# tjhladish/PLS

Hardware: AMD Instinct MI355X
Metric: NIPALS components/sec (higher is better)
Workload: dtype f64; 1 GPU; C3: synthetic tall n=1048576 x p=512, m=1, A=20, f64, resident in HBM; algo=nipals, fuse=1, deflation_written_back_every=1, rows_per_gpu=1048576, parallelism=single GPU

## Files before the change

pls_amd/csrc/ctx.hpp:

```cpp
#pragma once

namespace {

struct DevBuf {
    void *p = nullptr;
    size_t bytes = 0;
};

struct Launch {
    int fam;
    i64 bytes;
    hipEvent_t e0, e1;
};

}

struct pls_hip_context {
    int device = 0;
    hipStream_t stream = nullptr;
    pls_hip_allreduce_fn reducer = nullptr;
    void *reducer_user = nullptr;
    int rank = 0, nranks = 1;
    double *user_red = nullptr;
    i64 user_red_count = 0;
    i64 opt_algo = PLS_HIP_ALGO_KERNEL, opt_fuse = 1, opt_profile = 0, opt_power_iters = 48;
    i64 opt_fused_grid = 0, opt_work_layout = 1, opt_defer = 1, opt_graph = 0;
    std::vector<uint64_t> graph_key, graph_seen;
    hipGraphExec_t graph_exec = nullptr;
    DevBuf zeros, part, sspart, xbpart, wide1, red, red2, xx, xyp, praw, xy, v, cs, coop, lm, gxx, gxy, tab, work, cvidx, cvx, cvy, cvws, cve, cvtx, cvty, cvtt, cvm, cvkeep, cvred, hX, hY, hT, hW, hP, hQ, hR, hB, hIn, hOut;
    DevBuf valout, valpart, vale, valacc, valkeys, valhist;
    DevBuf xdS, xdQ, xdPT, xdred, xdtv, xdoQ, xdoT, xdoS, xdsmall;
    DevBuf bws, bv, bred, bmsg, bssy, bY, boR, boQ, bott, boB, bossy;
    DevBuf dG, dpart, dV, dT, dY, dZ, dC, dscr;
    DevBuf dcv;
    DevBuf dbat;
    DevBuf dcvb, cvbpos, cvbidx, cvbo, cvboE;
    DevBuf rsw, rsB, rsacc, rsX, rsY, rsW, rsoS;
    DevBuf mX, mws, mit, mzo;
    i64 opt_missing_iters = 500;
    int *mconv_host = nullptr;
    i64 opt_val_lds_rows = -1;
    i64 val_lds_rows_dev = -1;
    std::string err;
    std::vector<hipEvent_t> ev_pool;
    size_t ev_used = 0;
    std::vector<Launch> launches;
    std::vector<Launch> fits;
    Launch cur_fit{};
    bool fit_timed = false;
    int num_cu = 256;
    plsh::Stager stager;
    int copy_threads = 0;
    hipStream_t copy_stream = nullptr;
    const double *pre_xx = nullptr, *pre_xy = nullptr;
    bool defer_free = false;
    std::vector<void *> graveyard;
    struct XchgIpc *xchg = nullptr;
    struct XchgEndpoint {
        bool on = false;
        int n = 0, rank = 0;
        double *const *inbox = nullptr;
        unsigned long long *const *flags = nullptr;
        unsigned long long *seq = nullptr;
        int *status = nullptr, *host_status = nullptr;
        const long long *limit = nullptr;
    } xep;
    DevBuf tailcnt;
    DevBuf resident;
    DevBuf rgflags;
    unsigned rg_epoch = 0;
    unsigned long long resident_launches = 0;
    struct Env {
        bool turnaround = true;
        i64 turn_edge_bytes = plsk::TURN_EDGE_BYTES;
        bool batch_refit = false;
        i64 batch_round = 0;
        i64 dualcv_round = 0;
        i64 dualbatch_round = 0;
        i64 resample_round = 0;
        bool resample_refit = false;
        bool dualbatch_sweeps = false;
        bool cvbatch_refit = false;
        i64 dualcvb_round = 0;
        bool tiny = true, cv_refit = false, tail = true, replica_guard = true, resident = true;
        int tail_update = 1;
        int xb4 = 1;
        int resident_gram = 1;
    } env;
    int *diverged = nullptr, *diverged_dev = nullptr;
    DevBuf guard;
#ifdef PLS_HIP_TESTING
    int poison_new = -1;
#endif
};

#define PLS_HIP_WORKSPACES(SCRATCH, STATEFUL)                                                                                        \
    STATEFUL(zeros, WS_ALL, "256 zero bytes, cleared once when first used and only read afterwards: the source of out-of-range rows of the LDS-DMA panels") \
    STATEFUL(resident, 256, "two arrival counters of the resident fits, used in alternating parity (resident_launches): each launch zeroes the counter of the next; the payload behind the 256 bytes is scratch") \
    STATEFUL(rgflags, WS_ALL, "one arrival word per workgroup of resident_gram_fit_kernel: values only grow, a launch waits for words beyond rg_epoch, which the host advances by 4 per launch") \
    STATEFUL(gxx, c->pre_xx ? WS_ALL : 0, "X^T X accumulated during an upload, only while pre_xx points into it: from upload_accumulate to the end of the same host-memory fit") \
    STATEFUL(gxy, c->pre_xy ? WS_ALL : 0, "X^T Y accumulated during an upload, only while pre_xy points into it: from upload_accumulate to the end of the same host-memory fit") \
    SCRATCH(tailcnt) SCRATCH(part) SCRATCH(sspart) SCRATCH(xbpart) SCRATCH(wide1) SCRATCH(red) SCRATCH(red2) SCRATCH(xx) SCRATCH(xyp)  \
    SCRATCH(praw) SCRATCH(xy) SCRATCH(v) SCRATCH(cs) SCRATCH(coop) SCRATCH(lm) SCRATCH(tab) SCRATCH(work)                              \
    SCRATCH(cvidx) SCRATCH(cvx) SCRATCH(cvy) SCRATCH(cvws) SCRATCH(cve) SCRATCH(cvtx) SCRATCH(cvty) SCRATCH(cvtt) SCRATCH(cvm)         \
    SCRATCH(cvkeep) SCRATCH(cvred)                                                                                                     \
    SCRATCH(hX) SCRATCH(hY) SCRATCH(hT) SCRATCH(hW) SCRATCH(hP) SCRATCH(hQ) SCRATCH(hR) SCRATCH(hB) SCRATCH(hIn) SCRATCH(hOut)         \
    SCRATCH(valout) SCRATCH(valpart) SCRATCH(vale) SCRATCH(valacc) SCRATCH(valkeys) SCRATCH(valhist)                                   \
    SCRATCH(xdS) SCRATCH(xdQ) SCRATCH(xdPT) SCRATCH(xdred) SCRATCH(xdtv) SCRATCH(xdoQ) SCRATCH(xdoT) SCRATCH(xdoS) SCRATCH(xdsmall)    \
    SCRATCH(bws) SCRATCH(bv) SCRATCH(bred) SCRATCH(bmsg) SCRATCH(bssy) SCRATCH(bY) SCRATCH(boR) SCRATCH(boQ) SCRATCH(bott)             \
    SCRATCH(boB) SCRATCH(bossy)                                                                                                        \
    SCRATCH(dG) SCRATCH(dpart) SCRATCH(dV) SCRATCH(dT) SCRATCH(dY) SCRATCH(dZ) SCRATCH(dC) SCRATCH(dscr) SCRATCH(dcv) SCRATCH(dbat)    \
    SCRATCH(dcvb) SCRATCH(cvbpos) SCRATCH(cvbidx) SCRATCH(cvbo) SCRATCH(cvboE)                                                         \
    SCRATCH(rsw) SCRATCH(rsB) SCRATCH(rsacc) SCRATCH(rsX) SCRATCH(rsY) SCRATCH(rsW) SCRATCH(rsoS)                                      \
    SCRATCH(mX) SCRATCH(mws) SCRATCH(mit) SCRATCH(mzo)                                                                                 \
    SCRATCH(guard)

namespace {

constexpr size_t WS_ALL = ~(size_t)0;

template <typename F>
void for_each_workspace(pls_hip_context *c, F &&f) {
#define PLS_HIP_WS_SCRATCH(name) f(c->name, (size_t)0);
#define PLS_HIP_WS_STATEFUL(name, keep, reason) f(c->name, (size_t)(keep));
    PLS_HIP_WORKSPACES(PLS_HIP_WS_SCRATCH, PLS_HIP_WS_STATEFUL)
#undef PLS_HIP_WS_SCRATCH
#undef PLS_HIP_WS_STATEFUL
}

#define HIPCHK(ctx, call)                                                                  \
    do {                                                                                   \
        hipError_t e__ = (call);                                                           \
        if (e__ != hipSuccess) {                                                           \
            (ctx)->err = std::string(#call) + ": " + hipGetErrorString(e__);               \
            return PLS_HIP_ERR_DEVICE;                                                     \
        }                                                                                  \
    } while (0)

#define CHK(expr)                      \
    do {                               \
        int rc__ = (expr);             \
        if (rc__ != PLS_HIP_OK) return rc__; \
    } while (0)

int fail(pls_hip_context *c, int code, const std::string &msg) {
    c->err = msg;
    return code;
}

int ensure(pls_hip_context *c, DevBuf &b, size_t bytes) {
    if (bytes <= b.bytes && b.p) return PLS_HIP_OK;
    if (b.p) {
        if (c->defer_free) {
            c->graveyard.push_back(b.p);
        } else {
            HIPCHK(c, hipStreamSynchronize(c->stream));
            HIPCHK(c, hipFree(b.p));
        }
        b.p = nullptr;
        b.bytes = 0;
    }
    bytes = std::max<size_t>(bytes, 256);
    if (hipMalloc(&b.p, bytes) != hipSuccess) {
        (void)hipGetLastError();
        b.p = nullptr;
        return fail(c, PLS_HIP_ERR_ALLOC, "hipMalloc of " + std::to_string(bytes) + " bytes failed");
    }
    b.bytes = bytes;
#ifdef PLS_HIP_TESTING
    if (c->poison_new >= 0) {
        HIPCHK(c, hipMemsetAsync(b.p, c->poison_new, bytes, c->stream));
        HIPCHK(c, hipStreamSynchronize(c->stream));
    }
#endif
    return PLS_HIP_OK;
}

size_t esize(int dtype) { return dtype == PLS_HIP_F64 ? 8 : 4; }

hipEvent_t take_event(pls_hip_context *c) {
    if (c->ev_used == c->ev_pool.size()) {
        hipEvent_t e = nullptr;
        if (hipEventCreate(&e) != hipSuccess) return nullptr;
        c->ev_pool.push_back(e);
    }
    return c->ev_pool[c->ev_used++];
}
struct Scope {
    pls_hip_context *c;
    Launch l{};
    bool on;
    Scope(pls_hip_context *ctx, int fam, i64 bytes)
        : c(ctx), on(ctx->opt_profile >= 2 || (ctx->opt_profile == 1 && fam != PLS_HIP_FAM_SMALL)) {
        if (!on) return;
        l.fam = fam;
        l.bytes = bytes;
        l.e0 = take_event(c);
        l.e1 = take_event(c);
        if (!l.e0 || !l.e1) { on = false; return; }
        (void)hipEventRecord(l.e0, c->stream);
    }
    ~Scope() {
        if (!on) return;
        (void)hipEventRecord(l.e1, c->stream);
        c->launches.push_back(l);
    }
};

struct Roctx {
    int (*push)(const char *) = nullptr;
    int (*pop)() = nullptr;
    Roctx() {
        const char *e = getenv("PLS_HIP_ROCTX");
        if (!e || atoi(e) == 0) return;
        void *lib = dlopen("librocprofiler-sdk-roctx.so", RTLD_NOW | RTLD_GLOBAL);
        if (!lib) lib = dlopen("libroctx64.so", RTLD_NOW | RTLD_GLOBAL);
        if (!lib) return;
        push = reinterpret_cast<int (*)(const char *)>(dlsym(lib, "roctxRangePushA"));
        pop = reinterpret_cast<int (*)()>(dlsym(lib, "roctxRangePop"));
        if (!push || !pop) push = nullptr;
    }
};
inline Roctx &roctx() {
    static Roctx r;
    return r;
}
struct Range {
    bool on;
    explicit Range(const char *text) : on(roctx().push != nullptr) {
        if (on) roctx().push(text);
    }
    Range(const char *prefix, int n) : on(roctx().push != nullptr) {
        if (on) {
            char buf[64];
            std::snprintf(buf, sizeof(buf), "%s %d", prefix, n);
            roctx().push(buf);
        }
    }
    ~Range() {
        if (on) roctx().pop();
    }
};

#define LAUNCH_CHECK(ctx)                                                           \
    do {                                                                            \
        hipError_t e__ = hipGetLastError();                                         \
        if (e__ != hipSuccess) {                                                    \
            (ctx)->err = std::string("kernel launch: ") + hipGetErrorString(e__);   \
            return PLS_HIP_ERR_DEVICE;                                              \
        }                                                                           \
    } while (0)

}
```

pls_amd/csrc/fused_kernels.hpp:

```cpp
#pragma once
#include <type_traits>

#include "common.hpp"
#include "exchange_kernels.hpp"
#include "update_m1.hpp"

namespace plsk {

#ifdef PLS_HIP_TESTING
__device__ unsigned long long *g_pass_stamps = nullptr;
#define PLS_STAMP(slot)                                                                                 \
    do {                                                                                                \
        if (g_pass_stamps && threadIdx.x == 0) {                                                        \
            g_pass_stamps[(size_t)blockIdx.x * 8 + (slot)] = wall_clock64();                            \
            if ((slot) == 0) {         \
                g_pass_stamps[(size_t)blockIdx.x * 8 + 4] = __builtin_amdgcn_s_getreg((31 << 11) | 20);  \
                g_pass_stamps[(size_t)blockIdx.x * 8 + 5] = __builtin_amdgcn_s_getreg((31 << 11) | 4);   \
            }                                                                                           \
        }                                                                                               \
    } while (0)
#else
#define PLS_STAMP(slot) do { } while (0)
#endif

typedef unsigned int u32x4 __attribute__((ext_vector_type(4)));

constexpr int BUF_WORD3 = 0x00020000;
constexpr int AUX_SC1 = 16;

template <typename T, int V, int AUX = 0>
__device__ __forceinline__ Pack<T, V> buf_ld(__amdgpu_buffer_rsrc_t r, uint32_t voff) {
    static_assert(sizeof(Pack<T, V>) == 16, "16-byte accesses");
    const u32x4 raw = __builtin_amdgcn_raw_buffer_load_b128(r, voff, 0, AUX);
    Pack<T, V> p;
    __builtin_memcpy(&p, &raw, 16);
    return p;
}
template <typename T, int V, int AUX = 0>
__device__ __forceinline__ void buf_st(__amdgpu_buffer_rsrc_t r, uint32_t voff, const Pack<T, V> &p) {
    u32x4 raw;
    __builtin_memcpy(&raw, &p, 16);
    __builtin_amdgcn_raw_buffer_store_b128(raw, r, voff, 0, AUX);
}
template <typename T, int V, int AUX = 0>
__device__ __forceinline__ Pack<T, V> buf_ld_so(__amdgpu_buffer_rsrc_t r, uint32_t voff, int soff) {
    static_assert(sizeof(Pack<T, V>) == 16, "16-byte accesses");
    const u32x4 raw = __builtin_amdgcn_raw_buffer_load_b128(r, voff, soff, AUX);
    Pack<T, V> p;
    __builtin_memcpy(&p, &raw, 16);
    return p;
}
template <typename T, int V, int AUX = 0>
__device__ __forceinline__ void buf_st_so(__amdgpu_buffer_rsrc_t r, uint32_t voff, int soff, const Pack<T, V> &p) {
    u32x4 raw;
    __builtin_memcpy(&raw, &p, 16);
    __builtin_amdgcn_raw_buffer_store_b128(raw, r, voff, soff, AUX);
}

template <typename T, int V>
__device__ __forceinline__ Pack<T, V> ld_pack_u(const T *p) {
    Pack<T, V> o;
    __builtin_memcpy(&o, p, sizeof(o));
    return o;
}
template <typename T, int V>
__device__ __forceinline__ void st_pack_u(T *p, const Pack<T, V> &x) {
    __builtin_memcpy(p, &x, sizeof(x));
}

template <typename T>
__device__ __forceinline__ __amdgpu_buffer_rsrc_t score_rsrc(const T *col, i64 nvalid) {
    return __builtin_amdgcn_make_buffer_rsrc(const_cast<T *>(col), (short)0, (int)(nvalid * (i64)sizeof(T)), BUF_WORD3);
}

struct TailUpdate {
    double *XY = nullptr;
    double *W = nullptr, *P = nullptr, *Q = nullptr, *R = nullptr, *vnext = nullptr;
    int A = 0, a = 0, nipals = 0;
};

struct WalkWeights {
    int nfull = -1;
    unsigned mask = 0;
    int rev = 0;
    int edge = 0;
};

struct Turn {
    bool on = false;
    bool rev = false;
    i64 edge_bytes = 0;
};

#ifdef PLS_HIP_TESTING
struct TurnRecord {
    int rev = 0, edge = 0, ntiles = 0, grid = 0;
};
inline TurnRecord g_test_turn;
#endif

struct SliceTail {
    unsigned *cnt = nullptr;
    double *red = nullptr;
    int nrows = 0;
    int npush = 0;
    unsigned long long seq = 0;
    XchgPeers peers;
    TailUpdate upd;
    XchgGather gx;
};

constexpr int TAIL_MIN_WG = 32;
constexpr int TAIL_AUX_SYS = 17;

__device__ __noinline__ void tail_update_m1(const double *src, i64 stride, int n, int sys, int ok, double *XY, double *W, double *P,
                                            double *Q, double *R, double *vnext, int K, int A, int a, int nipals, double *scratch,
                                            double *wl) {
    typedef unsigned int u32x2 __attribute__((ext_vector_type(2)));
    static_assert(XCHG_MAX == 2 * RED_SLICES, "two batches of RED_SLICES loads");
    const int L = K + 1;
    update_m1<512, 1>(
        [&](int j) -> double {
            double sum = 0.0;
#pragma unroll
            for (int h = 0; h < 2; ++h) {
                if (h * RED_SLICES >= n) break;
                double x[RED_SLICES];
#pragma unroll
                for (int m = 0; m < RED_SLICES; ++m) {
                    const int mm = h * RED_SLICES + m;
                    const __amdgpu_buffer_rsrc_t rs = __builtin_amdgcn_make_buffer_rsrc(
                        const_cast<double *>(src + (i64)(mm < n ? mm : 0) * stride), (short)0, L * 8, BUF_WORD3);
                    const u32x2 raw = sys ? __builtin_amdgcn_raw_buffer_load_b64(rs, (uint32_t)j * 8u, 0, TAIL_AUX_SYS)
                                          : __builtin_amdgcn_raw_buffer_load_b64(rs, (uint32_t)j * 8u, 0, AUX_SC1);
                    __builtin_memcpy(&x[m], &raw, 8);
                }
#pragma unroll
                for (int m = 0; m < RED_SLICES; ++m)
                    if (h * RED_SLICES + m < n) sum += x[m];
            }
            return ok ? sum : __builtin_nan("");
        },
        XY, W, P, Q, R, vnext, K, A, a, nipals, 0, scratch + UPD1_VWAVES, scratch, wl);
}

template <int NT>
__device__ __forceinline__ void slice_tail(const SliceTail &st, const double *part, const double *sspart, int K, int *role,
                                        double *sm, double *scratch, double *wl) {
    static_assert(NT >= WG, "the t^T t sum takes the first four waves");
    const int tid = threadIdx.x, nb = st.nrows, nwg = gridDim.x, b = blockIdx.x;
    constexpr int NSL = RED_SLICES;
    const int sl = (int)(((i64)(b + 1) * NSL + nb - 1) / nb) - 1;
    if (tid == 0) {
        const int lo_ = (int)((i64)nb * sl / NSL), hi_ = (int)((i64)nb * (sl + 1) / NSL);
        const unsigned mine = (unsigned)(min(hi_, nwg) - lo_);
        const unsigned ticket = __hip_atomic_fetch_add(st.cnt + sl, 1u, __ATOMIC_RELAXED, __HIP_MEMORY_SCOPE_AGENT);
        const int last = (ticket + 1u == mine);
        if (last) {
            __hip_atomic_store(st.cnt + sl, 0u, __ATOMIC_RELAXED, __HIP_MEMORY_SCOPE_AGENT);
        }
        *role = last;
    }
    __syncthreads();
    if (!*role) return;
    const i64 LP = K + 1;
    typedef unsigned int u32x2 __attribute__((ext_vector_type(2)));
    {
        const int s8 = sl;
        const int lo = (int)((i64)nb * s8 / RED_SLICES), hi = (int)((i64)nb * (s8 + 1) / RED_SLICES);
        double ssl = 0.0;
        {
            const __amdgpu_buffer_rsrc_t rq =
                __builtin_amdgcn_make_buffer_rsrc(const_cast<double *>(sspart), (short)0, nb * 8, BUF_WORD3);
            if (tid < WG)
                for (int r = lo + tid; r < hi; r += WG) {
                    const u32x2 raw = __builtin_amdgcn_raw_buffer_load_b64(rq, (uint32_t)r * 8u, 0, AUX_SC1);
                    double d;
                    __builtin_memcpy(&d, &raw, 8);
                    ssl += d;
                }
        }
        {
            const __amdgpu_buffer_rsrc_t rs = __builtin_amdgcn_make_buffer_rsrc(const_cast<double *>(part + (i64)lo * K), (short)0,
                                                                                (int)((i64)(hi - lo) * K * 8), BUF_WORD3);
            auto ld = [&](int row, int j) -> double {
                const u32x2 raw = __builtin_amdgcn_raw_buffer_load_b64(rs, (uint32_t)(((i64)row * K + j) * 8), 0, AUX_SC1);
                double d;
                __builtin_memcpy(&d, &raw, 8);
                return d;
            };
            const int nr = hi - lo;
            for (int j = tid; j < K; j += NT) {
                double c[4] = {0.0, 0.0, 0.0, 0.0};
                int r = 0;
                for (; r + 16 <= nr; r += 16) {
                    double x[16];
#pragma unroll
                    for (int u = 0; u < 16; ++u) x[u] = ld(r + u, j);
#pragma unroll
                    for (int u = 0; u < 16; ++u) c[u & 3] += x[u];
                }
                for (; r < nr; r += 4) {
                    double x[4];
#pragma unroll
                    for (int u = 0; u < 4; ++u) x[u] = (r + u < nr) ? ld(r + u, j) : 0.0;
#pragma unroll
                    for (int u = 0; u < 4; ++u)
                        if (r + u < nr) c[u] += x[u];
                }
                st_agent(st.red + (i64)s8 * LP + j, (c[0] + c[1]) + (c[2] + c[3]));
            }
        }
        {
            double sw = wave_sum(ssl);
            __syncthreads();
            if ((tid & 63) == 0 && tid < WG) sm[tid >> 6] = sw;
            __syncthreads();
            if (tid == 0) st_agent(st.red + (i64)s8 * LP + K, ((sm[0] + sm[1]) + sm[2]) + sm[3]);
        }
    }
    if (st.npush <= 0 && !st.upd.XY) return;
    asm volatile("s_waitcnt vmcnt(0)" ::: "memory");
    __syncthreads();
    {
        if (tid == 0) {
            const unsigned ticket = __hip_atomic_fetch_add(st.cnt + RED_SLICES, 1u, __ATOMIC_RELAXED, __HIP_MEMORY_SCOPE_AGENT);
            const int last = (ticket + 1u == (unsigned)NSL);
            if (last) {
                __hip_atomic_store(st.cnt + RED_SLICES, 0u, __ATOMIC_RELAXED, __HIP_MEMORY_SCOPE_AGENT);
            }
            *role = last;
        }
        __syncthreads();
        if (!*role) return;
    }
    const __amdgpu_buffer_rsrc_t rr =
        __builtin_amdgcn_make_buffer_rsrc(st.red, (short)0, (int)((i64)RED_SLICES * LP * 8), BUF_WORD3);
    if (st.npush > 0) {
        for (int j = tid; j <= K; j += NT) {
            double x[RED_SLICES];
#pragma unroll
            for (int i = 0; i < RED_SLICES; ++i) {
                const u32x2 raw = __builtin_amdgcn_raw_buffer_load_b64(rr, (uint32_t)(((i64)i * LP + j) * 8), 0, AUX_SC1);
                __builtin_memcpy(&x[i], &raw, 8);
            }
            double sum = x[0];
#pragma unroll
            for (int i = 1; i < RED_SLICES; ++i) sum += x[i];
            for (int d = 0; d < st.npush; ++d) __hip_atomic_store(st.peers.slot[d] + j, sum, __ATOMIC_RELAXED, __HIP_MEMORY_SCOPE_SYSTEM);
        }
        asm volatile("s_waitcnt vmcnt(0)" ::: "memory");
        __syncthreads();
        if (tid < st.npush) __hip_atomic_store(st.peers.flag[tid], st.seq, __ATOMIC_RELEASE, __HIP_MEMORY_SCOPE_SYSTEM);
    }
    if (!st.upd.XY) return;
    const TailUpdate &u = st.upd;
    if (st.gx.n > 0) {
        const XchgGather &gx = st.gx;
        if (tid == 0) *role = (*gx.status == 0);
        __syncthreads();
        if (tid < gx.n && *role) {
            const long long t0 = wall_clock64();
            while (__hip_atomic_load(gx.flags + tid, __ATOMIC_RELAXED, __HIP_MEMORY_SCOPE_SYSTEM) < gx.seq) {
                if (wall_clock64() - t0 > gx.limit) {
                    *role = 0;
                    break;
                }
                __builtin_amdgcn_s_sleep(4);
            }
            __builtin_amdgcn_fence(__ATOMIC_ACQUIRE, "");
            asm volatile("s_waitcnt vmcnt(0)" ::: "memory");
        }
        __syncthreads();
        const int ok = *role;
        if (!ok && tid == 0) {
            *gx.status = 1;
            __hip_atomic_store(gx.host_status, 1, __ATOMIC_RELAXED, __HIP_MEMORY_SCOPE_SYSTEM);
        }
        tail_update_m1(gx.inbox, gx.cap, gx.n, 1, ok, u.XY, u.W, u.P, u.Q, u.R, u.vnext, K, u.A, u.a, u.nipals, scratch, wl);
        return;
    }
    tail_update_m1(st.red, LP, RED_SLICES, 0, 1, u.XY, u.W, u.P, u.Q, u.R, u.vnext, K, u.A, u.a, u.nipals, scratch, wl);
}

constexpr int AUX_NT = 2;
constexpr i64 TURN_EDGE_BYTES = 192ll << 20;
constexpr bool TURN_LEAD_ST_DEFAULT = true;

template <bool XCD, int R>
struct TileWalk {
    __device__ __forceinline__ explicit TileWalk(i64) {}
    __device__ __forceinline__ unsigned first() const { return blockIdx.x; }
    __device__ __forceinline__ unsigned step() const { return gridDim.x; }
    __device__ __forceinline__ i64 nlim(i64 N) const { return N; }
};
template <int R>
struct TileWalk<true, R> {
    i64 first_, step_, nlim_;
    __device__ __forceinline__ explicit TileWalk(i64 N) : first_(blockIdx.x), step_(gridDim.x), nlim_(N) {
        if ((gridDim.x & 7) == 0) {
            const i64 per = ((N + R - 1) / R + 7) / 8;
            first_ = (i64)(blockIdx.x & 7) * per + (blockIdx.x >> 3);
            step_ = gridDim.x >> 3;
            nlim_ = min(N, (i64)((blockIdx.x & 7) + 1) * per * R);
        }
    }
    __device__ __forceinline__ i64 first() const { return first_; }
    __device__ __forceinline__ i64 step() const { return step_; }
    __device__ __forceinline__ i64 nlim(i64) const { return nlim_; }
};

template <typename T, int V, int R, int NT, int CPT, bool DEFL, int LDAUX_ = AUX_NT, int STAUX = AUX_NT, bool RDST = false,
          int EDGE = 0, bool TILED = false, bool ONEWG = false, bool STORE = true>
__global__ __launch_bounds__(NT, (NT / 256) * ((CPT <= 16 && !DEFL && !ONEWG) ? 2 : 1)) void fused_pass_kernel(
    const T *X, i64 ldx, i64 tsx, T *dst, i64 ldd, i64 tsd, i64 N, int K,
    const double *__restrict__ v, const T *__restrict__ tprev, const double *__restrict__ pprev,
    T *__restrict__ tout, double *__restrict__ part, double *__restrict__ sspart, int rdst, i64 NV, const SliceTail st,
    const WalkWeights wk) {
    constexpr int RP = R / V;
    constexpr int CG = NT / RP;
    constexpr int NW = NT / WAVE;
    constexpr int LDAUX = (EDGE == 2) ? 0 : LDAUX_;
    static_assert(RP <= WAVE && WAVE % RP == 0 && NT % RP == 0, "tile shape");
    static_assert(!TILED || (EDGE == 0 && !RDST), "the tiled copy is aligned and keeps one tile shape");
    static_assert(STORE || (DEFL && !RDST), "only a deflating pass has a store side to drop; without it there is no destination tile shape");
    constexpr bool DYN = (size_t)2 * CG * CPT * sizeof(double) > 48 * 1024;
    struct alignas(16) Lds {
        alignas(16) double ps[(DEFL && !DYN) ? CG * CPT : 2];
        alignas(16) double vs[DYN ? 2 : CG * CPT];
        alignas(16) double tred[2][NW][R];
        alignas(16) double sred[NW];
    };
    __shared__ Lds lds;
    extern __shared__ double fused_dyn[];
    double *vs = DYN ? fused_dyn : lds.vs, *ps = DYN ? fused_dyn + CG * CPT : lds.ps;
    auto &tred = lds.tred;
    double *sred = lds.sred;

    const int tid = threadIdx.x, lane = tid & 63, wv = tid >> 6;
    const int rp = tid % RP, cg = tid / RP;
    PLS_STAMP(0);
    constexpr bool LATE_OK = TILED && DEFL && CG * CPT <= NT;
    const bool LATE_FILL = LATE_OK && (rdst & 0x10000);
    double v_late = 0.0, p_late = 0.0;
    if (LATE_FILL) {
        if (tid < CG * CPT) {
            v_late = (tid < K) ? v[tid] : 0.0;
            p_late = (tid < K) ? pprev[tid] : 0.0;
        }
    } else {
        for (int k = tid; k < CG * CPT; k += NT) {
            vs[k] = (k < K) ? v[k] : 0.0;
            if (DEFL) ps[k] = (k < K) ? pprev[k] : 0.0;
        }
        __syncthreads();
    }
    bool first_tile = true;

    double pacc[CPT];
#pragma unroll
    for (int j = 0; j < CPT; ++j) pacc[j] = 0.0;
    double ss = 0.0;
    int buf = 0;
    constexpr int CGD = EDGE ? WAVE / RP : CG;
    const int cgw = EDGE ? __builtin_amdgcn_readfirstlane(cg) : 0;
    const uint32_t xoff = (uint32_t)(((i64)rp * V + (i64)(cg - cgw) * ldx) * (i64)sizeof(T));
    uint32_t doff = (DEFL && STORE) ? (uint32_t)(((i64)rp * V + (i64)cg * ldd) * (i64)sizeof(T)) : 0u;
    i64 dtile = tsd;
    if constexpr (RDST && DEFL) {
        doff = (uint32_t)(((i64)((rp * V) / rdst) * tsd + (rp * V) % rdst + (i64)cg * ldd) * (i64)sizeof(T));
        dtile = (R / rdst) * tsd;
    }
    constexpr uint32_t OOR = 0x80000000u;
    constexpr bool TBUF = DEFL && sizeof(T) == 8 && R == 32 && CPT == 16;
    const __amdgpu_buffer_rsrc_t rs_tin = score_rsrc<T>(DEFL ? tprev : tout, NV);

    TileWalk<EDGE == 2, R> walk(N);
    const int pace = rdst & 0xffff;
    constexpr bool WEIGHTED = DEFL && EDGE != 2;
    const int wfast = (WEIGHTED && wk.nfull >= 0) ? ((wk.mask >> (blockIdx.x & 7)) & 1) : 0;
    const i64 wswitch = (WEIGHTED && wk.nfull >= 0) ? (i64)wk.nfull * gridDim.x : (i64)1 << 62;
    i64 wstep = walk.step();
    bool wshared = true;
    constexpr bool TURNS = DEFL;
    constexpr bool EDGES = TILED && DEFL && STORE;
    const bool rev = TURNS && wk.rev;
    const i64 ntl = (N + R - 1) / R;
    const i64 etrail = ntl - wk.edge;
    for (i64 pos = walk.first(); pos * R < walk.nlim(N); buf ^= 1) {
        const i64 tile = rev ? ntl - 1 - pos : pos;
        if constexpr (EDGES) {
            if (pos < wk.edge) {
                constexpr int LA = 0, SA = TURN_LEAD_ST_DEFAULT ? 0 : STAUX;
#include "fused_pass_tile.inc"
            } else if (pos >= etrail) {
                constexpr int LA = 0, SA = 0;
#include "fused_pass_tile.inc"
            } else {
                constexpr int LA = LDAUX, SA = STAUX;
#include "fused_pass_tile.inc"
            }
        } else {
            constexpr int LA = LDAUX, SA = STAUX;
#include "fused_pass_tile.inc"
        }
        if constexpr (!WEIGHTED) {
            pos += walk.step();
            continue;
        }
        pos += wstep;
        if (wshared && pos >= wswitch) {
            if (!wfast) break;
            wshared = false;
            const int nfc = __builtin_popcount(wk.mask), below = __builtin_popcount(wk.mask & ((1u << (blockIdx.x & 7)) - 1u));
            pos = wswitch + (i64)(blockIdx.x >> 3) * nfc + below;
            wstep = (i64)(gridDim.x >> 3) * nfc;
        }
    }

    PLS_STAMP(1);
#pragma unroll
    for (int j = 0; j < CPT; ++j) {
        const double s = xor_range_sum<1, RP>(pacc[j]);
        const int k = cg + CG * j;
        if (rp == 0 && k < K) st_agent(part + (i64)blockIdx.x * K + k, s);
    }
    ss = block_sum<NW>(ss, sred);
    if (tid == 0) st_agent(sspart + blockIdx.x, ss);
    constexpr bool ONE_PER_CU = !(CPT <= 16 && !DEFL) || ONEWG;
    if (ONE_PER_CU && st.cnt) {
        asm volatile("s_waitcnt vmcnt(0)" ::: "memory");
        __syncthreads();
        static_assert(NT == 512, "tail_update_m1 plays the update's 1024 virtual threads with 512");
        PLS_STAMP(2);
        slice_tail<NT>(st, part, sspart, K, reinterpret_cast<int *>(sred + NW - 1), sred, &tred[0][0][0], vs);
    }
    PLS_STAMP(3);
}

template <typename T, int V, int R, int NT, int CPT, int EDGE = 0>
__global__ __launch_bounds__(NT, (NT / 256) * 2) void deflate_score_kernel(
    const T *src, i64 lds_, i64 tss, T *dst, i64 ldd, i64 tsd, int rdst, i64 N, int K, const T *__restrict__ tprev,
    const double *__restrict__ pprev, const double *__restrict__ w, T *__restrict__ tout,
    double *__restrict__ sspart, i64 NV) {
    constexpr int RP = R / V, CG = NT / RP, NW = NT / WAVE;
    extern __shared__ double dyn[];
    __shared__ double tred[2][NW][R];
    __shared__ double sred[NW];
    double *ws = dyn, *ps = dyn + K;
    const int tid = threadIdx.x, lane = tid & 63, wv = tid >> 6;
    const int rp = tid % RP, cg = tid / RP;
    for (int k = tid; k < K; k += NT) {
        ws[k] = w[k];
        ps[k] = pprev[k];
    }
    __syncthreads();
    constexpr int CGD = EDGE ? WAVE / RP : CG;
    constexpr int LDAUX = (EDGE == 2) ? 0 : AUX_NT;
    const int cgw = EDGE ? __builtin_amdgcn_readfirstlane(cg) : 0;
    const uint32_t soff = (uint32_t)(((i64)rp * V + (i64)(cg - cgw) * lds_) * (i64)sizeof(T));
    const int dsub = (rp * V) / rdst, dwithin = (rp * V) % rdst, dtiles = R / rdst;
    const uint32_t doff = (uint32_t)(((i64)dsub * tsd + dwithin + (i64)cg * ldd) * (i64)sizeof(T));
    constexpr uint32_t OOR = 0x80000000u;
    const int ngroups = (K + CG - 1) / CG;
    const __amdgpu_buffer_rsrc_t rs_tin = score_rsrc<T>(tprev, NV);
    double ss = 0.0;
    int buf = 0;
    TileWalk<EDGE == 2, R> walk(N);
    for (i64 tile = walk.first(); tile * R < walk.nlim(N); tile += walk.step(), buf ^= 1) {
        const i64 i0 = tile * R + (i64)rp * V;
        const bool rowok = (i0 < N);
        const uint32_t so = rowok ? soff : OOR, dof = rowok ? doff : OOR;
        double tp[V], tacc[V];
        {
            const Pack<T, V> tpk = buf_ld<T, V>(rs_tin, rowok ? (uint32_t)(i0 * (i64)sizeof(T)) : OOR);
#pragma unroll
            for (int e = 0; e < V; ++e) tp[e] = -(double)tpk.v[e];
        }
#pragma unroll
        for (int e = 0; e < V; ++e) tacc[e] = 0.0;
        for (int g0 = 0; g0 < ngroups; g0 += CPT) {
            Pack<T, V> x[CPT];
#pragma unroll
            for (int j = 0; j < CPT; ++j) {
                const int cols = min(CGD, K - CG * (g0 + j) - cgw);
                const uint32_t nrec = cols > 0 ? (uint32_t)((i64)cols * lds_ * (i64)sizeof(T)) : 0u;
                const __amdgpu_buffer_rsrc_t rs = __builtin_amdgcn_make_buffer_rsrc(
                    const_cast<T *>(src + tile * tss + (i64)((g0 + j) * CG + cgw) * lds_), (short)0, (int)nrec, BUF_WORD3);
                x[j] = buf_ld<T, V, LDAUX>(rs, so);
                __builtin_amdgcn_sched_barrier(0);
            }
#pragma unroll
            for (int j = 0; j < CPT; ++j) {
                const int k = cg + CG * (g0 + j);
                const double pk = (k < K) ? ps[k] : 0.0, wk = (k < K) ? ws[k] : 0.0;
#pragma unroll
                for (int e = 0; e < V; ++e) {
                    x[j].v[e] = (T)fma(tp[e], pk, (double)x[j].v[e]);
                    tacc[e] = fma((double)x[j].v[e], wk, tacc[e]);
                }
                const __amdgpu_buffer_rsrc_t rd = __builtin_amdgcn_make_buffer_rsrc(
                    dst + tile * dtiles * tsd + (i64)(g0 + j) * CG * ldd, (short)0, 0x7fffffff, BUF_WORD3);
                buf_st<T, V, AUX_NT>(rd, (k < K) ? dof : OOR, x[j]);
            }
        }
#pragma unroll
        for (int e = 0; e < V; ++e)
            tacc[e] = xor_range_sum<RP, WAVE>(tacc[e]);
        if (lane < RP)
#pragma unroll
            for (int e = 0; e < V; ++e) tred[buf][wv][rp * V + e] = tacc[e];
        __syncthreads();
        if (cg == 0 && rowok) {
            Pack<T, V> o;
#pragma unroll
            for (int e = 0; e < V; ++e) {
                double s = 0.0;
#pragma unroll
                for (int q = 0; q < NW; ++q) s += tred[buf][q][rp * V + e];
                o.v[e] = (T)s;
                const double ts = (double)o.v[e];
                ss = fma(ts, ts, ss);
            }
            if (i0 + V <= NV) {
                st_pack_u<T, V>(tout + i0, o);
            } else {
#pragma unroll
                for (int e = 0; e < V; ++e)
                    if (i0 + e < NV) tout[i0 + e] = o.v[e];
            }
        }
    }
    ss = block_sum<NW>(ss, sred);
    if (tid == 0) sspart[blockIdx.x] = ss;
}

template <typename T>
struct TailArgs {
    const T *src = nullptr; i64 lds = 0, tss = 0; int rs = 1;
    T *dst = nullptr; i64 ldd = 0, tsd = 0; int rd = 1;
    const T *tprev = nullptr; const double *pprev = nullptr;
    const double *v = nullptr; T *tout = nullptr; const T *tgiven = nullptr;
    double *part = nullptr, *sspart = nullptr;
    const T *Y = nullptr; i64 ldy = 0; int M = 0;
    i64 row0 = 0; int nrows = 0, K = 0;
    int zero_rows = 0;
};

template <typename T>
__global__ __launch_bounds__(WG) void tail_rows_kernel(TailArgs<T> a) {
    __shared__ double sm[WG / WAVE];
    constexpr int MAXR = 16 / sizeof(T) - 1;
    double t[MAXR];
    double ss = 0.0;
    for (int r = 0; r < MAXR; ++r) {
        t[r] = 0.0;
        if (r >= a.nrows) continue;
        const i64 i = a.row0 + r;
        const T *srow = a.src + (i / a.rs) * a.tss + i % a.rs;
        T *drow = a.dst ? a.dst + (i / a.rd) * a.tsd + i % a.rd : nullptr;
        const double tp = a.tprev ? -(double)a.tprev[i] : 0.0;
        double sum = 0.0;
        for (int k = threadIdx.x; k < a.K; k += WG) {
            T x = srow[(i64)k * a.lds];
            if (a.tprev) x = (T)fma(tp, a.pprev[k], (double)x);
            if (drow) drow[(i64)k * a.ldd] = x;
            if (a.v) sum = fma((double)x, a.v[k], sum);
        }
        if (a.v) {
            t[r] = (double)(T)block_sum<WG / WAVE>(sum, sm);
            if (threadIdx.x == 0 && a.tout) a.tout[i] = (T)t[r];
        } else if (a.tgiven) {
            t[r] = (double)a.tgiven[i];
        }
        ss = fma(t[r], t[r], ss);
    }
    if (a.dst)
        for (int r = 0; r < a.zero_rows; ++r) {
            const i64 i = a.row0 + a.nrows + r;
            T *drow = a.dst + (i / a.rd) * a.tsd + i % a.rd;
            for (int k = threadIdx.x; k < a.K; k += WG) drow[(i64)k * a.ldd] = (T)0;
        }
    if (a.part) {
        const int nm = a.Y ? a.M : 1;
        for (int k = threadIdx.x; k < a.K; k += WG)
            for (int m = 0; m < nm; ++m) {
                double p = 0.0;
                for (int r = 0; r < MAXR; ++r)
                    if (r < a.nrows) {
                        const i64 i = a.row0 + r;
                        double x;
                        if (a.dst) {
                            x = (double)a.dst[(i / a.rd) * a.tsd + i % a.rd + (i64)k * a.ldd];
                        } else {
                            const T xs = a.src[(i / a.rs) * a.tss + i % a.rs + (i64)k * a.lds];
                            x = a.tprev ? (double)(T)fma(-(double)a.tprev[i], a.pprev[k], (double)xs) : (double)xs;
                        }
                        p = fma(x, a.Y ? (double)a.Y[i + (i64)m * a.ldy] : t[r], p);
                    }
                a.part[k + (i64)m * a.K] = p;
            }
    }
    if (a.sspart && threadIdx.x == 0) *a.sspart = ss;
}

template <typename T>
void launch_tail_rows(hipStream_t stream, const TailArgs<T> &a) {
    hipLaunchKernelGGL((tail_rows_kernel<T>), dim3(1), dim3(WG), 0, stream, a);
}

template <typename T, int V, int R, int NT, int CPTB, int MT, int EDGE = 0, bool LT = false>
__global__ __launch_bounds__(NT, NT / 256) void retile_xty_kernel(const T *src, i64 lds_, const T *__restrict__ Y,
                                                                        i64 ldy, T *dst, i64 ldd, i64 tsd, int rdst, i64 N,
                                                                        int K, int M, double *__restrict__ part, int tpw) {
    constexpr int RP = R / V, CG = NT / RP;
    constexpr int LDAUX = (EDGE == 2) ? 0 : AUX_NT;
    constexpr bool YLDS = MT >= 4;
    constexpr int TU = (CPTB < 8) ? 2 : 1;
    constexpr int YE = (TU * R * MT + NT - 1) / NT;
    __shared__ alignas(16) T ys[2][YLDS ? TU * MT : 1][YLDS ? R : V];
    extern __shared__ __attribute__((aligned(16))) unsigned char retile_dyn[];
    Pack<T, V> *trans = reinterpret_cast<Pack<T, V> *>(retile_dyn);
    constexpr int W = CG * CPTB;
    static_assert(!LT || (W % 16 == 0 && (RP * W) % NT == 0 && RP <= 16), "transposed store shape");
    const int rp = threadIdx.x % RP, cg = threadIdx.x / RP;
    const int g0 = blockIdx.y * CPTB;
    constexpr int CGD = EDGE ? WAVE / RP : CG;
    const int cgw = EDGE ? __builtin_amdgcn_readfirstlane(cg) : 0;
    const uint32_t soff = (uint32_t)(((i64)rp * V + (i64)(cg - cgw) * lds_) * (i64)sizeof(T));
    const int dsub = (rp * V) / rdst, dwithin = (rp * V) % rdst, dtiles = R / rdst;
    const uint32_t doff = (uint32_t)(((i64)dsub * tsd + dwithin + (i64)cg * ldd) * (i64)sizeof(T));
    constexpr uint32_t OOR = 0x80000000u;
    const i64 ntiles = (N + R - 1) / R;
    const i64 tile0 = (i64)blockIdx.x * tpw, tile1 = min(ntiles, tile0 + (i64)tpw);
    double acc[CPTB][MT];
#pragma unroll
    for (int j = 0; j < CPTB; ++j)
#pragma unroll
        for (int m = 0; m < MT; ++m) acc[j][m] = 0.0;
    int buf = 0;
    for (i64 tile = tile0; tile < tile1; tile += TU, buf ^= 1) {
        Pack<T, V> x[TU][CPTB];
#pragma unroll
        for (int u = 0; u < TU; ++u) {
            const bool rowok = (tile + u < tile1) && ((tile + u) * R + (i64)rp * V < N);
#pragma unroll
            for (int j = 0; j < CPTB; ++j) {
                const int cols = min(CGD, K - CG * (g0 + j) - cgw);
                const uint32_t nrec = cols > 0 ? (uint32_t)((i64)cols * lds_ * (i64)sizeof(T)) : 0u;
// ... 32 lines not shown
                __syncthreads();
#pragma unroll
                for (int j = 0; j < CPTB; ++j) trans[rp * W + ((cg + CG * j) ^ rp)] = x[u][j];
                __syncthreads();
                const __amdgpu_buffer_rsrc_t rd =
                    __builtin_amdgcn_make_buffer_rsrc(dst + (tile + u) * dtiles * tsd, (short)0, 0x7fffffff, BUF_WORD3);
                const int Q = rdst / V;
#pragma unroll
                for (int jj = 0; jj < RP * W / NT; ++jj) {
                    const int L = jj * NT + (int)threadIdx.x;
                    const int d = L / (W * Q), rem = L - d * (W * Q);
                    const int c = (Q == 1) ? rem : (rem >> 1), q = (Q == 1) ? 0 : (rem & 1);
                    const int rp2 = d * Q + q;
                    const Pack<T, V> pk = trans[rp2 * W + (c ^ rp2)];
                    const int k = g0 * CG + c;
                    const bool ok = (tile + u < tile1) && ((tile + u) * R + (i64)rp2 * V < N) && (k < K);
                    const uint32_t off = (uint32_t)(((i64)d * tsd + (i64)q * V + (i64)k * ldd) * (i64)sizeof(T));
                    buf_st<T, V, AUX_NT>(rd, ok ? off : OOR, pk);
                }
            }
#pragma unroll
            for (int m = 0; m < MT; ++m) {
                Pack<T, V> yp;
                if constexpr (YLDS) {
                    yp = *reinterpret_cast<const Pack<T, V> *>(&ys[buf][u * MT + m][rp * V]);
                } else {
                    if (m < M && rowok) {
                        yp = ld_pack_u<T, V>(Y + i0 + (i64)m * ldy);
                    } else {
#pragma unroll
                        for (int e = 0; e < V; ++e) yp.v[e] = (T)0;
                    }
                }
#pragma unroll
                for (int e = 0; e < V; ++e) {
                    const double ye = (double)yp.v[e];
#pragma unroll
                    for (int j = 0; j < CPTB; ++j) acc[j][m] = fma((double)x[u][j].v[e], ye, acc[j][m]);
                }
            }
        }
    }
#pragma unroll
    for (int j = 0; j < CPTB; ++j) {
        const int k = cg + CG * (g0 + j);
#pragma unroll
        for (int m = 0; m < MT; ++m) {
            const double s = xor_range_sum<1, RP>(acc[j][m]);
            if (rp == 0 && k < K && m < M) part[(i64)blockIdx.x * ((i64)K * M) + k + (i64)m * K] = s;
        }
    }
}

template <typename T, int CGX = 32>
int launch_retile_xty(hipStream_t stream, int num_cu, const T *src, i64 lds_, const T *Y, i64 ldy, T *dst, i64 ldd, i64 tsd,
                      int rdst, i64 N, int K, int M, double *part, int max_rows, int *nb) {
    constexpr int V = 16 / sizeof(T);
    constexpr int R = (512 / CGX) * V, NT = 512;
    constexpr int CG = NT / (R / V);
    const bool nostore = dst == nullptr;
    if (nostore) { ldd = R; tsd = (i64)R * K; rdst = R; }
    if ((!nostore && !cols_aligned((uintptr_t)dst, ldd, sizeof(T))) || tsd % V != 0 || rdst < V || R % rdst != 0 || N < 1 || M < 1 || M > 8 || max_rows < 2 ||
        !elem_aligned((uintptr_t)Y, sizeof(T)))
        return 1;
    const int edge = edge_level((uintptr_t)src, lds_, sizeof(T), CG, WAVE / (R / V));
    if (edge < 0) return 1;
    if (!nostore && ((i64)(R / rdst) * tsd + (i64)CG * ldd) * (i64)sizeof(T) >= (1ll << 31)) return 1;
    const i64 Nf = N - N % V;
    int gx = 0;
    if (Nf > 0) {
        const i64 ntiles = (Nf + R - 1) / R;
        const int cptb = (M > 4 || (M > 2 && sizeof(T) == 4)) ? 4 : 8;
        const int nkb = (K + CG * cptb - 1) / (CG * cptb);
        const i64 want = std::max<i64>(1, std::min<i64>(((i64)(nostore ? 4 : 1) * num_cu + nkb - 1) / nkb, max_rows - 1));
        const i64 tpw = (ntiles + want - 1) / want;
        gx = (int)((ntiles + tpw - 1) / tpw);
        const dim3 g((unsigned)gx, (unsigned)nkb), b(NT);
        const bool lt = CGX == 32 && rdst == V && M <= 2 && !nostore;
#define RX_LAUNCH(CPTB_, MT_, E_) \
    hipLaunchKernelGGL((retile_xty_kernel<T, V, R, NT, CPTB_, MT_, E_>), g, b, 0, stream, src, lds_, Y, ldy, dst, ldd, tsd, rdst, Nf, K, M, part, (int)tpw)
#define RX_LAUNCH_LT(CPTB_, MT_, E_)                                                                                      \
    do {                                                                                                                  \
        if constexpr (CGX == 32) {                                                                                        \
            auto kfn = &retile_xty_kernel<T, V, R, NT, CPTB_, MT_, E_, true>;                                             \
            const int dynb = (R / V) * CG * CPTB_ * 16;                                                                   \
            if (dynb > 48 * 1024 && !raise_dynamic_lds(reinterpret_cast<const void *>(kfn), dynb)) return 1;              \
            hipLaunchKernelGGL(kfn, g, b, dynb, stream, src, lds_, Y, ldy, dst, ldd, tsd, rdst, Nf, K, M, part, (int)tpw); \
        }                                                                                                                 \
    } while (0)
#define RX_CASE(CPTB_, MT_)                                                                                               \
    do {                                                                                                                  \
        if (lt) { if (edge == 2) RX_LAUNCH_LT(CPTB_, MT_, 2); else if (edge) RX_LAUNCH_LT(CPTB_, MT_, 1); else RX_LAUNCH_LT(CPTB_, MT_, 0); } \
        else if (edge == 2) RX_LAUNCH(CPTB_, MT_, 2); else if (edge) RX_LAUNCH(CPTB_, MT_, 1); else RX_LAUNCH(CPTB_, MT_, 0); \
    } while (0)
#define RX_CASE_D(CPTB_, MT_) \
    do { if (edge == 2) RX_LAUNCH(CPTB_, MT_, 2); else if (edge) RX_LAUNCH(CPTB_, MT_, 1); else RX_LAUNCH(CPTB_, MT_, 0); } while (0)
        if (M > 4) RX_CASE_D(4, 8);
        else if (M > 2 && cptb == 4) RX_CASE_D(4, 4);
        else if (M > 2) RX_CASE_D(8, 4);
        else if (M > 1) RX_CASE(8, 2);
        else RX_CASE(8, 1);
#undef RX_CASE_D
#undef RX_CASE
#undef RX_LAUNCH_LT
#undef RX_LAUNCH
    }
    if (Nf < N) {
        TailArgs<T> a;
        a.src = src; a.lds = lds_; a.tss = R; a.rs = R;
        a.dst = dst; a.ldd = ldd; a.tsd = tsd; a.rd = rdst;
        a.part = part + (i64)gx * K * M; a.Y = Y; a.ldy = ldy; a.M = M;
        a.row0 = Nf; a.nrows = (int)(N - Nf); a.K = K; a.zero_rows = V - a.nrows;
        launch_tail_rows(stream, a);
        ++gx;
    }
    *nb = gx;
    return 0;
}

template <typename T>
int launch_deflate_score(hipStream_t stream, int num_cu, const T *src, i64 lds_, i64 tss, T *dst, i64 ldd, i64 tsd,
                         int rdst, i64 N, int K, const T *tprev, const double *pprev, const double *w, T *tout,
                         double *sspart, int max_rows, int *nss, bool src_padded = false) {
    constexpr int V = 16 / sizeof(T);
    constexpr int R = 256 / sizeof(T), NT = 512, CPT = 8;
    constexpr int CG = NT / (R / V);
    if (N < 1 || max_rows < 2 || !cols_aligned((uintptr_t)dst, ldd, sizeof(T)) || !elem_aligned((uintptr_t)tprev, sizeof(T)) || !elem_aligned((uintptr_t)tout, sizeof(T))) return 1;
    if ((N + V) * (i64)sizeof(T) >= (1ll << 31)) return 1;
    const int edge = edge_level((uintptr_t)src, lds_, sizeof(T), CG, WAVE / (R / V));
    if (edge < 0 || (edge == 0 && tss % V != 0)) return 1;
    if (tsd % V != 0 || rdst < V || R % rdst != 0) return 1;
    if (((i64)(R / rdst) * tsd + (i64)CG * ldd) * (i64)sizeof(T) >= (1ll << 31)) return 1;
    if ((i64)CG * ldd * (i64)sizeof(T) >= (1ll << 31)) return 1;
    const size_t dyn = (size_t)K * 16;
    if (dyn > 72 * 1024) return 1;
    auto kfn = edge == 2 ? &deflate_score_kernel<T, V, R, NT, CPT, 2>
                         : (edge == 1 ? &deflate_score_kernel<T, V, R, NT, CPT, 1> : &deflate_score_kernel<T, V, R, NT, CPT, 0>);
    if (dyn > 48 * 1024 && !raise_dynamic_lds(reinterpret_cast<const void *>(kfn), 72 * 1024)) return 1;
    const i64 Nf = src_padded ? (N + V - 1) / V * V : N - N % V;
    i64 grid = 0;
    if (Nf > 0) {
        const i64 ntiles = (Nf + R - 1) / R;
        grid = std::min<i64>(std::min<i64>(ntiles, 2 * (i64)num_cu), max_rows - 1);
        hipLaunchKernelGGL(kfn, dim3((unsigned)grid), dim3(NT), (size_t)K * 16, stream, src, lds_, tss, dst, ldd, tsd, rdst, Nf,
                           K, tprev, pprev, w, tout, sspart, N);
    }
    if (Nf < N) {
        TailArgs<T> a;
        a.src = src; a.lds = lds_; a.tss = tss; a.rs = R;
        a.dst = dst; a.ldd = ldd; a.tsd = tsd; a.rd = rdst;
        a.tprev = tprev; a.pprev = pprev; a.v = w; a.tout = tout; a.sspart = sspart + grid;
        a.row0 = Nf; a.nrows = (int)(N - Nf); a.K = K; a.zero_rows = V - a.nrows;
        launch_tail_rows(stream, a);
        ++grid;
    }
    *nss = (int)grid;
    return 0;
}

template <typename T, int V, int R, int NT, int CPT, int EDGE = 0>
__global__ __launch_bounds__(NT, (NT / 256) * 2) void retile_kernel(const T *src, i64 lds_, T *dst, i64 ldd, i64 tsd,
                                                                    int rdst, i64 N, int K) {
    constexpr int RP = R / V, CG = NT / RP;
    constexpr int CGD = EDGE ? WAVE / RP : CG;
    constexpr int LDAUX = (EDGE == 2) ? 0 : AUX_NT;
    const int rp = threadIdx.x % RP, cg = threadIdx.x / RP;
    const int cgw = EDGE ? __builtin_amdgcn_readfirstlane(cg) : 0;
    const uint32_t soff = (uint32_t)(((i64)rp * V + (i64)(cg - cgw) * lds_) * (i64)sizeof(T));
    const int dsub = (rp * V) / rdst, dwithin = (rp * V) % rdst, dtiles = R / rdst;
    const uint32_t doff = (uint32_t)(((i64)dsub * tsd + dwithin + (i64)cg * ldd) * (i64)sizeof(T));
    constexpr uint32_t OOR = 0x80000000u;
    const int ngroups = (K + CG - 1) / CG;
    TileWalk<EDGE == 2, R> walk(N);
    for (i64 tile = walk.first(); tile * R < walk.nlim(N); tile += walk.step()) {
        const bool rowok = (tile * R + (i64)rp * V < N);
        const uint32_t so = rowok ? soff : OOR, dof = rowok ? doff : OOR;
        for (int g0 = 0; g0 < ngroups; g0 += CPT) {
            Pack<T, V> x[CPT];
#pragma unroll
            for (int j = 0; j < CPT; ++j) {
                const int cols = min(CGD, K - CG * (g0 + j) - cgw);
                const uint32_t nrec = cols > 0 ? (uint32_t)((i64)cols * lds_ * (i64)sizeof(T)) : 0u;
                const __amdgpu_buffer_rsrc_t rs = __builtin_amdgcn_make_buffer_rsrc(
                    const_cast<T *>(src + tile * R + (i64)((g0 + j) * CG + cgw) * lds_), (short)0, (int)nrec, BUF_WORD3);
                x[j] = buf_ld<T, V, LDAUX>(rs, so);
                __builtin_amdgcn_sched_barrier(0);
            }
#pragma unroll
            for (int j = 0; j < CPT; ++j) {
                const int k = cg + CG * (g0 + j);
                const __amdgpu_buffer_rsrc_t rd = __builtin_amdgcn_make_buffer_rsrc(
                    dst + tile * dtiles * tsd + (i64)(g0 + j) * CG * ldd, (short)0, 0x7fffffff, BUF_WORD3);
                buf_st<T, V, AUX_NT>(rd, (k < K) ? dof : OOR, x[j]);
            }
        }
    }
}

template <typename T>
int launch_retile(hipStream_t stream, int num_cu, const T *src, i64 lds_, T *dst, i64 ldd, i64 tsd, int rdst, i64 N,
                  int K) {
    constexpr int V = 16 / sizeof(T);
    constexpr int R = 256 / sizeof(T), NT = 512, CPT = 8;
    constexpr int CG = NT / (R / V);
    if (!cols_aligned((uintptr_t)dst, ldd, sizeof(T)) || tsd % V != 0 || rdst < V || R % rdst != 0 || N < 1) return 1;
    const int edge = edge_level((uintptr_t)src, lds_, sizeof(T), CG, WAVE / (R / V));
    if (edge < 0) return 1;
    if (((i64)(R / rdst) * tsd + (i64)CG * ldd) * (i64)sizeof(T) >= (1ll << 31)) return 1;
    const i64 Nf = N - N % V;
    if (Nf > 0) {
        const i64 ntiles = (Nf + R - 1) / R;
        const i64 grid = std::min<i64>(ntiles, 2 * (i64)num_cu);
        auto kfn = edge == 2 ? &retile_kernel<T, V, R, NT, CPT, 2>
                             : (edge == 1 ? &retile_kernel<T, V, R, NT, CPT, 1> : &retile_kernel<T, V, R, NT, CPT, 0>);
        hipLaunchKernelGGL(kfn, dim3((unsigned)grid), dim3(NT), 0, stream, src, lds_, dst, ldd, tsd, rdst, Nf, K);
    }
    if (Nf < N) {
        TailArgs<T> a;
        a.src = src; a.lds = lds_; a.tss = R; a.rs = R;
        a.dst = dst; a.ldd = ldd; a.tsd = tsd; a.rd = rdst;
        a.row0 = Nf; a.nrows = (int)(N - Nf); a.K = K; a.zero_rows = V - a.nrows;
        launch_tail_rows(stream, a);
    }
    return 0;
}

template <typename T, int V, int R, int NT, int CPT>
__global__ __launch_bounds__(NT, (NT / 256) * 2) void xty_tiled_kernel(const T *X, i64 ldx, i64 tsx, i64 N, int K,
                                                                       const T *__restrict__ t,
                                                                       double *__restrict__ part, int tpw, i64 NV) {
    constexpr int RP = R / V, CG = NT / RP;
    const int rp = threadIdx.x % RP, cg = threadIdx.x / RP;
    const int g0 = blockIdx.y * CPT;
    const i64 ntiles = (N + R - 1) / R;
    const i64 tile0 = (i64)blockIdx.x * tpw, tile1 = min(ntiles, tile0 + (i64)tpw);
    const uint32_t xoff = (uint32_t)(((i64)rp * V + (i64)cg * ldx) * (i64)sizeof(T));
    constexpr uint32_t OOR = 0x80000000u;
    const __amdgpu_buffer_rsrc_t rs_t = score_rsrc<T>(t, NV);
    double pacc[CPT];
#pragma unroll
    for (int j = 0; j < CPT; ++j) pacc[j] = 0.0;
    for (i64 tile = tile0; tile < tile1; ++tile) {
        const i64 i0 = tile * R + (i64)rp * V;
        const bool rowok = (i0 < N);
        const uint32_t xo = rowok ? xoff : OOR;
        Pack<T, V> x[CPT];
#pragma unroll
        for (int j = 0; j < CPT; ++j) {
            const int cols = min(CG, K - CG * (g0 + j));
            const uint32_t nrec = cols > 0 ? (uint32_t)((i64)cols * ldx * (i64)sizeof(T)) : 0u;
            const __amdgpu_buffer_rsrc_t rs = __builtin_amdgcn_make_buffer_rsrc(
                const_cast<T *>(X + tile * tsx + (i64)(g0 + j) * CG * ldx), (short)0, (int)nrec, BUF_WORD3);
            x[j] = buf_ld<T, V, AUX_NT>(rs, xo);
            __builtin_amdgcn_sched_barrier(0);
        }
        double tv[V];
        {
            const Pack<T, V> tpk = buf_ld<T, V>(rs_t, rowok ? (uint32_t)(i0 * (i64)sizeof(T)) : OOR);
#pragma unroll
            for (int e = 0; e < V; ++e) tv[e] = (double)tpk.v[e];
        }
#pragma unroll
        for (int j = 0; j < CPT; ++j)
#pragma unroll
            for (int e = 0; e < V; ++e) pacc[j] = fma((double)x[j].v[e], tv[e], pacc[j]);
    }
#pragma unroll
    for (int j = 0; j < CPT; ++j) {
        const double s = xor_range_sum<1, RP>(pacc[j]);
        const int k = cg + CG * (g0 + j);
        if (rp == 0 && k < K) part[(i64)blockIdx.x * K + k] = s;
    }
}

template <typename T, int CGX = 32>
int launch_xty_tiled(hipStream_t stream, int num_cu, const T *X, i64 ldx, i64 tsx, i64 N, int K, const T *t,
                     double *part, int max_rows, int *nb) {
    constexpr int V = 16 / sizeof(T);
    constexpr int R = (512 / CGX) * V, NT = 512, CPT = 16;
    constexpr int CG = NT / (R / V);
    if (!cols_aligned((uintptr_t)X, ldx, sizeof(T)) || !elem_aligned((uintptr_t)t, sizeof(T)) || tsx % V != 0 || N < 1 || max_rows < 2) return 1;
    if ((N + V) * (i64)sizeof(T) >= (1ll << 31)) return 1;
    if ((i64)CG * ldx * (i64)sizeof(T) >= (1ll << 31)) return 1;
    const i64 Nf = (N + V - 1) / V * V;
    const i64 ntiles = (Nf + R - 1) / R;
    const int nkb = (K + CG * CPT - 1) / (CG * CPT);
    const i64 want = std::max<i64>(1, std::min<i64>((8 * (i64)num_cu + nkb - 1) / nkb, max_rows));
    const i64 tpw = (ntiles + want - 1) / want;
    const i64 gx = (ntiles + tpw - 1) / tpw;
    hipLaunchKernelGGL((xty_tiled_kernel<T, V, R, NT, CPT>), dim3((unsigned)gx, (unsigned)nkb), dim3(NT), 0, stream, X,
                       ldx, tsx, Nf, K, t, part, (int)tpw, N);
    *nb = (int)gx;
    return 0;
}

template <typename T, int CGX = 32>
constexpr int tile_rows() { return (512 / CGX) * (16 / (int)sizeof(T)); }

template <typename T, int CGX = 32>
int launch_fused_pass(hipStream_t stream, int num_cu, const T *X, i64 ldx, i64 tsx, T *dst, i64 ldd, i64 tsd,
                      i64 N, int K, const double *v, const T *tprev, const double *pprev, T *tout,
                      double *part, int max_rows, double *sspart, int *nb, int *nss, int grid_hint, int rdst = 0,
                      bool src_padded = false, const SliceTail *tail = nullptr, bool *tail_used = nullptr,
                      bool *upd_done = nullptr, bool store = true, const Turn &turn = Turn()) {
    constexpr int V = 16 / sizeof(T);
    constexpr int R = tile_rows<T, CGX>(), NT = 512;
    constexpr int CG = NT / (R / V);
    static_assert(CG == CGX, "tile shape");
    const bool defl = (tprev != nullptr);
    const bool stores = defl && store;
    if (!stores) dst = nullptr;
    if (!elem_aligned((uintptr_t)tout, sizeof(T)) || (defl && !elem_aligned((uintptr_t)tprev, sizeof(T))) || (stores && !cols_aligned((uintptr_t)dst, ldd, sizeof(T)))) return 1;
    int edge = edge_level((uintptr_t)X, ldx, sizeof(T), CG, WAVE / (R / V));
    if (edge < 0 || (edge == 0 && tsx % V != 0) || (stores && tsd % V != 0)) return 1;
    if (K > CG * ((CGX == 64 || CGX == 128 || CGX == 256 || CGX < 32 || (CGX == 512 && defl)) ? 16 : 32) || N < 1 || max_rows < 2) return 1;
    if ((N + V) * (i64)sizeof(T) >= (1ll << 31)) return 1;
    if (stores && (i64)CG * ldd * (i64)sizeof(T) >= (1ll << 31)) return 1;
    if (rdst > 0 && (CGX != 32 || !stores || rdst < V || R % rdst != 0 ||
                     ((i64)(R / rdst) * tsd + (i64)CG * ldd) * (i64)sizeof(T) >= (1ll << 31)))
        return 1;
    if (CGX > 32 && edge != 0) return 1;
    if constexpr (CGX == 32) {
        if (rdst > 0 && K <= CG * 16) return 1;
    }
    const i64 Nf = src_padded ? (N + V - 1) / V * V : N - N % V;
    i64 grid = 0;
    if (tail_used) *tail_used = false;
    if (upd_done) *upd_done = false;
    if (Nf > 0) {
        const i64 ntiles = (Nf + R - 1) / R;
        const bool onewg = !defl && K <= CG * 16 && CGX <= 64 && edge == 0 && tail && tail->cnt && rdst == 0 &&
                           ntiles >= (i64)num_cu && (double)ntiles * R * K * sizeof(T) <= 1.5e9;
        const int per_cu = (K <= CG * 16 && !defl && !onewg) ? 2 : 1;
        grid = grid_hint > 0 ? grid_hint : per_cu * (i64)num_cu;
        grid = std::min<i64>(std::min<i64>(grid, ntiles), max_rows - 1);
        if (grid < 1) return 1;
        const dim3 g((unsigned)grid), b(NT);
        SliceTail st;
        if (tail && tail->cnt && grid >= TAIL_MIN_WG && per_cu == 1 && grid <= (i64)num_cu) {
            st = *tail;
            st.nrows = (int)grid + (Nf < N ? 1 : 0);
            if (tail_used) *tail_used = true;
            if (st.upd.XY && upd_done && K <= UPD1_VTHREADS && 2 * (NT / WAVE) * R >= UPD1_VWAVES + st.upd.A) {
                *upd_done = true;
            } else {
                st.upd.XY = nullptr;
                st.gx.n = 0;
            }
        }
        if (Nf < N) {
            TailArgs<T> a;
            a.src = X; a.lds = ldx; a.tss = tsx; a.rs = R;
            if (defl) {
                if (stores) { a.dst = dst; a.ldd = ldd; a.tsd = tsd; a.rd = rdst > 0 ? rdst : R; }
                a.tprev = tprev; a.pprev = pprev;
            }
            a.v = v; a.tout = tout; a.part = part + grid * K; a.sspart = sspart + grid;
            a.row0 = Nf; a.nrows = (int)(N - Nf); a.K = K; a.zero_rows = V - a.nrows;
            launch_tail_rows(stream, a);
        }
        const bool tiled = defl && edge == 0 && rdst == 0 && ldx == R && tsx == (i64)R * K && (!stores || (ldd == R && tsd == (i64)R * K));
        WalkWeights wk;
        {
            constexpr double rho = 1.08;
            constexpr unsigned fast_mask = 0x55u;
            const int nfc = __builtin_popcount(fast_mask);
            if (defl && per_cu == 1 && grid == (i64)num_cu && grid % 8 == 0 && edge != 2 && ntiles >= 2 * grid) {
                const double share = (double)ntiles / ((double)grid * (1.0 + (rho - 1.0) * nfc / 8.0));
                wk.nfull = (int)std::max<i64>(1, std::min<i64>((i64)(share + 0.5), ntiles / grid));
                wk.mask = fast_mask;
            }
        }
        if (turn.on && defl) {
            wk.rev = turn.rev ? 1 : 0;
            if (tiled) {
                const i64 round_bytes = grid * (i64)R * K * (i64)sizeof(T);
                const i64 epos = turn.edge_bytes / round_bytes * grid;
                wk.edge = (int)(2 * epos >= ntiles ? ntiles : epos);
            }
        }
#ifdef PLS_HIP_TESTING
        if (stores) g_test_turn = TurnRecord{wk.rev, wk.edge, (int)ntiles, (int)grid};
#endif
        if (CGX > 32 && defl && !tiled) return 1;
#define FUSED_LAUNCH(CPT_, DEFL_, EDGE_, TILED_, STORE_, dyn_)                                                            \
    do {                                                                                                                  \
        if constexpr (!(DEFL_) && (CPT_) <= 16 && CGX <= 64 && (EDGE_) == 0) {                                            \
            if (onewg) {                                                                                                  \
                auto kfn1 = &fused_pass_kernel<T, V, R, NT, CPT_, DEFL_, AUX_NT, AUX_NT, false, EDGE_, TILED_, true>;     \
                hipLaunchKernelGGL(kfn1, g, b, dyn_, stream, X, ldx, tsx, dst, ldd, tsd, Nf, K, v, tprev, pprev, tout, part, sspart, 0, N, st, wk); \
                break;                                                                                                    \
            }                                                                                                             \
        }                                                                                                                 \
        auto kfn = &fused_pass_kernel<T, V, R, NT, CPT_, DEFL_, AUX_NT, AUX_NT, false, EDGE_, TILED_, false, STORE_>;    \
        if ((dyn_) > 48 * 1024 && !raise_dynamic_lds(reinterpret_cast<const void *>(kfn), (int)(dyn_))) return 1;         \
        hipLaunchKernelGGL(kfn, g, b, dyn_, stream, X, ldx, tsx, dst, ldd, tsd, Nf, K, v, tprev, pprev, tout, part, sspart, (TILED_) ? ((STORE_) ? 2 * (CPT_) : 0) | 0x10000 : 0, N, st, wk); \
    } while (0)
#define FUSED_EDGE(CPT_, DEFL_, STORE_, dyn_)                                                                             \
    do {                                                                                                                  \
        if constexpr (DEFL_) {                                                                                            \
            if (tiled) { FUSED_LAUNCH(CPT_, DEFL_, 0, true, STORE_, dyn_); break; }                                       \
        }                                                                                                                 \
        if constexpr (CGX <= 32) {                                                                                        \
            if (edge == 2) { FUSED_LAUNCH(CPT_, DEFL_, 2, false, STORE_, dyn_); break; }                                  \
            if (edge == 1) { FUSED_LAUNCH(CPT_, DEFL_, 1, false, STORE_, dyn_); break; }                                  \
        }                                                                                                                 \
        if constexpr (CGX <= 32 || !DEFL_) FUSED_LAUNCH(CPT_, DEFL_, 0, false, STORE_, dyn_);                             \
    } while (0)
#define FUSED_CASE(CPT_)                                                                                                  \
    do {                                                                                                                  \
        const size_t dyn = ((size_t)2 * CG * CPT_ * sizeof(double) > 48 * 1024) ? (size_t)2 * CG * CPT_ * sizeof(double) : 0; \
        if (stores) FUSED_EDGE(CPT_, true, true, dyn);                                                                    \
        else if (defl) FUSED_EDGE(CPT_, true, false, dyn);                        \
        else FUSED_EDGE(CPT_, false, true, (CGX >= 512 ? dyn / 2 : dyn));    \
    } while (0)
        if constexpr (CGX == 32) {
            if (rdst > 0) {
                auto kfn = edge == 2 ? &fused_pass_kernel<T, V, R, NT, 32, true, AUX_NT, AUX_NT, true, 2>
                                     : (edge == 1 ? &fused_pass_kernel<T, V, R, NT, 32, true, AUX_NT, AUX_NT, true, 1>
                                                  : &fused_pass_kernel<T, V, R, NT, 32, true, AUX_NT, AUX_NT, true, 0>);
                hipLaunchKernelGGL(kfn, g, b, 0, stream, X, ldx, tsx, dst, ldd, tsd, Nf, K, v, tprev, pprev, tout, part, sspart, rdst, N, st, wk);
            } else if (K <= CG * 4) FUSED_CASE(4);
            else if (K <= CG * 8) FUSED_CASE(8);
            else if (K <= CG * 12) FUSED_CASE(12);
            else if (K <= CG * 16) FUSED_CASE(16);
            else if (K <= CG * 24) FUSED_CASE(24);
            else FUSED_CASE(32);
        } else if constexpr (CGX == 64 || CGX == 128) {
            if (K <= CG * 12) FUSED_CASE(12);
            else FUSED_CASE(16);
        } else if constexpr (CGX == 8) {
            if (K <= CG * 4) FUSED_CASE(4);
            else if (K <= CG * 8) FUSED_CASE(8);
            else if (K <= CG * 12) FUSED_CASE(12);
            else FUSED_CASE(16);
        } else if constexpr (CGX == 16) {
            if (K <= CG * 12) FUSED_CASE(12);
            else FUSED_CASE(16);
        } else if constexpr (CGX == 512) {
            if (K <= CG * 12) FUSED_CASE(12);
            else if (K <= CG * 16) FUSED_CASE(16);
            else FUSED_EDGE(32, false, true, (size_t)CG * 32 * sizeof(double));
        } else {
            if (K <= CG * 12) FUSED_CASE(12);
            else FUSED_CASE(16);
        }
#undef FUSED_CASE
#undef FUSED_EDGE
#undef FUSED_LAUNCH
    }
    if (Nf < N) {
        if (Nf <= 0) {
            TailArgs<T> a;
            a.src = X; a.lds = ldx; a.tss = tsx; a.rs = R;
            if (defl) {
                if (stores) { a.dst = dst; a.ldd = ldd; a.tsd = tsd; a.rd = rdst > 0 ? rdst : R; }
                a.tprev = tprev; a.pprev = pprev;
            }
            a.v = v; a.tout = tout; a.part = part + grid * K; a.sspart = sspart + grid;
            a.row0 = Nf; a.nrows = (int)(N - Nf); a.K = K; a.zero_rows = V - a.nrows;
            launch_tail_rows(stream, a);
        }
        ++grid;
    }
    *nb = (int)grid;
    *nss = (int)grid;
    return 0;
}

}
```

pls_amd/csrc/fused_pass_tile.inc:

```
        const i64 i0 = tile * R + (i64)rp * V;
        const bool rowok = (i0 < N);
        const uint32_t xo = rowok ? xoff : OOR, dof = rowok ? doff : OOR;
        int cgz = cg;
        asm volatile("" : "+v"(cgz));
        if constexpr (TILED && DEFL && STORE) {
            if (!LATE_FILL || !first_tile)
                for (int q = 0; q < pace; ++q) __builtin_amdgcn_s_sleep(1);
        }
        Pack<T, V> x[CPT];
        constexpr int GSTEP = CG * R * (int)sizeof(T);
        const int trec = K * R * (int)sizeof(T);
        if constexpr (TILED) {
            const __amdgpu_buffer_rsrc_t rs =
                __builtin_amdgcn_make_buffer_rsrc(const_cast<T *>(X + tile * tsx), (short)0, trec, BUF_WORD3);
#pragma unroll
            for (int j = 0; j < CPT; ++j) x[j] = buf_ld_so<T, V, LA>(rs, xo, j * GSTEP);
            __builtin_amdgcn_sched_barrier(0);
            if constexpr (LATE_OK) {
                if (LATE_FILL && first_tile) {
                    first_tile = false;
                    if (tid < CG * CPT) {
                        vs[tid] = v_late;
                        ps[tid] = p_late;
                    }
                    __syncthreads();
                }
            }
        } else {
#pragma unroll
            for (int j = 0; j < CPT; ++j) {
                const int cols = min(CGD, K - CG * j - cgw);
                const uint32_t nrec = cols > 0 ? (uint32_t)((i64)cols * ldx * (i64)sizeof(T)) : 0u;
                const __amdgpu_buffer_rsrc_t rs = __builtin_amdgcn_make_buffer_rsrc(
                    const_cast<T *>(X + tile * tsx + (i64)(j * CG + cgw) * ldx), (short)0, (int)nrec, BUF_WORD3);
                x[j] = buf_ld<T, V, LA>(rs, xo);
                __builtin_amdgcn_sched_barrier(0);
            }
        }
        if (DEFL) {
            double tp[V];
            {
                Pack<T, V> tpk;
                if constexpr (TBUF) {
                    tpk = buf_ld<T, V>(rs_tin, rowok ? (uint32_t)(i0 * (i64)sizeof(T)) : OOR);
                } else if (rowok && i0 + V <= NV) {
                    tpk = ld_pack_u<T, V>(tprev + i0);
                } else {
#pragma unroll
                    for (int e = 0; e < V; ++e) tpk.v[e] = (rowok && i0 + e < NV) ? tprev[i0 + e] : (T)0;
                }
#pragma unroll
                for (int e = 0; e < V; ++e) tp[e] = -(double)tpk.v[e];
            }
#pragma unroll
            for (int j = 0; j < CPT; ++j) {
                const double pk = ps[cgz + CG * j];
#pragma unroll
                for (int e = 0; e < V; ++e) x[j].v[e] = (T)fma(tp[e], pk, (double)x[j].v[e]);
                if constexpr (!STORE) {
                    continue;
                } else if constexpr (TILED) {
                    const __amdgpu_buffer_rsrc_t rd =
                        __builtin_amdgcn_make_buffer_rsrc(dst + tile * tsd, (short)0, trec, BUF_WORD3);
                    buf_st_so<T, V, SA>(rd, dof, j * GSTEP, x[j]);
                } else if constexpr (RDST) {
                    const __amdgpu_buffer_rsrc_t rd = __builtin_amdgcn_make_buffer_rsrc(
                        dst + tile * dtile + (i64)j * CG * ldd, (short)0, 0x7fffffff, BUF_WORD3);
                    buf_st<T, V, SA>(rd, (cg + CG * j < K) ? dof : OOR, x[j]);
                } else {
                    const int cols = min(CG, K - CG * j);
                    const uint32_t nrec = cols > 0 ? (uint32_t)((i64)cols * ldd * (i64)sizeof(T)) : 0u;
                    const __amdgpu_buffer_rsrc_t rd = __builtin_amdgcn_make_buffer_rsrc(
                        dst + tile * tsd + (i64)j * CG * ldd, (short)0, (int)nrec, BUF_WORD3);
                    buf_st<T, V, SA>(rd, dof, x[j]);
                }
            }
        }
        if constexpr (DEFL && STORE) __builtin_amdgcn_sched_barrier(0);
        double tp2[V];
#pragma unroll
        for (int e = 0; e < V; ++e) tp2[e] = 0.0;
#pragma unroll
        for (int j = 0; j < CPT; ++j) {
            const double vk = vs[cgz + CG * j];
#pragma unroll
            for (int e = 0; e < V; ++e) tp2[e] = fma((double)x[j].v[e], vk, tp2[e]);
        }
#pragma unroll
        for (int e = 0; e < V; ++e)
            tp2[e] = xor_range_sum<RP, WAVE>(tp2[e]);
        if (lane < RP)
#pragma unroll
            for (int e = 0; e < V; ++e) tred[buf][wv][rp * V + e] = tp2[e];
        __syncthreads();
        double t[V];
#pragma unroll
        for (int e = 0; e < V; ++e) {
            double s = 0.0;
#pragma unroll
            for (int w = 0; w < NW; ++w) s += tred[buf][w][rp * V + e];
            t[e] = (double)(T)s;
        }
        if (cg == 0 && rowok) {
            Pack<T, V> o;
#pragma unroll
            for (int e = 0; e < V; ++e) o.v[e] = (T)t[e];
            if (i0 + V <= NV) {
                st_pack_u<T, V>(tout + i0, o);
            } else {
#pragma unroll
                for (int e = 0; e < V; ++e)
                    if (i0 + e < NV) tout[i0 + e] = o.v[e];
            }
#pragma unroll
            for (int e = 0; e < V; ++e) ss = fma(t[e], t[e], ss);
        }
        if (sizeof(T) < sizeof(double)) {
#pragma unroll
            for (int j = 0; j < CPT; ++j)
#pragma unroll
                for (int e = 0; e < V; ++e) asm volatile("" : "+v"(x[j].v[e]));
        }
#pragma unroll
        for (int j = 0; j < CPT; ++j)
#pragma unroll
            for (int e = 0; e < V; ++e) pacc[j] = fma((double)x[j].v[e], t[e], pacc[j]);
```

pls_amd/csrc/launch_update.hpp:

```cpp
#pragma once

namespace {

constexpr i64 ROTATE_SPLIT_MIN = 16384;

int launch_update_large(pls_hip_context *c, const double *red, double *XY, double *W, double *P, double *Q, double *R,
                        double *v, int K, int M, int A, int a, int nip) {
    const i64 MM = (i64)M * M;
    const int nparts = (K + plsk::WG - 1) / plsk::WG;
    const i64 prows = max_partial_rows(c, K, M);
    const size_t need = (size_t)(3 * MM + 2 * M + nparts + 8 + K + prows * MM + (i64)plsk::RED_SLICES * MM) * 8;
    CHK(ensure(c, c->lm, need));
    double *G = (double *)c->lm.p, *Bm = G + MM, *Cm = Bm + MM, *qe = Cm + MM, *qv = qe + M, *ssp = qv + M;
    double *tr = ssp + nparts, *wraw = tr + 8, *xpart = wraw + K, *xred = xpart + prows * MM;
    const dim3 blk(plsk::WG);
    Scope s(c, PLS_HIP_FAM_SMALL, ((i64)K * M * 4 + MM * 3 * c->opt_power_iters) * 8);
    if (a >= 0) {
        hipLaunchKernelGGL(plsk::lm_pq_kernel, dim3(M + nparts), blk, 0, c->stream, red, (const double *)XY, (const double *)R, P,
                           Q, qv, K, M, a);
        LAUNCH_CHECK(c);
        hipLaunchKernelGGL(plsk::lm_deflate_kernel, dim3((unsigned)(((i64)K * M + plsk::WG - 1) / plsk::WG)), blk, 0, c->stream,
                           red, XY, (const double *)P, (const double *)qv, K, M, a);
        LAUNCH_CHECK(c);
    } else {
        hipLaunchKernelGGL(plsk::sum_slices_kernel, dim3((unsigned)(((i64)K * M + plsk::WG - 1) / plsk::WG)), blk, 0, c->stream,
                           red, K * M, XY);
        LAUNCH_CHECK(c);
    }
    const int n = a + 1;
    if (n >= A) return PLS_HIP_OK;
    {
        int nb = 0;
        CHK(launch_xty<double>(c, XY, K, XY, K, K, M, M, xpart, &nb));
        CHK(launch_reduce(c, xpart, nb, (int)MM, nullptr, 0, xred));
        hipLaunchKernelGGL(plsk::sum_slices_kernel, dim3((unsigned)((MM + plsk::WG - 1) / plsk::WG)), blk, 0, c->stream,
                           (const double *)xred, (int)MM, G);
        LAUNCH_CHECK(c);
    }
    if (M <= plsk::MMAX) {
        hipLaunchKernelGGL(plsk::lm_eig_lds_kernel, dim3(1), dim3(plsk::UPD_THREADS), 0, c->stream, (const double *)G, M,
                           (int)c->opt_power_iters, qe);
        LAUNCH_CHECK(c);
    } else if (M <= plsk::LM_LDS_MAX &&
               plsk::raise_dynamic_lds(reinterpret_cast<const void *>(&plsk::lm_eig_lds_big_kernel), (2 * M * M + M) * 8)) {
        hipLaunchKernelGGL(plsk::lm_eig_lds_big_kernel, dim3(1), dim3(plsk::UPD_THREADS), (size_t)(2 * M * M + M) * 8, c->stream,
                           (const double *)G, M, (int)c->opt_power_iters, qe);
        LAUNCH_CHECK(c);
    } else {
        const dim3 sq((M + 15) / 16, (M + 15) / 16), sqb(16, 16);
        const double *src = G;
        double *dst = Bm;
        for (int it = 0; it < std::max(1, (int)c->opt_power_iters); ++it) {
            hipLaunchKernelGGL(plsk::lm_square_normalised_kernel, sq, sqb, 0, c->stream, src, M, dst);
            src = dst;
            dst = (dst == Bm) ? Cm : Bm;
        }
        LAUNCH_CHECK(c);
        const double *Bfin = src;
        hipLaunchKernelGGL(plsk::lm_eig_finish_kernel, dim3(1), dim3(plsk::UPD_THREADS), 0, c->stream, (const double *)G,
                           Bfin, M, qe);
        LAUNCH_CHECK(c);
    }
    hipLaunchKernelGGL(plsk::lm_w_kernel, dim3(nparts), blk, 0, c->stream, (const double *)XY, (const double *)qe, K, M, wraw, ssp);
    LAUNCH_CHECK(c);
    double *wn = W + (i64)n * K;
    hipLaunchKernelGGL(plsk::lm_normalize_kernel, dim3(nparts), blk, 0, c->stream, (const double *)wraw, (const double *)ssp,
                       nparts, K, wn, n == 0 ? R : (double *)nullptr, n == 0 ? v : (double *)nullptr);
    LAUNCH_CHECK(c);
    if (n > 0) {
        double *cs = (double *)c->cs.p;
        hipLaunchKernelGGL(plsk::rotate_dots_kernel, dim3(n), blk, 0, c->stream, P, W, K, n, cs);
        LAUNCH_CHECK(c);
        hipLaunchKernelGGL(plsk::rotate_apply_kernel, dim3(nparts), blk, 0, c->stream, W, R, cs, v, K, n, nip);
        LAUNCH_CHECK(c);
    }
    return PLS_HIP_OK;
}

constexpr int WIDE1_MIN = 4097;
constexpr int WIDEM_MIN = plsk::COOP_MAXG * plsk::COOP_WG + 1;

bool update_is_single(int K, int M, int A, int a) {
    int g = 0, e = 0;
    if (M > plsk::MMAX || (M > 8 && (i64)K * M >= 16384)) return false;
    if (M == 1 && K >= WIDE1_MIN && plsk::wide1_geometry(K, &g, &e)) return false;
    if (M >= 2 && M <= 8 && K >= WIDEM_MIN && (i64)K * M >= 16384 && A <= 4096 && plsk::wide1_geometry(K, &g, &e)) return false;
    if (plsk::coop_update_covers(K, M) && A <= 4096) return false;
    const int n = a + 1;
    return !(n < A && n > 0 && (i64)n * K >= ROTATE_SPLIT_MIN);
}

int launch_update(pls_hip_context *c, double *red, double *XY, double *W, double *P,
                  double *Q, double *R, double *v, int K, int M, int A, int a, int nip, const plsk::XchgGather *gx = nullptr) {
    const int n = a + 1;
    if (M > plsk::MMAX || (M > 8 && (i64)K * M >= 16384))
        return launch_update_large(c, (const double *)red, XY, W, P, Q, R, v, K, M, A, a, nip);
    int w1g = 0, w1e = 0;
    if (M == 1 && K >= WIDE1_MIN && plsk::wide1_geometry(K, &w1g, &w1e)) {
        CHK(ensure(c, c->wide1, (size_t)((i64)(A + 2) * w1g + A + 1) * 8));
        double *w1part = (double *)c->wide1.p, *w1q = w1part + (i64)(A + 1) * w1g, *w1tot = w1q + w1g;
        Scope s(c, PLS_HIP_FAM_SMALL, ((i64)K * 3 + (i64)K * (2 * (a + 2)) + K) * 8);
        hipLaunchKernelGGL(plsk::wide1_a_kernel, dim3(w1g), dim3(plsk::W1_WG), (size_t)plsk::W1_WG * w1e * 8, c->stream, red, XY, P, Q,
                           K, A, a, w1e, (const double *)w1q, w1part);
        LAUNCH_CHECK(c);
        if (n < A && n + 1 <= 4096) {
            hipLaunchKernelGGL(plsk::wide1_b_kernel<false>, dim3(w1g), dim3(plsk::W1_WG), (size_t)(n + 1) * 8, c->stream,
                               (const double *)XY, W, R, v, K, n, w1e, nip, (const double *)w1part, w1q, (const double *)nullptr);
            LAUNCH_CHECK(c);
        } else if (n < A) {
            hipLaunchKernelGGL(plsk::wide1_totals_kernel, dim3((n + 4) / 4), dim3(plsk::W1_WG), 0, c->stream, (const double *)w1part, n,
                               w1g, w1tot);
            hipLaunchKernelGGL(plsk::wide1_b_kernel<true>, dim3(w1g), dim3(plsk::W1_WG), 0, c->stream, (const double *)XY, W, R, v, K,
                               n, w1e, nip, (const double *)w1part, w1q, (const double *)w1tot);
            LAUNCH_CHECK(c);
        }
        return PLS_HIP_OK;
    }
    if (M >= 2 && M <= 8 && K >= WIDEM_MIN && (i64)K * M >= 16384 && A <= 4096 && plsk::wide1_geometry(K, &w1g, &w1e)) {
        CHK(ensure(c, c->wide1, (size_t)((i64)(A + plsk::WM_GSTRIDE + plsk::WM_QSTRIDE) * w1g) * 8));
        double *gp = (double *)c->wide1.p, *cp = gp + (i64)plsk::WM_GSTRIDE * w1g, *qp = cp + (i64)A * w1g;
        const dim3 g(w1g), b(plsk::W1_WG);
        Scope s(c, PLS_HIP_FAM_SMALL, ((i64)K * M * 3 + (i64)K * (2 * (a + 2)) + K) * 8);
        with_mm(M, [&](auto mm) {
            constexpr int MM = decltype(mm)::value;
            hipLaunchKernelGGL((plsk::widem_a_kernel<MM>), g, b, 0, c->stream, red, XY, P, Q, K, M, A, a, w1e, (const double *)qp, gp);
            if (n < A) {
                hipLaunchKernelGGL((plsk::widem_b_kernel<MM>), g, b, (size_t)plsk::W1_WG * w1e * 8, c->stream, (const double *)XY, W,
                                   (const double *)P, K, M, n, w1e, (int)c->opt_power_iters, (const double *)gp, cp);
                hipLaunchKernelGGL((plsk::widem_c_kernel<MM>), g, b, (size_t)(n + 1) * 8, c->stream, (const double *)XY,
                                   (const double *)W, R, v, K, M, n, w1e, nip, (const double *)cp, qp);
            }
        });
        LAUNCH_CHECK(c);
        return PLS_HIP_OK;
    }
    if (plsk::coop_update_covers(K, M) && A <= 4096) {
        const size_t need = plsk::coop_scratch_bytes(A);
        if (c->coop.bytes < need) {
            CHK(ensure(c, c->coop, need));
            HIPCHK(c, hipMemsetAsync(c->coop.p, 0, c->coop.bytes, c->stream));
        }
        unsigned *cnt = (unsigned *)c->coop.p;
        if (a < 0) HIPCHK(c, hipMemsetAsync(cnt, 0, 256, c->stream));
        double *qraw = (double *)((char *)c->coop.p + 256), *gpart = qraw + plsk::COOP_MAXG * plsk::COOP_QSTRIDE;
        double *cpart = gpart + plsk::COOP_MAXG * plsk::COOP_GSTRIDE;
        const dim3 grid((K + plsk::COOP_WG - 1) / plsk::COOP_WG), blk(plsk::COOP_WG);
        Scope s(c, PLS_HIP_FAM_SMALL, ((i64)K * M * 3 + (i64)K * (2 * (a + 2)) + K) * 8);
        with_mm(M, [&](auto mm) {
            hipLaunchKernelGGL((plsk::coop_update_kernel<decltype(mm)::value>), grid, blk, (size_t)A * sizeof(double), c->stream, red, XY, W, P,
                               Q, R, v, K, M, A, a, nip, (int)c->opt_power_iters, cnt, qraw, gpart, cpart);
        });
        LAUNCH_CHECK(c);
        return PLS_HIP_OK;
    }
    const bool split = n < A && n > 0 && (i64)n * K >= ROTATE_SPLIT_MIN;
    Scope s(c, PLS_HIP_FAM_SMALL, ((i64)K * M * 3 + (i64)K * (2 * (a + 2)) + K) * 8);
    if (gx) {
        if (split) return fail(c, PLS_HIP_ERR_DEVICE, "internal: gather prologue on a split update");
        hipLaunchKernelGGL(plsk::component_update_gather_kernel, dim3(1), dim3(plsk::UPD_THREADS),
                           (size_t)std::min(A, 4096) * sizeof(double), c->stream, *gx, red, XY, W, P, Q, R, v, K, M, A, a, nip,
                           (int)c->opt_power_iters, 0);
    } else {
        hipLaunchKernelGGL(plsk::component_update_kernel, dim3(1), dim3(plsk::UPD_THREADS),
                           (size_t)std::min(A, 4096) * sizeof(double), c->stream, (const double *)red, XY, W, P, Q, R, v, K, M, A, a, nip,
                           (int)c->opt_power_iters, (int)split);
    }
    LAUNCH_CHECK(c);
    if (split) {
        double *cs = (double *)c->cs.p;
        hipLaunchKernelGGL(plsk::rotate_dots_kernel, dim3(n), dim3(plsk::WG), 0, c->stream, P, W, K, n, cs);
        LAUNCH_CHECK(c);
        hipLaunchKernelGGL(plsk::rotate_apply_kernel, dim3((K + plsk::WG - 1) / plsk::WG), dim3(plsk::WG), 0,
                           c->stream, W, R, cs, v, K, n, nip);
        LAUNCH_CHECK(c);
    }
    return PLS_HIP_OK;
}

}
```

pls_amd/csrc/plan_fit.hpp:

```cpp
#pragma once

namespace {

template <typename T>
struct FitWork {
    double *red, *part, *sspart, *XY, *v;
    T *work;
    plsk::SliceTail tail;
    bool retiled = false;
    bool xx_local_done = false;
    int nip;
};

template <typename T>
int fit_workspace(pls_hip_context *c, const plsk::FitShape &shape, plsk::FitPlan &plan, FitWork<T> &w) {
    CHK(ensure(c, c->part, plan.part_bytes));
    CHK(ensure(c, c->sspart, plan.sspart_bytes));
    CHK(ensure(c, c->xy, (size_t)shape.K * shape.M * 8));
    CHK(ensure(c, c->v, (size_t)shape.K * 8));
    CHK(ensure(c, c->cs, (size_t)shape.A * 8));
    if (c->user_red) {
        if (c->user_red_count < (i64)(plan.red_bytes / 8)) return fail(c, PLS_HIP_ERR_INVALID, "reduce buffer too small");
        w.red = c->user_red;
    } else {
        CHK(ensure(c, c->red, plan.red_bytes));
        w.red = (double *)c->red.p;
    }
    if (plan.retile_fit && ensure(c, c->work, plan.work_bytes) != PLS_HIP_OK) {
        c->err.clear();
        plan = plsk::fit_plan(shape, plsk::FIT_NO_COPY);
    }
    if (plan.work_bytes) CHK(ensure(c, c->work, plan.work_bytes));
    w.part = (double *)c->part.p;
    w.sspart = (double *)c->sspart.p;
    w.XY = (double *)c->xy.p;
    w.v = (double *)c->v.p;
    w.work = (T *)c->work.p;
    if (c->env.tail && c->opt_fuse && shape.N > 0) {
        if (!c->tailcnt.p) CHK(ensure(c, c->tailcnt, 256));
        HIPCHK(c, hipMemsetAsync(c->tailcnt.p, 0, 256, c->stream));
        w.tail.cnt = (unsigned *)c->tailcnt.p;
        w.tail.red = w.red;
    }
    w.nip = plan.algo == plsk::FIT_NIPALS ? 1 : 0;
    return PLS_HIP_OK;
}

template <typename T>
int fit_xty(pls_hip_context *c, const FitArgs<T> &f, const plsk::FitPlan &p, FitWork<T> &w) {
    const T *X = f.X;
    const i64 N = f.N, ldx = f.ldx;
    const int K = f.K, M = f.M;
    const i64 L0 = (i64)K * M;
    const bool type2 = p.algo == plsk::FIT_GRAM || p.algo == plsk::FIT_TYPE2;
    Range r_phase("X^T Y");
    if (!p.use_pre && N > 0 && (p.retile_fit || p.nip_copy) && M <= 8) {
        int nb = 0, rc = 1;
        {
            Scope s(c, PLS_HIP_FAM_DEFLATE, 2 * (i64)N * K * sizeof(T) + (i64)N * M * sizeof(T) + L0 * 8);
            rc = pick_int<8, 16, 32>(p.fused_mode ? p.tall_cg : 32, [&](auto cg) {
                return plsk::launch_retile_xty<T, decltype(cg)::value>(c->stream, c->num_cu, X, ldx, f.Y, f.ldy, w.work, p.WR, p.WR * (i64)K, (int)p.WR, N, K,
                                                                       M, w.part, (int)p.prow, &nb);
            });
            if (rc != 0) s.on = false;
        }
        if (rc == 0) {
            LAUNCH_CHECK(c);
            CHK(launch_reduce(c, w.part, nb, (int)L0, nullptr, 0, w.red));
            w.retiled = true;
        }
    }
    if (p.wide_only && !w.retiled && N > 0 && M <= 8) return fail(c, PLS_HIP_ERR_DEVICE, "copy into row-pack tiles failed");
    if (w.retiled) {
    } else if (p.use_pre) {
        hipLaunchKernelGGL(plsk::fill_slices_kernel, dim3((unsigned)((L0 + plsk::WG - 1) / plsk::WG)), dim3(plsk::WG), 0,
                           c->stream, c->pre_xy, (int)L0, w.red);
        LAUNCH_CHECK(c);
    } else if (N > 0) {
        bool xy_from_syrk = false;
        if (type2) {
            CHK(compute_xx_local<T>(c, X, ldx, N, K, f.Y, f.ldy, M, w.red, &xy_from_syrk));
            w.xx_local_done = true;
            w.part = (double *)c->part.p;
        }
        if (!xy_from_syrk) {
            int nb = 0;
            CHK(launch_xty<T>(c, X, ldx, f.Y, f.ldy, N, K, M, w.part, &nb));
            CHK(launch_reduce(c, w.part, nb, (int)L0, nullptr, 0, w.red));
        }
    } else {
        HIPCHK(c, hipMemsetAsync(w.red, 0, (size_t)plsk::RED_SLICES * L0 * 8, c->stream));
    }
    CHK(do_allreduce(c, w.red, (i64)plsk::RED_SLICES * L0));
    CHK(launch_update(c, w.red, w.XY, f.W, f.P, f.Q, f.R, w.v, K, M, f.A, -1, w.nip));
    return PLS_HIP_OK;
}

template <typename T>
int fit_type2(pls_hip_context *c, const FitArgs<T> &f, const plsk::FitPlan &p, FitWork<T> &w) {
    const i64 N = f.N;
    const int K = f.K, M = f.M, A = f.A;
    double *red = w.red, *XY = w.XY, *v = w.v, *W = f.W, *P = f.P, *Q = f.Q, *R = f.R;
    CHK(ensure(c, c->xx, (size_t)K * K * 8));
    CHK(ensure(c, c->praw, (size_t)K * 8));
    double *XX = (double *)c->xx.p, *praw = (double *)c->praw.p;
    {
        Range r_phase("X^T X (SYRK)");
        if (p.use_pre) {
            const i64 KK = (i64)K * K;
            CHK(ensure(c, c->red2, (size_t)plsk::RED_SLICES * KK * 8));
            hipLaunchKernelGGL(plsk::fill_slices_kernel, dim3((unsigned)((KK + plsk::WG - 1) / plsk::WG)), dim3(plsk::WG), 0,
                               c->stream, c->pre_xx, (int)KK, (double *)c->red2.p);
            LAUNCH_CHECK(c);
            CHK(do_allreduce(c, (double *)c->red2.p, (i64)plsk::RED_SLICES * KK));
            hipLaunchKernelGGL(plsk::sum_slices_kernel, dim3((unsigned)((KK + plsk::WG - 1) / plsk::WG)), dim3(plsk::WG), 0,
                               c->stream, (const double *)c->red2.p, (int)KK, XX);
            LAUNCH_CHECK(c);
        } else {
            if (!w.xx_local_done) CHK(compute_xx_local<T>(c, f.X, f.ldx, N, K));
            CHK(compute_xx_finish(c, K, XX));
        }
    }
    for (int a = 0; a < A; ++a) {
        Range r_comp("component", a);
        {
            Scope s(c, PLS_HIP_FAM_SMALL, ((i64)K * K + 2 * K) * 8);
            hipLaunchKernelGGL(plsk::symv_kernel, dim3((K + 3) / 4), dim3(plsk::WG), 0, c->stream,
                               (const double *)XX, (const double *)v, K, praw);
            LAUNCH_CHECK(c);
        }
        if (update_is_single(K, M, A, a)) {
            Scope s(c, PLS_HIP_FAM_SMALL, ((i64)K * M * 3 + (i64)K * (2 * (a + 2)) + 2 * K) * 8);
            hipLaunchKernelGGL(plsk::component_update_type2_kernel, dim3(1), dim3(plsk::UPD_THREADS),
                               (size_t)std::min(A, 4096) * sizeof(double), c->stream, (const double *)praw, (const double *)v, red,
                               XY, W, P, Q, R, v, K, M, A, a, (int)c->opt_power_iters, 0);
            LAUNCH_CHECK(c);
            continue;
        }
        hipLaunchKernelGGL(plsk::type2_pack_kernel, dim3(1), dim3(plsk::UPD_THREADS), 0, c->stream,
                           (const double *)praw, (const double *)v, K, red);
        LAUNCH_CHECK(c);
        CHK(launch_update(c, red, XY, W, P, Q, R, v, K, M, A, a, 0));
    }
    if (f.B) {
        const int nblk = (int)(((i64)K * M + plsk::WG - 1) / plsk::WG);
        hipLaunchKernelGGL(plsk::coefficients_kernel, dim3(nblk), dim3(plsk::WG), 0, c->stream, R, Q, K, M, A, f.B);
        LAUNCH_CHECK(c);
    }
    if (p.algo == plsk::FIT_GRAM && N > 0) {
        Range r_t("T = X R");
        int nss = 0;
        CHK(launch_xb<T>(c, f.X, f.ldx, N, K, R, K, A, f.Tm, f.ldt, nullptr, &nss));
    }
    return replica_guard(c, W, P, Q, R, f.B, K, M, A);
}

template <typename T>
struct PassState {
    const T *Xc;
    i64 ldc, tsc;
    bool cur_tiled = false;
    int defer_b = 0;
    bool tail_used, upd_done;
    bool store_x;
    plsk::Turn turn;
};
constexpr int PASS_NOT_COVERED = -1;

template <typename T>
int pass_deferred(pls_hip_context *c, const FitArgs<T> &f, const plsk::FitPlan &p, FitWork<T> &w, PassState<T> &st, int a) {
    if (!(p.fused_mode && p.defer > 1 && a > 0)) return PASS_NOT_COVERED;
    const i64 N = f.N;
    const int K = f.K;
    int nb = 0, nss = 0, rc;
    const int np = a - st.defer_b;
    const bool store = (np == p.defer) && (a + 1 < f.A);
    plsk::PendingUpdates<T> pend{};
    for (int n = 0; n < np; ++n) {
        pend.t[n] = f.Tm + (i64)(st.defer_b + n) * f.ldt;
        pend.p[n] = f.P + (i64)(st.defer_b + n) * K;
    }
    {
        const i64 bytes = (store ? 2 : 1) * (i64)N * K * sizeof(T) + (np + 1) * (i64)N * sizeof(T) +
                          (np + 2) * (i64)K * 8;
        Scope s(c, PLS_HIP_FAM_FUSED, bytes);
        rc = plsk::launch_fused_defer<T>(c->stream, c->num_cu, st.Xc, st.ldc, st.tsc, w.work, p.ldw, p.tsw, N, K, w.v, np, pend,
                                         store, f.Tm + (i64)a * f.ldt, w.part, (int)p.prow, w.sspart, &nb, &nss);
        if (rc != 0) s.on = false;
    }
    if (rc != 0) return fail(c, PLS_HIP_ERR_DEVICE, "deferred fused pass launch failed");
    LAUNCH_CHECK(c);
    if (store) { st.Xc = w.work; st.ldc = p.ldw; st.tsc = p.tsw; st.cur_tiled = true; st.defer_b = a; }
    CHK(launch_reduce(c, w.part, nb, K, w.sspart, nss, w.red));
    return PLS_HIP_OK;
}

template <typename T>
int pass_tall(pls_hip_context *c, const FitArgs<T> &f, const plsk::FitPlan &p, FitWork<T> &w, PassState<T> &st, int a) {
    if (!(p.fused_mode && !p.retile_fit)) return PASS_NOT_COVERED;
    const i64 N = f.N;
    const int K = f.K;
    const bool nipals = p.algo == plsk::FIT_NIPALS;
    T *work = w.work;
    int nb = 0, nss = 0;
    const T *tprev = (nipals && a > 0) ? f.Tm + (i64)(a - 1) * f.ldt : nullptr;
    const double *pprev = (nipals && a > 0) ? f.P + (i64)(a - 1) * K : nullptr;
    int rc;
    {
        const i64 bytes = ((tprev && st.store_x) ? 2 : 1) * (i64)N * K * sizeof(T) +
                          (tprev ? 2 : 1) * (i64)N * sizeof(T) + (tprev ? 3 : 2) * (i64)K * 8;
        Scope s(c, PLS_HIP_FAM_FUSED, bytes);
        if (p.mid_cg && a >= 2)
            rc = plsk::launch_fused_pass<T, 64>(c->stream, c->num_cu, work, p.ldw, p.tsw, work, p.ldw, p.tsw, N, K, w.v,
                                                tprev, pprev, f.Tm + (i64)a * f.ldt, w.part, (int)p.prow, w.sspart,
                                                &nb, &nss, (int)c->opt_fused_grid, 0, true, &w.tail, &st.tail_used, &st.upd_done, st.store_x, st.turn);
        else
            rc = pick_int<8, 16, 32>(p.tall_cg, [&](auto cg) {
                return plsk::launch_fused_pass<T, decltype(cg)::value>(
                    c->stream, c->num_cu, st.Xc, st.ldc, st.tsc, (tprev && st.store_x) ? work : nullptr, p.ldw, p.tsw, N, K, w.v, tprev, pprev,
                    f.Tm + (i64)a * f.ldt, w.part, (int)p.prow, w.sspart, &nb, &nss, (int)c->opt_fused_grid,
                    (p.mid_cg && tprev && st.store_x) ? (int)p.WR : 0, st.Xc == work, &w.tail, &st.tail_used, &st.upd_done, st.store_x, st.turn);
            });
        if (rc != 0) s.on = false;
    }
    if (rc != 0) return fail(c, PLS_HIP_ERR_DEVICE, "fused pass launch failed");
    LAUNCH_CHECK(c);
    if (tprev && st.store_x) { st.Xc = work; st.ldc = p.ldw; st.tsc = p.tsw; st.cur_tiled = p.tiled_work; }
    if (!st.tail_used) CHK(launch_reduce(c, w.part, nb, K, w.sspart, nss, w.red));
    return PLS_HIP_OK;
}

template <typename T>
int pass_short_tile(pls_hip_context *c, const FitArgs<T> &f, const plsk::FitPlan &p, FitWork<T> &w, PassState<T> &st, int a) {
    const bool nipals = p.algo == plsk::FIT_NIPALS;
    if (!(p.wide_cg && (nipals ? (a >= 2 || w.retiled || p.wide_only) : true))) return PASS_NOT_COVERED;
    const i64 N = f.N;
    const int K = f.K;
    T *work = w.work;
    int nb = 0, nss = 0, rc;
    const T *tprev = (nipals && a > 0) ? f.Tm + (i64)(a - 1) * f.ldt : nullptr;
    const double *pprev = (nipals && a > 0) ? f.P + (i64)(a - 1) * K : nullptr;
    if ((!nipals || p.wide_only) && a == 0 && !w.retiled) {
        Scope s(c, PLS_HIP_FAM_DEFLATE, 2 * (i64)N * K * sizeof(T));
        if (plsk::launch_retile<T>(c->stream, c->num_cu, f.X, f.ldx, work, p.ldw, p.tsw, (int)p.WR, N, K) != 0) {
            s.on = false;
            return fail(c, PLS_HIP_ERR_DEVICE, "retile launch failed");
        }
        LAUNCH_CHECK(c);
    }
    {
        const i64 bytes = ((tprev && st.store_x) ? 2 : 1) * (i64)N * K * sizeof(T) + (tprev ? 2 : 1) * (i64)N * sizeof(T) + 3 * (i64)K * 8;
        Scope s(c, PLS_HIP_FAM_FUSED, bytes);
        rc = pick_int<8, 16, 32, 64, 128, 256, 512>(p.wide_cg, [&](auto cg) {
            return plsk::launch_fused_pass<T, decltype(cg)::value>(c->stream, c->num_cu, work, p.ldw, p.tsw, work, p.ldw, p.tsw, N, K, w.v, tprev, pprev,
                                                                   f.Tm + (i64)a * f.ldt, w.part, (int)p.prow, w.sspart, &nb, &nss, (int)c->opt_fused_grid, 0,
                                                                   true, &w.tail, &st.tail_used, &st.upd_done, st.store_x, st.turn);
        });
        if (rc != 0) s.on = false;
    }
    if (rc != 0) return fail(c, PLS_HIP_ERR_DEVICE, "short-tile fused pass launch failed");
    LAUNCH_CHECK(c);
    if (!st.tail_used) CHK(launch_reduce(c, w.part, nb, K, w.sspart, nss, w.red));
    return PLS_HIP_OK;
}

template <typename T>
int pass_unfused(pls_hip_context *c, const FitArgs<T> &f, const plsk::FitPlan &p, FitWork<T> &w, PassState<T> &st, int a) {
    const i64 N = f.N;
    const int K = f.K;
    T *work = w.work;
    int nss = 0, nb = 0;
    bool have_t = false;
    if (p.algo == plsk::FIT_NIPALS && a > 0) {
        const T *tprev = f.Tm + (i64)(a - 1) * f.ldt;
        const double *pprev = f.P + (i64)(a - 1) * K;
        if (p.semi_fit) {
            const i64 bytes = 2 * (i64)N * K * sizeof(T) + 2 * (i64)N * sizeof(T) + 2 * (i64)K * 8;
            Scope s(c, PLS_HIP_FAM_DEFLATE, bytes);
            const int rc = plsk::launch_deflate_score<T>(c->stream, c->num_cu, st.Xc, st.ldc, st.tsc, work, p.ldw, p.tsw,
                                                         (int)(p.tiled_work ? p.WR : p.TR), N, K, tprev, pprev, w.v,
                                                         f.Tm + (i64)a * f.ldt, w.sspart, (int)p.ssmax, &nss, st.Xc == work);
            if (rc != 0) {
                s.on = false;
                return fail(c, PLS_HIP_ERR_DEVICE, "deflate+score launch failed");
            }
            LAUNCH_CHECK(c);
            have_t = true;
        }
        if (!have_t) CHK(launch_deflate<T>(c, st.Xc, st.ldc, work, p.ldw, N, K, tprev, pprev));
        st.Xc = work;
        st.ldc = p.ldw;
        st.tsc = p.tsw;
        st.cur_tiled = p.tiled_work;
    }
    if (!have_t)
        CHK(launch_xb<T>(c, st.Xc, st.ldc, N, K, w.v, K, 1, f.Tm + (i64)a * f.ldt, f.ldt, w.sspart, &nss));
    if (st.cur_tiled) {
        Scope s(c, PLS_HIP_FAM_XTY, (i64)N * K * sizeof(T) + (i64)N * sizeof(T) + (i64)K * 8);
        const T *ta = f.Tm + (i64)a * f.ldt;
        const int cg = (p.wide_cg == 64 || p.wide_cg == 128 || p.wide_cg == 256) ? p.wide_cg : 32;
        const int xrc = pick_int<32, 64, 128, 256>(cg, [&](auto g) {
            return plsk::launch_xty_tiled<T, decltype(g)::value>(c->stream, c->num_cu, st.Xc, st.ldc, st.tsc, N, K, ta, w.part, (int)p.prow, &nb);
        });
        if (xrc != 0) {
            s.on = false;
            return fail(c, PLS_HIP_ERR_DEVICE, "tiled loading launch failed");
        }
        LAUNCH_CHECK(c);
    } else {
        CHK(launch_xty<T>(c, st.Xc, st.ldc, f.Tm + (i64)a * f.ldt, f.ldt, N, K, 1, w.part, &nb));
    }
    CHK(launch_reduce(c, w.part, nb, K, w.sspart, nss, w.red));
    return PLS_HIP_OK;
}

inline plsk::XchgGather exchange_gather(const pls_hip_context *c, unsigned long long seq) {
    const int par = (int)(seq & 1);
    plsk::XchgGather gx;
    gx.inbox = c->xep.inbox[c->xep.rank] + (i64)par * c->xep.n * plsk::XCHG_CAP;
    gx.flags = c->xep.flags[c->xep.rank] + par * c->xep.n;
    gx.n = c->xep.n; gx.cap = plsk::XCHG_CAP; gx.seq = seq;
    gx.status = c->xep.status; gx.host_status = c->xep.host_status; gx.limit = *c->xep.limit;
    return gx;
}

template <typename T>
int fit_passes(pls_hip_context *c, const FitArgs<T> &f, const plsk::FitPlan &p, FitWork<T> &w) {
    const i64 N = f.N;
    const int K = f.K, M = f.M, A = f.A;
    plsk::SliceTail &tail = w.tail;
    PassState<T> st;
    st.Xc = f.X;
    st.ldc = f.ldx;
    st.tsc = p.TR;
    using Route = int (*)(pls_hip_context *, const FitArgs<T> &, const plsk::FitPlan &, FitWork<T> &, PassState<T> &, int);
    const Route routes[] = {pass_deferred<T>, pass_tall<T>, pass_short_tile<T>, pass_unfused<T>};
    for (int a = 0; a < A; ++a) {
        Range r_comp("component", a);
        st.tail_used = st.upd_done = false;
        const bool want_push = tail.cnt && p.xep_ok && update_is_single(K, M, A, a);
        const bool defl_pass = w.nip && a > 0;
        st.store_x = (a + 1 < A);
        st.turn = plsk::Turn{c->env.turnaround, c->env.turnaround && a % 2 == 0, c->env.turn_edge_bytes};
        const bool want_upd = tail.cnt && (c->env.tail_update == 2 || (c->env.tail_update == 1 && !defl_pass)) && M == 1 &&
                              K <= plsk::UPD1_KMAX && update_is_single(K, M, A, a) && (!c->reducer || want_push);
        tail.npush = 0;
        tail.upd = plsk::TailUpdate();
        tail.gx = plsk::XchgGather();
        if (want_push) {
            const unsigned long long seq = *c->xep.seq + 1;
            const int par = (int)(seq & 1);
            tail.npush = c->xep.n;
            tail.seq = seq;
            for (int j = 0; j < c->xep.n; ++j) {
                tail.peers.slot[j] = c->xep.inbox[j] + ((i64)par * c->xep.n + c->xep.rank) * plsk::XCHG_CAP;
                tail.peers.flag[j] = c->xep.flags[j] + par * c->xep.n + c->xep.rank;
            }
            if (want_upd) tail.gx = exchange_gather(c, seq);
        }
        if (want_upd) {
            tail.upd.XY = w.XY; tail.upd.W = f.W; tail.upd.P = f.P; tail.upd.Q = f.Q; tail.upd.R = f.R; tail.upd.vnext = w.v;
            tail.upd.A = A; tail.upd.a = a; tail.upd.nipals = w.nip;
        }
        if (N > 0) {
            int rc = PASS_NOT_COVERED;
            for (Route route : routes)
                if ((rc = route(c, f, p, w, st, a)) != PASS_NOT_COVERED) break;
            CHK(rc);
        } else {
            HIPCHK(c, hipMemsetAsync(w.red, 0, (size_t)plsk::RED_SLICES * (K + 1) * 8, c->stream));
        }
        if (st.upd_done) {
            if (want_push) ++*c->xep.seq;
        } else if (st.tail_used && want_push) {
            const plsk::XchgGather gx = exchange_gather(c, ++*c->xep.seq);
            CHK(launch_update(c, w.red, w.XY, f.W, f.P, f.Q, f.R, w.v, K, M, A, a, w.nip, &gx));
        } else {
            CHK(do_allreduce(c, w.red, (i64)plsk::RED_SLICES * (K + 1)));
            CHK(launch_update(c, w.red, w.XY, f.W, f.P, f.Q, f.R, w.v, K, M, A, a, w.nip));
        }
    }
    if (f.B) {
        Scope s(c, PLS_HIP_FAM_SMALL, ((i64)K * A + (i64)M * A + (i64)K * M) * 8);
        const int nblk = (int)(((i64)K * M + plsk::WG - 1) / plsk::WG);
        hipLaunchKernelGGL(plsk::coefficients_kernel, dim3(nblk), dim3(plsk::WG), 0, c->stream, f.R, f.Q,
                           K, M, A, f.B);
        LAUNCH_CHECK(c);
    }
    return replica_guard(c, f.W, f.P, f.Q, f.R, f.B, K, M, A);
}

template <typename T>
int fit_device(pls_hip_context *c, const T *X, i64 ldx, const T *Y, i64 ldy, i64 N, int K, int M,
               int A, int method, double *W, double *P, double *Q, double *R, T *Tm, i64 ldt, double *B) {
    if (method == PLS_HIP_KERNEL_TYPE1 && c->opt_algo == PLS_HIP_ALGO_DUAL)
        return fit_dual<T>(c, X, ldx, Y, ldy, N, K, M, A, W, P, Q, R, Tm, ldt, B);
    const FitArgs<T> f{X, ldx, Y, ldy, N, K, M, A, method, W, P, Q, R, Tm, ldt, B};
    bool taken = false;
    CHK(fit_single_launch<T>(c, f, &taken));
    if (taken) return PLS_HIP_OK;
    const plsk::FitShape shape{N, K, M, A, (int)sizeof(T), ldx, ldy, ldt, (uintptr_t)X, (uintptr_t)Y, (uintptr_t)Tm, c->num_cu, method,
                               c->opt_algo, c->opt_fuse, c->opt_work_layout, c->opt_defer, c->opt_fused_grid,
                               c->reducer != nullptr, c->pre_xx && c->pre_xy, c->xep.on};
    plsk::FitPlan plan = plsk::fit_plan(shape, 0);
    FitWork<T> w;
    CHK(fit_workspace<T>(c, shape, plan, w));
    Range r_fit("pls_hip_fit");
    CHK(fit_xty<T>(c, f, plan, w));
    if (plan.algo == plsk::FIT_GRAM || plan.algo == plsk::FIT_TYPE2) return fit_type2<T>(c, f, plan, w);
    return fit_passes<T>(c, f, plan, w);
}

}
```

pls_amd/csrc/pls_hip.hip:

```cpp
#include <dlfcn.h>
#include <unistd.h>
#include <hip/hip_runtime.h>

#include <algorithm>
#include <atomic>
#include <cstdio>
#include <cstring>
#include <memory>
#include <new>
#include <string>
#include <type_traits>
#include <vector>

#include "../../include/pls_hip.h"
#include "fused_kernels.hpp"
#include "defer_kernels.hpp"
#include "small_kernels.hpp"
#include "coop_update.hpp"
#include "wide1_update.hpp"
#include "largem_kernels.hpp"
#include "tiny_kernels.hpp"
#include "resident_kernels.hpp"
#include "resident_gram.hpp"
#include "stream_kernels.hpp"
#include "xb_mfma4.hpp"
#include "xb_mfma4w.hpp"
#include "syrk_kernels.hpp"
#include "cv_kernels.hpp"
#include "validation_kernels.hpp"
#include "xdiag_kernels.hpp"
#include "batch_kernels.hpp"
#include "dual_kernels.hpp"
#include "dual_cv_kernels.hpp"
#include "dual_batch_kernels.hpp"
#include "dual_cvbatch_kernels.hpp"
#include "resample_kernels.hpp"
#include "synth_kernels.hpp"
#include "missing_kernels.hpp"
#include "host_pipeline.hpp"
#include "exchange_kernels.hpp"

using plsk::i64;

#include "ctx.hpp"
#include "xb_route.hpp"
#include "launch_products.hpp"
#include "plan_common.hpp"
#include "launch_update.hpp"
#include "plan_dual.hpp"
#include "plan_fit_single.hpp"
#include "plan_fit.hpp"
#include "host_entry.hpp"
#include "plan_validation.hpp"
#include "plan_xdiag.hpp"

extern "C" {

int pls_hip_abi_version(void) { return PLS_HIP_ABI_VERSION; }

#ifdef PLS_HIP_TESTING
__attribute__((visibility("default"))) int pls_hip_test_set_pass_stamps(void *buf) {
    unsigned long long *p = (unsigned long long *)buf;
    return hipMemcpyToSymbol(HIP_SYMBOL(plsk::g_pass_stamps), &p, sizeof(p)) == hipSuccess ? 0 : 1;
}
__attribute__((visibility("default"))) int pls_hip_test_last_turn(int *out) {
    if (!out) return 1;
    out[0] = plsk::g_test_turn.rev; out[1] = plsk::g_test_turn.edge; out[2] = plsk::g_test_turn.ntiles; out[3] = plsk::g_test_turn.grid;
    return 0;
}
__attribute__((visibility("default"))) long long pls_hip_test_poison_workspace(pls_hip_handle h, int byte, int also_new) {
    if (!h || hipSetDevice(h->device) != hipSuccess || hipStreamSynchronize(h->stream) != hipSuccess) return -1;
    long long filled = 0;
    bool ok = true;
    for_each_workspace(h, [&](DevBuf &b, size_t keep) {
        if (!b.p || keep >= b.bytes) return;
        ok = ok && hipMemsetAsync((char *)b.p + keep, byte & 0xFF, b.bytes - keep, h->stream) == hipSuccess;
        filled += (long long)(b.bytes - keep);
    });
    h->poison_new = also_new ? (byte & 0xFF) : -1;
    return ok && hipStreamSynchronize(h->stream) == hipSuccess ? filled : -1;
}
#endif

int pls_hip_create(pls_hip_handle *out, int device, void *stream) {
    if (!out) return PLS_HIP_ERR_INVALID;
    *out = nullptr;
    int ndev = 0;
    if (hipGetDeviceCount(&ndev) != hipSuccess || ndev <= 0 || device < 0 || device >= ndev) {
        (void)hipGetLastError();
        return PLS_HIP_ERR_DEVICE;
    }
    hipDeviceProp_t prop;
    if (hipGetDeviceProperties(&prop, device) != hipSuccess) return PLS_HIP_ERR_DEVICE;
    if (std::strncmp(prop.gcnArchName, "gfx950", 6) != 0) return PLS_HIP_ERR_DEVICE;
    pls_hip_context *c = new (std::nothrow) pls_hip_context();
    if (!c) return PLS_HIP_ERR_ALLOC;
    {
        auto off = [](const char *name) { const char *e = getenv(name); return e && atoi(e) == 0; };
        auto on = [](const char *name) { const char *e = getenv(name); return e && atoi(e) != 0; };
        c->env.tiny = !off("PLS_HIP_TINY");
        c->env.cv_refit = on("PLS_HIP_CV_REFIT");
        c->env.batch_refit = on("PLS_HIP_BATCH_REFIT");
        if (const char *e = getenv("PLS_HIP_BATCH_ROUND")) c->env.batch_round = atoll(e);
        if (const char *e = getenv("PLS_HIP_DUALCV_ROUND")) c->env.dualcv_round = atoll(e);
        if (const char *e = getenv("PLS_HIP_DUALBATCH_ROUND")) c->env.dualbatch_round = atoll(e);
        if (const char *e = getenv("PLS_HIP_RESAMPLE_ROUND")) c->env.resample_round = atoll(e);
        c->env.resample_refit = on("PLS_HIP_RESAMPLE_REFIT");
        c->env.dualbatch_sweeps = on("PLS_HIP_DUALBATCH_SWEEPS");
        c->env.cvbatch_refit = on("PLS_HIP_CVBATCH_REFIT");
        if (const char *e = getenv("PLS_HIP_DUALCVB_ROUND")) c->env.dualcvb_round = atoll(e);
        c->env.tail = !off("PLS_HIP_TAIL");
        {
            const char *e = getenv("PLS_HIP_TAIL");
            c->env.tail_update = e ? (atoi(e) >= 2 ? 2 : 0) : 1;
        }
        c->env.replica_guard = !off("PLS_HIP_REPLICA_GUARD");
        c->env.resident = !off("PLS_HIP_RESIDENT");
        c->env.turnaround = !off("PLS_HIP_TURNAROUND");
#ifdef PLS_HIP_TESTING
        if (const char *e = getenv("PLS_HIP_TEST_TURN_EDGE_BYTES")) c->env.turn_edge_bytes = atoll(e);
#endif
        if (const char *e = getenv("PLS_HIP_XB4")) c->env.xb4 = atoi(e);
        if (const char *e = getenv("PLS_HIP_RESIDENT_GRAM")) c->env.resident_gram = atoi(e);
    }
    c->device = device;
    c->num_cu = prop.multiProcessorCount > 0 ? prop.multiProcessorCount : 256;
    if (hipSetDevice(device) != hipSuccess) { delete c; return PLS_HIP_ERR_DEVICE; }
    c->stream = (hipStream_t)stream;
    *out = c;
    return PLS_HIP_OK;
}

int pls_hip_destroy(pls_hip_handle h) {
    if (!h) return PLS_HIP_OK;
    (void)hipSetDevice(h->device);
    (void)hipStreamSynchronize(h->stream);
    for_each_workspace(h, [](DevBuf &b, size_t) {
        if (b.p) (void)hipFree(b.p);
    });
    for (void *q : h->graveyard) (void)hipFree(q);
    if (h->xchg) xchg_release(h);
    if (h->diverged) (void)hipHostFree(h->diverged);
    if (h->mconv_host) (void)hipHostFree(h->mconv_host);
    for (hipEvent_t e : h->ev_pool) (void)hipEventDestroy(e);
    if (h->graph_exec) (void)hipGraphExecDestroy(h->graph_exec);
    h->stager.release();
    if (h->copy_stream) (void)hipStreamDestroy(h->copy_stream);
    delete h;
    return PLS_HIP_OK;
}

int pls_hip_set_stream(pls_hip_handle h, void *stream) {
    CHK(check_handle(h));
    CHK(set_device(h));
    HIPCHK(h, hipStreamSynchronize(h->stream));
    h->stream = (hipStream_t)stream;
    return PLS_HIP_OK;
}

int pls_hip_set_option(pls_hip_handle h, int option, int64_t value) {
    CHK(check_handle(h));
    switch (option) {
        case PLS_HIP_OPT_ALGO:
            if (value != PLS_HIP_ALGO_KERNEL && value != PLS_HIP_ALGO_NIPALS && value != PLS_HIP_ALGO_GRAM &&
                value != PLS_HIP_ALGO_AUTO && value != PLS_HIP_ALGO_DUAL)
                return fail(h, PLS_HIP_ERR_INVALID, "unknown algo");
            h->opt_algo = value;
            return PLS_HIP_OK;
        case PLS_HIP_OPT_FUSE: h->opt_fuse = value ? 1 : 0; return PLS_HIP_OK;
        case PLS_HIP_OPT_PROFILE: h->opt_profile = value < 0 ? 0 : (value > 2 ? 2 : value); return PLS_HIP_OK;
        case PLS_HIP_OPT_POWER_ITERS:
            if (value < 1 || value > 4096) return fail(h, PLS_HIP_ERR_INVALID, "power iters out of range");
            h->opt_power_iters = value;
            return PLS_HIP_OK;
        case PLS_HIP_OPT_FUSED_GRID:
            if (value < 0 || value > (1 << 20)) return fail(h, PLS_HIP_ERR_INVALID, "fused grid out of range");
            h->opt_fused_grid = value;
            return PLS_HIP_OK;
        case PLS_HIP_OPT_WORK_LAYOUT: h->opt_work_layout = value ? 1 : 0; return PLS_HIP_OK;
        case PLS_HIP_OPT_DEFER:
            if (value < 1 || value > plsk::DEFER_MAX) return fail(h, PLS_HIP_ERR_INVALID, "defer out of range");
            h->opt_defer = value;
            return PLS_HIP_OK;
        case PLS_HIP_OPT_GRAPH: h->opt_graph = value ? 1 : 0; return PLS_HIP_OK;
        case PLS_HIP_OPT_VALIDATION_LDS_ROWS:
            if (value < 0 || value > val_lds_rows_device(h)) return fail(h, PLS_HIP_ERR_INVALID, "validation LDS rows out of range");
            h->opt_val_lds_rows = value;
            return PLS_HIP_OK;
        case PLS_HIP_OPT_MISSING_ITERS:
            if (value < 1 || value > (1 << 20)) return fail(h, PLS_HIP_ERR_INVALID, "missing iters out of range");
            h->opt_missing_iters = value;
            return PLS_HIP_OK;
        default: return fail(h, PLS_HIP_ERR_INVALID, "unknown option");
    }
}

int pls_hip_get_option(pls_hip_handle h, int option, int64_t *value) {
    CHK(check_handle(h));
    if (!value) return PLS_HIP_ERR_INVALID;
    switch (option) {
        case PLS_HIP_OPT_ALGO: *value = h->opt_algo; return PLS_HIP_OK;
        case PLS_HIP_OPT_FUSE: *value = h->opt_fuse; return PLS_HIP_OK;
        case PLS_HIP_OPT_PROFILE: *value = h->opt_profile; return PLS_HIP_OK;
        case PLS_HIP_OPT_POWER_ITERS: *value = h->opt_power_iters; return PLS_HIP_OK;
        case PLS_HIP_OPT_FUSED_GRID: *value = h->opt_fused_grid; return PLS_HIP_OK;
        case PLS_HIP_OPT_GRAPH: *value = h->opt_graph; return PLS_HIP_OK;
        case PLS_HIP_OPT_WORK_LAYOUT: *value = h->opt_work_layout; return PLS_HIP_OK;
        case PLS_HIP_OPT_DEFER: *value = h->opt_defer; return PLS_HIP_OK;
        case PLS_HIP_OPT_VALIDATION_LDS_ROWS: *value = h->opt_val_lds_rows >= 0 ? h->opt_val_lds_rows : val_lds_rows_device(h); return PLS_HIP_OK;
        case PLS_HIP_OPT_MISSING_ITERS: *value = h->opt_missing_iters; return PLS_HIP_OK;
        default: return fail(h, PLS_HIP_ERR_INVALID, "unknown option");
    }
}

int pls_hip_set_reducer(pls_hip_handle h, pls_hip_allreduce_fn fn, void *user, int rank, int nranks) {
    CHK(check_handle(h));
    if (nranks < 1 || rank < 0 || rank >= nranks || (nranks > 1 && !fn))
        return fail(h, PLS_HIP_ERR_INVALID, "bad reducer arguments");
    h->reducer = fn;
    h->reducer_user = user;
    h->rank = rank;
    h->nranks = nranks;
    return PLS_HIP_OK;
}

int pls_hip_get_reducer(pls_hip_handle h, int *installed, int *rank, int *nranks) {
    CHK(check_handle(h));
    if (installed) *installed = h->reducer ? 1 : 0;
    if (rank) *rank = h->rank;
    if (nranks) *nranks = h->nranks;
    return PLS_HIP_OK;
}

int pls_hip_set_reduce_buffer(pls_hip_handle h, void *buf, int64_t count) {
    CHK(check_handle(h));
    if ((buf && count <= 0) || (!buf && count != 0)) return fail(h, PLS_HIP_ERR_INVALID, "bad reduce buffer");
    h->user_red = (double *)buf;
    h->user_red_count = count;
    return PLS_HIP_OK;
}

int pls_hip_synchronize(pls_hip_handle h) {
    CHK(check_handle(h));
    CHK(set_device(h));
    HIPCHK(h, hipStreamSynchronize(h->stream));
    return check_diverged(h);
}

const char *pls_hip_last_error(pls_hip_handle h) { return h ? h->err.c_str() : "null handle"; }

int pls_hip_get_timing(pls_hip_handle h, pls_hip_timing *out) {
    CHK(check_handle(h));
    if (!out) return PLS_HIP_ERR_INVALID;
    std::memset(out, 0, sizeof(*out));
    CHK(set_device(h));
    HIPCHK(h, hipStreamSynchronize(h->stream));
    for (const Launch &l : h->fits) {
        float ms = 0.f;
        HIPCHK(h, hipEventElapsedTime(&ms, l.e0, l.e1));
        out->fit_ms += ms;
        out->fits += 1;
    }
    for (const Launch &l : h->launches) {
        float ms = 0.f;
        HIPCHK(h, hipEventElapsedTime(&ms, l.e0, l.e1));
        out->fam_ms[l.fam] += ms;
        out->fam_launches[l.fam] += 1;
        out->fam_bytes[l.fam] += l.bytes;
    }
    h->launches.clear();
    h->fits.clear();
    h->ev_used = 0;
    return PLS_HIP_OK;
}

int pls_hip_fit(pls_hip_handle h, const void *X, int64_t ldx, const void *Y, int64_t ldy, int64_t N,
                int64_t K, int64_t M, int64_t A, int method, int dtype, int mem, double *W, double *P,
                double *Q, double *R, void *T, int64_t ldt, double *B) {
    CHK(check_handle(h));
    if (dtype != PLS_HIP_F64 && dtype != PLS_HIP_F32) return fail(h, PLS_HIP_ERR_INVALID, "bad dtype");
    if (mem != PLS_HIP_MEM_HOST && mem != PLS_HIP_MEM_DEVICE) return fail(h, PLS_HIP_ERR_INVALID, "bad mem kind");
    if (method != PLS_HIP_KERNEL_TYPE1 && method != PLS_HIP_KERNEL_TYPE2)
        return fail(h, PLS_HIP_ERR_INVALID, "bad method");
    const bool sharded = h->nranks > 1;
    if (N < 0 || (N == 0 && !sharded) || K < 1 || M < 1 || A < 1 || A > K)
        return fail(h, PLS_HIP_ERR_INVALID, "bad shape: need N>=1, K>=1, M>=1, 1<=A<=K");
    if (K > (1 << 30) || M > plsk::LM_MAX)
        return fail(h, PLS_HIP_ERR_UNSUPPORTED, "more than 1024 responses (or K > 2^30) not supported on the device");
    if (N > 0 && (!X || !Y || (!T && method == PLS_HIP_KERNEL_TYPE1))) return fail(h, PLS_HIP_ERR_INVALID, "null X/Y/T");
    if ((method == PLS_HIP_KERNEL_TYPE2 || h->opt_algo == PLS_HIP_ALGO_GRAM) && K > 32768)
        return fail(h, PLS_HIP_ERR_UNSUPPORTED, "KERNEL_TYPE2 keeps a K x K matrix and 8 reduction slices of it (77 GB at K = 32768): K <= 32768");
    if (!W || !P || !Q || !R) return fail(h, PLS_HIP_ERR_INVALID, "null W/P/Q/R");
    if (ldx < std::max<i64>(N, 1) || ldy < std::max<i64>(N, 1) || (T && ldt < std::max<i64>(N, 1)))
        return fail(h, PLS_HIP_ERR_INVALID, "leading dimension smaller than N");
    const bool dual = method == PLS_HIP_KERNEL_TYPE1 && h->opt_algo == PLS_HIP_ALGO_DUAL;
    if (dual)
        if (const char *why = dual_refusal(h, N, M)) return fail(h, PLS_HIP_ERR_UNSUPPORTED, why);
    CHK(set_device(h));
    const size_t es = esize(dtype);
    const int Ki = (int)K, Mi = (int)M, Ai = (int)A;

    const void *dX = X, *dY = Y;
    void *dT = T;
    double *dW = W, *dP = P, *dQ = Q, *dR = R, *dB = B;
    i64 dldx = ldx, dldy = ldy, dldt = ldt;
    if (mem == PLS_HIP_MEM_HOST) {
        const i64 ldn = std::max<i64>(N, 1) + (std::max<i64>(N, 1) & 1);
        CHK(ensure(h, h->hX, (size_t)ldn * K * es));
        CHK(ensure(h, h->hY, (size_t)ldn * M * es));
        CHK(ensure(h, h->hT, (size_t)ldn * A * es));
        CHK(ensure(h, h->hW, (size_t)K * A * 8));
        CHK(ensure(h, h->hP, (size_t)K * A * 8));
        CHK(ensure(h, h->hR, (size_t)K * A * 8));
        CHK(ensure(h, h->hQ, (size_t)M * A * 8));
        CHK(ensure(h, h->hB, (size_t)K * M * 8));
        CHK(h2d(h, h->hY.p, ldn, Y, ldy, N, M, es));
        bool pre = false;
        const bool wants_gram = h->opt_algo == PLS_HIP_ALGO_AUTO || h->opt_algo == PLS_HIP_ALGO_GRAM || method == PLS_HIP_KERNEL_TYPE2;
        const bool single_launch = method == PLS_HIP_KERNEL_TYPE1 && h->opt_algo == PLS_HIP_ALGO_AUTO && h->opt_fuse &&
                                   (plsk::tiny_fit_covers(N, Ki, Mi, Ai, ldn, es) || plsk::tiny_fit_m_covers(N, Ki, Mi, Ai, ldn, es) ||
                                    plsk::micro_fit_covers(N, Ki, Mi, Ai, ldn, es));
        if (wants_gram && !single_launch && !h->reducer && N > 0 && K <= 4096 && ensure(h, h->gxx, (size_t)K * K * 8) == PLS_HIP_OK &&
            ensure(h, h->gxy, (size_t)K * M * 8) == PLS_HIP_OK) {
            CHK(by_dtype(dtype, [&](auto t) {
                using Tx = decltype(t);
                return upload_accumulate<Tx>(h, (Tx *)h->hX.p, ldn, (const Tx *)X, ldx, N, Ki, (const Tx *)h->hY.p, ldn, Mi, (double *)h->gxx.p,
                                            (double *)h->gxy.p, &pre);
            }));
        } else {
            h->err.clear();
            CHK(h2d(h, h->hX.p, ldn, X, ldx, N, K, es));
        }
        if (pre) {
            h->pre_xx = (const double *)h->gxx.p;
            h->pre_xy = (const double *)h->gxy.p;
        }
        dX = h->hX.p; dY = h->hY.p; dT = h->hT.p;
        dW = (double *)h->hW.p; dP = (double *)h->hP.p; dQ = (double *)h->hQ.p; dR = (double *)h->hR.p;
        dB = B ? (double *)h->hB.p : nullptr;
        dldx = dldy = dldt = ldn;
    }
    const bool graphable = h->opt_graph && mem == PLS_HIP_MEM_DEVICE && !h->reducer && h->opt_profile == 0 && !h->user_red &&
                           h->stream != nullptr && !dual;
    std::vector<uint64_t> key;
    if (graphable) {
        key = {(uint64_t)(uintptr_t)X, (uint64_t)ldx, (uint64_t)(uintptr_t)Y, (uint64_t)ldy, (uint64_t)N, (uint64_t)K, (uint64_t)M,
               (uint64_t)A, (uint64_t)method, (uint64_t)dtype, (uint64_t)(uintptr_t)W, (uint64_t)(uintptr_t)P, (uint64_t)(uintptr_t)Q,
               (uint64_t)(uintptr_t)R, (uint64_t)(uintptr_t)T, (uint64_t)ldt, (uint64_t)(uintptr_t)B, (uint64_t)h->opt_algo,
               (uint64_t)h->opt_fuse, (uint64_t)h->opt_power_iters, (uint64_t)h->opt_fused_grid, (uint64_t)h->opt_work_layout,
               (uint64_t)h->opt_defer, (uint64_t)(uintptr_t)h->stream, (uint64_t)(uintptr_t)h->pre_xx, (uint64_t)(uintptr_t)h->pre_xy};
        if (h->graph_exec && key == h->graph_key) {
            HIPCHK(h, hipGraphLaunch(h->graph_exec, h->stream));
            return PLS_HIP_OK;
        }
    }
    const bool capture = graphable && key == h->graph_seen;
    if (capture) {
        if (h->graph_exec) { (void)hipGraphExecDestroy(h->graph_exec); h->graph_exec = nullptr; h->graph_key.clear(); }
        HIPCHK(h, hipStreamBeginCapture(h->stream, hipStreamCaptureModeThreadLocal));
    }
    begin_fit_timing(h);
    const int rc = by_dtype(dtype, [&](auto t) {
        using Tx = decltype(t);
        return fit_device<Tx>(h, (const Tx *)dX, dldx, (const Tx *)dY, dldy, N, Ki, Mi, Ai, method, dW, dP, dQ, dR, (Tx *)dT, dldt, dB);
    });
    end_fit_timing(h);
    if (capture) {
        hipGraph_t graph = nullptr;
        const hipError_t ce = hipStreamEndCapture(h->stream, &graph);
        if (rc == PLS_HIP_OK && ce == hipSuccess && graph && hipGraphInstantiate(&h->graph_exec, graph, nullptr, nullptr, 0) == hipSuccess) {
            h->graph_key = key;
            (void)hipGraphDestroy(graph);
            HIPCHK(h, hipGraphLaunch(h->graph_exec, h->stream));
        } else {
            if (graph) (void)hipGraphDestroy(graph);
            h->graph_exec = nullptr;
            h->graph_seen.clear();
            (void)hipGetLastError();
            if (rc != PLS_HIP_OK) return rc;
            return fail(h, PLS_HIP_ERR_DEVICE, "stream capture of the fit failed");
        }
    } else if (graphable) {
        h->graph_seen = key;
    }
    if (mem == PLS_HIP_MEM_HOST) h->pre_xx = h->pre_xy = nullptr;
    if (rc != PLS_HIP_OK) return rc;
    if (mem == PLS_HIP_MEM_HOST) {
        CHK(d2h(h, W, K, dW, K, K, A, 8));
        CHK(d2h(h, P, K, dP, K, K, A, 8));
        CHK(d2h(h, R, K, dR, K, K, A, 8));
        CHK(d2h(h, Q, M, dQ, M, M, A, 8));
        if (B) CHK(d2h(h, B, K, dB, K, K, M, 8));
        if (method == PLS_HIP_KERNEL_TYPE1) CHK(d2h(h, T, ldt, dT, dldt, N, A, es));
        HIPCHK(h, hipStreamSynchronize(h->stream));
        CHK(check_diverged(h));
    }
    return PLS_HIP_OK;
}

int pls_hip_coefficients(pls_hip_handle h, const double *R, const double *Q, int64_t K, int64_t M,
                         int64_t A, int64_t cc, int mem, double *B) {
    CHK(check_handle(h));
    if (!R || !Q || !B || K < 1 || M < 1 || A < 1 || cc < 0 || cc > A || K > (1 << 30))
        return fail(h, PLS_HIP_ERR_INVALID, "bad coefficients arguments");
    CHK(set_device(h));
    const double *dR = R, *dQ = Q;
    double *dB = B;
    if (mem == PLS_HIP_MEM_HOST) {
        CHK(ensure(h, h->hR, (size_t)K * A * 8));
        CHK(ensure(h, h->hQ, (size_t)M * A * 8));
        CHK(ensure(h, h->hB, (size_t)K * M * 8));
        CHK(h2d(h, h->hR.p, K, R, K, K, A, 8));
        CHK(h2d(h, h->hQ.p, M, Q, M, M, A, 8));
        dR = (double *)h->hR.p; dQ = (double *)h->hQ.p; dB = (double *)h->hB.p;
    } else if (mem != PLS_HIP_MEM_DEVICE) {
        return fail(h, PLS_HIP_ERR_INVALID, "bad mem kind");
    }
    const int nblk = (int)((K * M + plsk::WG - 1) / plsk::WG);
    hipLaunchKernelGGL(plsk::coefficients_kernel, dim3(nblk), dim3(plsk::WG), 0, h->stream, dR, dQ,
                       (int)K, (int)M, (int)cc, dB);
    LAUNCH_CHECK(h);
// ... 569 lines not shown
```

pls_amd/csrc/small_kernels.hpp:

```cpp
#pragma once
#include "common.hpp"
#include "exchange_kernels.hpp"
#include "fused_kernels.hpp"
#include "update_m1.hpp"
#include "stream_kernels.hpp"

namespace plsk {

__device__ __forceinline__ double red_sum(const double *red, int LP, int j) {
    double s = 0.0;
#pragma unroll
    for (int i = 0; i < RED_SLICES; ++i) s += red[(i64)i * LP + j];
    return s;
}
__device__ __forceinline__ double red_sum_n(const double *red, int nsl, int LP, int j) {
    if (nsl == RED_SLICES) return red_sum(red, LP, j);
    double s = 0.0;
    for (int i = 0; i < nsl; ++i) s += red[(i64)i * LP + j];
    return s;
}

struct UpdShared {
    double sred[1024 / 64];
    double qs[32];
// ... 18 lines not shown
            double s = 0.0;
            for (int c = 0; c < M; ++c) s = fma(Bm[a + c * M], Bm[c + b * M], s);
            Cm[a + b * M] = s;
        }
        __syncthreads();
        double t2 = 0.0;
        for (int c = 0; c < M; ++c) t2 += Cm[c + c * M];
        int same = 1;
        if (act) {
            const double nb = Cm[a + b * M] / t2, ob = Bm[a + b * M];
            same = fabs(nb - ob) <= 4.0e-16 * fabs(nb) + 1.0e-18;
            Bm[a + b * M] = nb;
        }
        if (__syncthreads_and(same)) break;
    }
    int best = 0;
    double bd = Bm[0];
    for (int c = 1; c < M; ++c)
        if (Bm[c + c * M] > bd) { bd = Bm[c + c * M]; best = c; }
    if (tid < M) qv[tid] = Bm[tid + best * M];
    __syncthreads();
    for (int pol = 0; pol < 2; ++pol) {
        double s = 0.0;
        if (tid < M)
            for (int c = 0; c < M; ++c) s = fma(G[tid + c * M], qv[c], s);
        __syncthreads();
        if (tid < M) qv[tid] = s;
        __syncthreads();
        double n2 = 0.0;
        for (int c = 0; c < M; ++c) n2 = fma(qv[c], qv[c], n2);
        const double inv = 1.0 / sqrt(n2);
        __syncthreads();
        if (tid < M) qv[tid] = s * inv;
        __syncthreads();
    }
    int big = 0;
    for (int c = 1; c < M; ++c)
        if (fabs(qv[c]) > fabs(qv[big])) big = c;
    const double sgn = (qv[big] < 0.0) ? -1.0 : 1.0;
    __syncthreads();
    if (tid < M) qv[tid] *= sgn;
    __syncthreads();
}


__device__ __forceinline__ void wave_lds_sync() {
    __builtin_amdgcn_fence(__ATOMIC_SEQ_CST, "wavefront");
    __builtin_amdgcn_wave_barrier();
}

template <int MM>
__device__ __forceinline__ void dominant_eigvec_wave(const double *G, double *Bm, double *Cm, double *qv, int iters) {
    static_assert(MM * MM <= WAVE, "one matrix entry per lane");
    const int lane = threadIdx.x & 63;
    const int a = lane % MM, b = lane / MM;
    const bool act = lane < MM * MM;
    double tr = 0.0;
#pragma unroll
    for (int c = 0; c < MM; ++c) tr += G[c + c * MM];
    double cur = act ? G[a + b * MM] / tr : 0.0;
    if (act) Bm[a + b * MM] = cur;
    wave_lds_sync();
    for (int it = 0; it < iters; ++it) {
        double s = 0.0;
        if (act) {
#pragma unroll
            for (int c = 0; c < MM; ++c) s = fma(Bm[a + c * MM], Bm[c + b * MM], s);
            Cm[a + b * MM] = s;
        }
        wave_lds_sync();
        double t2 = 0.0;
#pragma unroll
        for (int c = 0; c < MM; ++c) t2 += Cm[c + c * MM];
        const double nb = s / t2;
        const bool moved = act && !(fabs(nb - cur) <= 4.0e-16 * fabs(nb) + 1.0e-18);
        cur = nb;
        if (act) Bm[a + b * MM] = nb;
        wave_lds_sync();
        if (__builtin_amdgcn_ballot_w64(moved) == 0) break;
    }
    int best = 0;
    double bd = Bm[0];
#pragma unroll
    for (int c = 1; c < MM; ++c)
        if (Bm[c + c * MM] > bd) { bd = Bm[c + c * MM]; best = c; }
    if (lane < MM) qv[lane] = Bm[lane + best * MM];
    wave_lds_sync();
    for (int pol = 0; pol < 2; ++pol) {
        double s = 0.0;
        if (lane < MM) {
#pragma unroll
            for (int c = 0; c < MM; ++c) s = fma(G[lane + c * MM], qv[c], s);
        }
        wave_lds_sync();
        if (lane < MM) qv[lane] = s;
        wave_lds_sync();
        double n2 = 0.0;
#pragma unroll
        for (int c = 0; c < MM; ++c) n2 = fma(qv[c], qv[c], n2);
        const double inv = 1.0 / sqrt(n2);
        wave_lds_sync();
        if (lane < MM) qv[lane] = s * inv;
        wave_lds_sync();
    }
    int big = 0;
#pragma unroll
    for (int c = 1; c < MM; ++c)
        if (fabs(qv[c]) > fabs(qv[big])) big = c;
    const double sgn = (qv[big] < 0.0) ? -1.0 : 1.0;
    wave_lds_sync();
    if (lane < MM) qv[lane] *= sgn;
    wave_lds_sync();
}

template <int N, int LEVEL>
__device__ __forceinline__ int wave_multi_sum_levels(double *g, int lane, bool &valid) {
    if constexpr (LEVEL == 6) {
        return 0;
    } else {
        constexpr int H = (N + 1) / 2;
        constexpr int BIT = LEVEL == 0 ? 32 : LEVEL == 1 ? 16 : LEVEL == 2 ? 8 : LEVEL == 3 ? 4 : LEVEL == 4 ? 2 : 1;
        const bool up = (lane & BIT) != 0;
#pragma unroll
        for (int i = 0; i < H; ++i) {
            double lo = g[i], hi = (N > 1) ? ((i + H < N) ? g[i + H] : 0.0) : g[i];
            if constexpr (LEVEL <= 1) {
                permlane_swap_f64<LEVEL == 1>(lo, hi);
                g[i] = lo + hi;
            } else {
                const double keep = (N > 1 && up) ? hi : lo, send = (N > 1 && up) ? lo : hi;
                constexpr int CTRL = LEVEL == 2 ? 0x140 : LEVEL == 3 ? 0x141 : LEVEL == 4 ? 0x4E : 0xB1;
                g[i] = keep + dpp_mov_f64<CTRL>(send);
            }
        }
        const int idx = wave_multi_sum_levels<H, LEVEL + 1>(g, lane, valid) + ((N > 1 && up) ? H : 0);
        valid = valid && (idx < N);
        return idx;
    }
}

template <int N, int MASK>
__device__ __forceinline__ int wave_multi_sum(double *g, int lane, bool &valid) {
    static_assert(MASK == 32, "whole-wave sums");
    return wave_multi_sum_levels<N, 0>(g, lane, valid);
}

template <int MM>
__device__ __forceinline__ void gram_add(const double (&x)[MM], double (&g)[MM * (MM + 1) / 2]) {
#pragma unroll
    for (int i = 0; i < MM; ++i)
#pragma unroll
        for (int j = i; j < MM; ++j) {
            const int idx = i * MM - (i * (i - 1)) / 2 + (j - i);
            g[idx] = fma(x[i], x[j], g[idx]);
        }
}

template <int MM>
__device__ __forceinline__ void narrow_update(const double *__restrict__ red, int nsl, double *__restrict__ XY,
                                     double *__restrict__ P, double *__restrict__ Q,
                                     const double *__restrict__ R, double *__restrict__ W, int K, int M, int A,
                                     int a, int power_iters, UpdShared &sh) {
    constexpr int NP = MM * (MM + 1) / 2;
    static_assert(UPD_WAVES * NP <= 32 * 32, "wave partials live in UpdShared::Bs");
    const int tid = threadIdx.x, lane = tid & 63, wv = tid >> 6;
    const bool last = (a + 1 >= A);
    i64 co[MM];
#pragma unroll
    for (int m = 0; m < MM; ++m) co[m] = (i64)(m < M ? m : M - 1) * K;
    double g[NP];
#pragma unroll
    for (int i = 0; i < NP; ++i) g[i] = 0.0;

    if (a >= 0) {
        const double tt = red_sum_n(red, nsl, K + 1, K);
        const double *ra = R + (i64)a * K;
        double qa[MM];
#pragma unroll
        for (int m = 0; m < MM; ++m) qa[m] = 0.0;
        double *pa = P + (i64)a * K;
#pragma unroll 2
        for (int k = tid; k < K; k += UPD_THREADS) {
            pa[k] = red_sum_n(red, nsl, K + 1, k) / tt;
            const double rk = ra[k];
            double x[MM];
#pragma unroll
            for (int m = 0; m < MM; ++m) x[m] = XY[k + co[m]];
#pragma unroll
            for (int m = 0; m < MM; ++m) qa[m] = fma(rk, (m < M) ? x[m] : 0.0, qa[m]);
        }
        {
            bool valid = true;
            const int idx = wave_multi_sum<MM, 32>(qa, lane, valid);
            if (valid) sh.Cs[wv * MM + idx] = qa[0];
        }
        __syncthreads();
        if (tid < MM) {
            double s = 0.0;
#pragma unroll
            for (int w = 0; w < UPD_WAVES; ++w) s += sh.Cs[w * MM + tid];
            s /= tt;
            sh.qs[tid] = s;
            if (tid < M) Q[tid + (i64)a * M] = s;
        }
        __syncthreads();
        double qv[MM];
#pragma unroll
        for (int m = 0; m < MM; ++m) qv[m] = sh.qs[m];
        for (int k = tid; k < K; k += UPD_THREADS) {
            const double p = pa[k];
            double x[MM];
#pragma unroll
            for (int m = 0; m < MM; ++m) x[m] = XY[k + co[m]];
#pragma unroll
            for (int m = 0; m < MM; ++m) x[m] = (m < M) ? x[m] - (p * qv[m]) * tt : 0.0;
#pragma unroll
            for (int m = 0; m < MM; ++m)
                if (m < M) XY[k + (i64)m * K] = x[m];
            if (!last) gram_add<MM>(x, g);
        }
    } else {
        for (int k = tid; k < K; k += UPD_THREADS) {
            double x[MM];
#pragma unroll
            for (int m = 0; m < MM; ++m) {
                x[m] = 0.0;
                if (m < M) {
                    if (red) {
                        x[m] = red_sum_n(red, nsl, K * M, k + m * K);
                        XY[k + (i64)m * K] = x[m];
                    } else {
                        x[m] = XY[k + (i64)m * K];
                    }
                }
            }
            gram_add<MM>(x, g);
        }
    }
    if (last) return;

    double *part = sh.Bs;
    {
        bool valid = true;
        const int idx = wave_multi_sum<NP, 32>(g, lane, valid);
        if (valid) part[wv * NP + idx] = g[0];
    }
    __syncthreads();
    if (tid < NP) {
        int i = 0, rem = tid;
        while (rem >= MM - i) { rem -= MM - i; ++i; }
        const int j = i + rem;
        double s = 0.0;
#pragma unroll
        for (int w = 0; w < UPD_WAVES; ++w) s += part[w * NP + tid];
        sh.Gs[i + j * MM] = s;
        sh.Gs[j + i * MM] = s;
    }
    __syncthreads();
    if (wv == 0) dominant_eigvec_wave<MM>(sh.Gs, sh.Bs, sh.Cs, sh.qs, power_iters);
    __syncthreads();
    double qv[MM];
#pragma unroll
    for (int m = 0; m < MM; ++m) qv[m] = sh.qs[m];
    double *wn = W + (i64)(a + 1) * K;
    double ss = 0.0;
    double wl[4];
#pragma unroll
    for (int i = 0; i < 4; ++i) {
        const int k = tid + i * UPD_THREADS, kc = k < K ? k : K - 1;
        double x[MM];
#pragma unroll
        for (int m = 0; m < MM; ++m) x[m] = XY[kc + co[m]];
        double s = 0.0;
#pragma unroll
        for (int m = 0; m < MM; ++m) s = fma((m < M) ? x[m] : 0.0, qv[m], s);
        wl[i] = (k < K) ? s : 0.0;
        ss = fma(wl[i], wl[i], ss);
    }
    for (int k = tid + 4 * UPD_THREADS; k < K; k += UPD_THREADS) {
        double x[MM];
#pragma unroll
        for (int m = 0; m < MM; ++m) x[m] = XY[k + co[m]];
        double s = 0.0;
#pragma unroll
        for (int m = 0; m < MM; ++m) s = fma((m < M) ? x[m] : 0.0, qv[m], s);
        wn[k] = s;
        ss = fma(s, s, ss);
    }
    ss = block_sum<UPD_WAVES>(ss, sh.sred);
    const double nrm = sqrt(ss);
#pragma unroll
    for (int i = 0; i < 4; ++i) {
        const int k = tid + i * UPD_THREADS;
        if (k < K) wn[k] = wl[i] / nrm;
    }
    for (int k = tid + 4 * UPD_THREADS; k < K; k += UPD_THREADS) wn[k] = wn[k] / nrm;
}

__device__ __forceinline__ void component_update_body(const double *__restrict__ red, int nsl,
                                             double *__restrict__ XY, double *__restrict__ W,
                                             double *__restrict__ P, double *__restrict__ Q,
                                             double *__restrict__ R, double *__restrict__ vnext, int K,
                                             int M, int A, int a, int nipals, int power_iters,
                                             int split_rotate, double *cs, UpdShared &sh) {
    double *sred = sh.sred, *qs = sh.qs, *Gs = sh.Gs, *Bs = sh.Bs, *Cs = sh.Cs;
    const int tid = threadIdx.x, lane = tid & 63, wv = tid >> 6;

    const bool fast = (M == 1 && K <= 4 * UPD_THREADS && a >= 0);
    const bool narrow = (M >= 2 && M <= 8);
    const double *Rq = R;
    if (narrow) {
        if (M <= 2)
            narrow_update<2>(red, nsl, XY, P, Q, Rq, W, K, M, A, a, power_iters, sh);
        else if (M <= 4)
            narrow_update<4>(red, nsl, XY, P, Q, Rq, W, K, M, A, a, power_iters, sh);
        else
            narrow_update<8>(red, nsl, XY, P, Q, Rq, W, K, M, A, a, power_iters, sh);
    } else if (fast) {
        if (K <= UPD1_VTHREADS)
            update_m1<UPD_THREADS, 1>([&](int j) { return red_sum_n(red, nsl, K + 1, j); }, XY, W, P, Q, R, vnext, K, A, a, nipals,
                                      split_rotate, cs, sred, (double *)nullptr);
        else
            update_m1<UPD_THREADS, 4>([&](int j) { return red_sum_n(red, nsl, K + 1, j); }, XY, W, P, Q, R, vnext, K, A, a, nipals,
                                      split_rotate, cs, sred, (double *)nullptr);
        return;
    } else if (a < 0) {
        if (red)
            for (int j = tid; j < K * M; j += UPD_THREADS) XY[j] = red_sum_n(red, nsl, K * M, j);
    } else {
        const double tt = red_sum_n(red, nsl, K + 1, K);
        const double *ra = Rq + (i64)a * K;
        for (int m = wv; m < M; m += UPD_WAVES) {
            const double *xm = XY + (i64)m * K;
            double s0 = 0.0, s1 = 0.0, s2 = 0.0, s3 = 0.0;
            int k = lane;
            for (; k + 3 * WAVE < K; k += 4 * WAVE) {
                s0 = fma(ra[k], xm[k], s0);
                s1 = fma(ra[k + WAVE], xm[k + WAVE], s1);
                s2 = fma(ra[k + 2 * WAVE], xm[k + 2 * WAVE], s2);
                s3 = fma(ra[k + 3 * WAVE], xm[k + 3 * WAVE], s3);
            }
            for (; k < K; k += WAVE) s0 = fma(ra[k], xm[k], s0);
            double s = wave_sum((s0 + s1) + (s2 + s3));
            if (lane == 0) {
                qs[m] = s / tt;
                Q[m + (i64)a * M] = s / tt;
            }
        }
        __syncthreads();
        for (int k = tid; k < K; k += UPD_THREADS) {
            const double p = red_sum_n(red, nsl, K + 1, k) / tt;
            P[k + (i64)a * K] = p;
            for (int m = 0; m < M; ++m) XY[k + (i64)m * K] -= (p * qs[m]) * tt;
        }
    }
    const int n = a + 1;
    if (n >= A) return;
    __syncthreads();

    double *wn = W + (i64)n * K;
    if (narrow) {
    } else if (M == 1) {
        double ss = 0.0;
        for (int k = tid; k < K; k += UPD_THREADS) ss = fma(XY[k], XY[k], ss);
        ss = block_sum<UPD_WAVES>(ss, sred);
        const double nrm = sqrt(ss);
        for (int k = tid; k < K; k += UPD_THREADS) wn[k] = XY[k] / nrm;
    } else {
        const int npairs = M * (M + 1) / 2;
        for (int pr = wv; pr < npairs; pr += UPD_WAVES) {
            int i = 0, rem = pr;
            while (rem >= M - i) { rem -= M - i; ++i; }
            const int j = i + rem;
            const double *xi = XY + (i64)i * K, *xj = XY + (i64)j * K;
            double s0 = 0.0, s1 = 0.0, s2 = 0.0, s3 = 0.0;
            int k = lane;
            for (; k + 3 * WAVE < K; k += 4 * WAVE) {
                s0 = fma(xi[k], xj[k], s0);
                s1 = fma(xi[k + WAVE], xj[k + WAVE], s1);
                s2 = fma(xi[k + 2 * WAVE], xj[k + 2 * WAVE], s2);
                s3 = fma(xi[k + 3 * WAVE], xj[k + 3 * WAVE], s3);
            }
            for (; k < K; k += WAVE) s0 = fma(xi[k], xj[k], s0);
            const double s = wave_sum((s0 + s1) + (s2 + s3));
            if (lane == 0) { Gs[i + j * M] = s; Gs[j + i * M] = s; }
        }
        __syncthreads();
        dominant_eigvec_lds(Gs, Bs, Cs, qs, M, power_iters);
        double ss = 0.0;
        for (int k = tid; k < K; k += UPD_THREADS) {
            double s = 0.0;
            for (int m = 0; m < M; ++m) s = fma(XY[k + (i64)m * K], qs[m], s);
            wn[k] = s;
            ss = fma(s, s, ss);
        }
        ss = block_sum<UPD_WAVES>(ss, sred);
        const double nrm = sqrt(ss);
        for (int k = tid; k < K; k += UPD_THREADS) wn[k] = wn[k] / nrm;
    }
    if (split_rotate) return;
    __syncthreads();
    for (int j = wv; j < n; j += UPD_WAVES) {
        const double *pj = P + (i64)j * K;
        double s0 = 0.0, s1 = 0.0, s2 = 0.0, s3 = 0.0;
        int k = lane;
        for (; k + 3 * WAVE < K; k += 4 * WAVE) {
            const double a0 = pj[k], a1 = pj[k + WAVE], a2 = pj[k + 2 * WAVE], a3 = pj[k + 3 * WAVE];
            s0 = fma(a0, wn[k], s0);
            s1 = fma(a1, wn[k + WAVE], s1);
            s2 = fma(a2, wn[k + 2 * WAVE], s2);
            s3 = fma(a3, wn[k + 3 * WAVE], s3);
        }
        for (; k < K; k += WAVE) s0 = fma(pj[k], wn[k], s0);
        const double s = wave_sum((s0 + s1) + (s2 + s3));
        if (lane == 0) cs[j] = s;
    }
    __syncthreads();
    double *rn = R + (i64)n * K;
    for (int k = tid; k < K; k += UPD_THREADS) {
        const double w = wn[k];
        double r = w;
        int j = 0;
        for (; j + 4 <= n; j += 4) {
            const double r0 = R[k + (i64)j * K], r1 = R[k + (i64)(j + 1) * K];
            const double r2 = R[k + (i64)(j + 2) * K], r3 = R[k + (i64)(j + 3) * K];
            r -= cs[j] * r0;
            r -= cs[j + 1] * r1;
            r -= cs[j + 2] * r2;
            r -= cs[j + 3] * r3;
        }
        for (; j < n; ++j) r -= cs[j] * R[k + (i64)j * K];
        rn[k] = r;
        vnext[k] = nipals ? w : r;
    }
}

__device__ __noinline__ void component_update_call(const double *red, int nsl, double *XY, double *W, double *P,
                                                   double *Q, double *R, double *vnext, int K, int M, int A,
                                                   int a, int nipals, int power_iters, int split_rotate,
                                                   double *cs, UpdShared &sh) {
    component_update_body(red, nsl, XY, W, P, Q, R, vnext, K, M, A, a, nipals, power_iters, split_rotate, cs, sh);
}

__global__ __launch_bounds__(UPD_THREADS) void component_update_kernel(
    const double *__restrict__ red, double *__restrict__ XY, double *__restrict__ W,
    double *__restrict__ P, double *__restrict__ Q, double *__restrict__ R,
    double *__restrict__ vnext, int K, int M, int A, int a, int nipals, int power_iters,
    int split_rotate) {
    extern __shared__ double cs[];
    __shared__ UpdShared sh;
    component_update_body(red, RED_SLICES, XY, W, P, Q, R, vnext, K, M, A, a, nipals, power_iters, split_rotate,
                          cs, sh);
}

constexpr int AUX_SYS = 17;
__global__ __launch_bounds__(UPD_THREADS) void component_update_gather_kernel(
    const XchgGather gx, double *red, double *__restrict__ XY, double *__restrict__ W, double *__restrict__ P,
    double *__restrict__ Q, double *__restrict__ R, double *__restrict__ vnext, int K, int M, int A, int a, int nipals,
    int power_iters, int split_rotate) {
    extern __shared__ double cs[];
    __shared__ UpdShared sh;
    __shared__ int ok;
    const int tid = threadIdx.x;
    if (tid == 0) ok = (*gx.status == 0);
    __syncthreads();
    if (tid < gx.n && ok) {
        const long long t0 = wall_clock64();
        while (__hip_atomic_load(gx.flags + tid, __ATOMIC_RELAXED, __HIP_MEMORY_SCOPE_SYSTEM) < gx.seq) {
            if (wall_clock64() - t0 > gx.limit) {
                ok = 0;
                break;
            }
            __builtin_amdgcn_s_sleep(4);
        }
        __builtin_amdgcn_fence(__ATOMIC_ACQUIRE, "");
        asm volatile("s_waitcnt vmcnt(0)" ::: "memory");
    }
    __syncthreads();
    if (!ok && tid == 0) {
        *gx.status = 1;
        __hip_atomic_store(gx.host_status, 1, __ATOMIC_RELAXED, __HIP_MEMORY_SCOPE_SYSTEM);
    }
    {
        const int L = K + 1;
        typedef unsigned int u32x2 __attribute__((ext_vector_type(2)));
        for (int j = tid; j < L; j += UPD_THREADS) {
            double x[XCHG_MAX];
#pragma unroll
            for (int m = 0; m < XCHG_MAX; ++m) {
                const __amdgpu_buffer_rsrc_t rs = __builtin_amdgcn_make_buffer_rsrc(
                    const_cast<double *>(gx.inbox + (i64)(m < gx.n ? m : 0) * gx.cap), (short)0, L * 8, BUF_WORD3);
                const u32x2 raw = __builtin_amdgcn_raw_buffer_load_b64(rs, (uint32_t)j * 8u, 0, AUX_SYS);
                __builtin_memcpy(&x[m], &raw, 8);
            }
            double sum = x[0];
#pragma unroll
            for (int m = 1; m < XCHG_MAX; ++m)
                if (m < gx.n) sum += x[m];
            red[j] = ok ? sum : __builtin_nan("");
        }
    }
    __syncthreads();
    component_update_body(red, 1, XY, W, P, Q, R, vnext, K, M, A, a, nipals, power_iters, split_rotate, cs, sh);
}

__global__ __launch_bounds__(UPD_THREADS) void component_update_type2_kernel(
    const double *__restrict__ praw, const double *r, double *red, double *__restrict__ XY, double *__restrict__ W,
    double *__restrict__ P, double *__restrict__ Q, double *__restrict__ R, double *vnext, int K, int M, int A, int a,
    int power_iters, int split_rotate) {
    extern __shared__ double cs[];
    __shared__ UpdShared sh;
    double s = 0.0;
    for (int k = threadIdx.x; k < K; k += UPD_THREADS) {
        const double p = praw[k];
        s = fma(r[k], p, s);
        red[k] = p;
    }
    s = block_sum<UPD_WAVES>(s, sh.sred);
    if (threadIdx.x == 0) red[K] = s;
    __syncthreads();
    component_update_body(red, 1, XY, W, P, Q, R, vnext, K, M, A, a, 0, power_iters, split_rotate, cs, sh);
}

__global__ __launch_bounds__(WG) void rotate_dots_kernel(const double *__restrict__ P,
                                                         const double *__restrict__ W, int K, int n,
                                                         double *__restrict__ cs) {
    __shared__ double sm[WG / WAVE];
    const int j = blockIdx.x;
    const double *pj = P + (i64)j * K, *wn = W + (i64)n * K;
    double s = 0.0;
    for (int k = threadIdx.x; k < K; k += WG) s = fma(pj[k], wn[k], s);
    s = block_sum<WG / WAVE>(s, sm);
    if (threadIdx.x == 0) cs[j] = s;
}

__global__ __launch_bounds__(WG) void rotate_apply_kernel(const double *__restrict__ W,
                                                          double *__restrict__ R,
                                                          const double *__restrict__ cs,
                                                          double *__restrict__ vnext, int K, int n,
                                                          int nipals) {
    const int k = blockIdx.x * WG + threadIdx.x;
    if (k >= K) return;
    const double w = W[k + (i64)n * K];
    double r = w;
    int j = 0;
    for (; j + 4 <= n; j += 4) {
        const double r0 = R[k + (i64)j * K], r1 = R[k + (i64)(j + 1) * K];
        const double r2 = R[k + (i64)(j + 2) * K], r3 = R[k + (i64)(j + 3) * K];
        r -= cs[j] * r0;
        r -= cs[j + 1] * r1;
        r -= cs[j + 2] * r2;
        r -= cs[j + 3] * r3;
    }
    for (; j < n; ++j) r -= cs[j] * R[k + (i64)j * K];
    R[k + (i64)n * K] = r;
    vnext[k] = nipals ? w : r;
}

__global__ __launch_bounds__(WG) void symv_kernel(const double *__restrict__ XX, const double *__restrict__ r,
                                                  int K, double *__restrict__ praw) {
    const int k = blockIdx.x * (WG / WAVE) + (threadIdx.x >> 6), lane = threadIdx.x & 63;
    if (k >= K) return;
    const double *col = XX + (i64)k * K;
    double s0 = 0.0, s1 = 0.0;
    int j = lane;
    for (; j + WAVE < K; j += 2 * WAVE) {
        s0 = fma(col[j], r[j], s0);
        s1 = fma(col[j + WAVE], r[j + WAVE], s1);
    }
    if (j < K) s0 = fma(col[j], r[j], s0);
    const double s = wave_sum(s0 + s1);
    if (lane == 0) praw[k] = s;
}

__global__ __launch_bounds__(UPD_THREADS) void type2_pack_kernel(const double *__restrict__ praw,
                                                                const double *__restrict__ r, int K,
                                                                double *__restrict__ red) {
    __shared__ double sm[UPD_WAVES];
    double s = 0.0;
    for (int k = threadIdx.x; k < K; k += UPD_THREADS) {
        const double p = praw[k];
        s = fma(r[k], p, s);
        red[k] = p;
        for (int i = 1; i < RED_SLICES; ++i) red[(i64)i * (K + 1) + k] = 0.0;
    }
    s = block_sum<UPD_WAVES>(s, sm);
    if (threadIdx.x == 0) {
        red[K] = s;
        for (int i = 1; i < RED_SLICES; ++i) red[(i64)i * (K + 1) + K] = 0.0;
    }
}

__global__ __launch_bounds__(WG) void colstat_finish_kernel(const double *__restrict__ red, int K,
                                                            double n, int mode, double *__restrict__ out) {
    const int k = blockIdx.x * WG + threadIdx.x;
    if (k >= K) return;
    const double s = red_sum(red, K, k);
    out[k] = (mode == 0) ? s / n : sqrt((n < 2.0 ? 0.0 : s) / (n - 1.0));
}

__global__ __launch_bounds__(WG) void sum_slices_kernel(const double *__restrict__ red, int L,
                                                        double *__restrict__ out) {
    const int j = blockIdx.x * WG + threadIdx.x;
    if (j < L) out[j] = red_sum(red, L, j);
}

__global__ __launch_bounds__(WG) void accumulate_slices_kernel(const double *__restrict__ red, int L,
                                                               double *__restrict__ out) {
    const int j = blockIdx.x * WG + threadIdx.x;
    if (j < L) out[j] += red_sum(red, L, j);
}

__global__ __launch_bounds__(WG) void fill_slices_kernel(const double *__restrict__ src, int L, double *__restrict__ red) {
    const int j = blockIdx.x * WG + threadIdx.x;
    if (j >= L) return;
    red[j] = src[j];
#pragma unroll
    for (int i = 1; i < RED_SLICES; ++i) red[(i64)i * L + j] = 0.0;
}

__global__ __launch_bounds__(WG) void coefficients_kernel(const double *__restrict__ R,
                                                          const double *__restrict__ Q, int K,
                                                          int M, int c, double *__restrict__ B) {
    const i64 idx = (i64)blockIdx.x * WG + threadIdx.x;
    if (idx >= (i64)K * M) return;
    const int k = (int)(idx % K), m = (int)(idx / K);
    double s = 0.0;
    for (int j = 0; j < c; ++j) s = fma(R[k + (i64)j * K], Q[m + (i64)j * M], s);
    B[idx] = s;
}

__device__ __forceinline__ unsigned long long guard_mix(unsigned long long z) {
    z = (z ^ (z >> 30)) * 0xBF58476D1CE4E5B9ull;
    z = (z ^ (z >> 27)) * 0x94D049BB133111EBull;
    return z ^ (z >> 31);
}

__global__ __launch_bounds__(UPD_THREADS) void replica_checksum_kernel(const double *__restrict__ W, const double *__restrict__ P,
                                                                       const double *__restrict__ Rm, const double *__restrict__ Q,
                                                                       const double *__restrict__ B, i64 nKA, i64 nMA, i64 nKM,
                                                                       double *__restrict__ out) {
    __shared__ unsigned long long acc;
    if (threadIdx.x == 0) acc = 0ull;
    __syncthreads();
    unsigned long long h = 0ull;
    const double *arr[5] = {W, P, Rm, Q, B};
    const i64 len[5] = {nKA, nKA, nKA, nMA, B ? nKM : 0};
    for (int a = 0; a < 5; ++a)
        for (i64 i = threadIdx.x; i < len[a]; i += UPD_THREADS)
            h += guard_mix((unsigned long long)__double_as_longlong(arr[a][i]) + 0x9E3779B97F4A7C15ull * (unsigned long long)(i * 5 + a + 1));
    atomicAdd(&acc, h);
    __syncthreads();
    if (threadIdx.x < RED_SLICES * 8) {
        double v = 0.0;
        if (threadIdx.x < 8) {
            const double p = (double)((acc >> (16 * (threadIdx.x & 3))) & 0xFFFFull);
            v = threadIdx.x < 4 ? p : p * p;
        }
        out[threadIdx.x] = v;
    }
}

__global__ __launch_bounds__(WAVE) void replica_verify_kernel(const double *__restrict__ red, int nranks, int *host_flag) {
    if (threadIdx.x < 4) {
        const double s1 = red_sum(red, 8, threadIdx.x), s2 = red_sum(red, 8, 4 + threadIdx.x);
        if ((double)nranks * s2 != s1 * s1) __hip_atomic_store(host_flag, 1, __ATOMIC_RELAXED, __HIP_MEMORY_SCOPE_SYSTEM);
    }
}

}
```

pls_amd/csrc/update_m1.hpp:

```cpp
#pragma once
#include "common.hpp"

namespace plsk {

constexpr int UPD1_VTHREADS = 1024;
constexpr int UPD1_VWAVES = UPD1_VTHREADS / WAVE;
constexpr int UPD1_KMAX = 4 * UPD1_VTHREADS;

template <int NT>
__device__ __forceinline__ double vblock_sum(const double (&x)[UPD1_VTHREADS / NT], double *sm) {
    constexpr int VT = UPD1_VTHREADS / NT, NW = NT / WAVE;
    double xs[VT];
#pragma unroll
    for (int u = 0; u < VT; ++u) xs[u] = wave_sum(x[u]);
    const int w = threadIdx.x >> 6;
    __syncthreads();
    if ((threadIdx.x & 63) == 0) {
#pragma unroll
        for (int u = 0; u < VT; ++u) sm[w + u * NW] = xs[u];
    }
    __syncthreads();
    double s = 0.0;
#pragma unroll
    for (int i = 0; i < UPD1_VWAVES; ++i) s += sm[i];
    return s;
}

template <int NT, int KI, typename SumF>
__device__ __forceinline__ void update_m1(SumF S, double *__restrict__ XY, double *__restrict__ W, double *__restrict__ P,
                                          double *__restrict__ Q, double *__restrict__ R, double *__restrict__ vnext, int K, int A,
                                          int a, int nipals, int split_rotate, double *cs, double *sm, double *wl) {
    constexpr int VT = UPD1_VTHREADS / NT, NW = NT / WAVE;
    const int tid = threadIdx.x, lane = tid & 63, wv = tid >> 6;
    const double tt = S(K);
    const double *ra = R + (i64)a * K;
    double xv[VT][KI], pv[VT][KI], part[VT];
#pragma unroll
    for (int u = 0; u < VT; ++u) {
        part[u] = 0.0;
#pragma unroll
        for (int i = 0; i < KI; ++i) {
            const int k = tid + u * NT + i * UPD1_VTHREADS;
            xv[u][i] = (k < K) ? XY[k] : 0.0;
            pv[u][i] = (k < K) ? S(k) / tt : 0.0;
            part[u] = fma((k < K) ? ra[k] : 0.0, xv[u][i], part[u]);
        }
    }
    const double q = vblock_sum<NT>(part, sm) / tt;
    if (tid == 0) Q[(i64)a] = q;
    double ssn[VT];
#pragma unroll
    for (int u = 0; u < VT; ++u) {
        ssn[u] = 0.0;
#pragma unroll
        for (int i = 0; i < KI; ++i) {
            const int k = tid + u * NT + i * UPD1_VTHREADS;
            if (k < K) {
                P[k + (i64)a * K] = pv[u][i];
                xv[u][i] -= (pv[u][i] * q) * tt;
                XY[k] = xv[u][i];
                ssn[u] = fma(xv[u][i], xv[u][i], ssn[u]);
            }
        }
    }
    const int n = a + 1;
    if (n >= A) return;
    const double nrm = sqrt(vblock_sum<NT>(ssn, sm));
    double *wn = W + (i64)n * K;
#pragma unroll
    for (int u = 0; u < VT; ++u)
#pragma unroll
        for (int i = 0; i < KI; ++i) {
            const int k = tid + u * NT + i * UPD1_VTHREADS;
            if (k < K) {
                const double w = xv[u][i] / nrm;
                wn[k] = w;
                if (wl) wl[k] = w;
            }
        }
    if (split_rotate) return;
    __syncthreads();
    const double *ws = wl ? wl : wn;
    for (int j = wv; j < n; j += NW) {
        const double *pj = P + (i64)j * K;
        double s0 = 0.0, s1 = 0.0, s2 = 0.0, s3 = 0.0;
        int k = lane;
        for (; k + 3 * WAVE < K; k += 4 * WAVE) {
            const double a0 = pj[k], a1 = pj[k + WAVE], a2 = pj[k + 2 * WAVE], a3 = pj[k + 3 * WAVE];
            s0 = fma(a0, ws[k], s0);
            s1 = fma(a1, ws[k + WAVE], s1);
            s2 = fma(a2, ws[k + 2 * WAVE], s2);
            s3 = fma(a3, ws[k + 3 * WAVE], s3);
        }
        for (; k < K; k += WAVE) s0 = fma(pj[k], ws[k], s0);
        const double s = wave_sum((s0 + s1) + (s2 + s3));
        if (lane == 0) cs[j] = s;
    }
    __syncthreads();
    double *rn = R + (i64)n * K;
    for (int k = tid; k < K; k += NT) {
        const double w = ws[k];
        double r = w;
        int j = 0;
        for (; j + 4 <= n; j += 4) {
            const double r0 = R[k + (i64)j * K], r1 = R[k + (i64)(j + 1) * K];
            const double r2 = R[k + (i64)(j + 2) * K], r3 = R[k + (i64)(j + 3) * K];
            r -= cs[j] * r0;
            r -= cs[j + 1] * r1;
            r -= cs[j + 2] * r2;
            r -= cs[j + 3] * r3;
        }
        for (; j < n; ++j) r -= cs[j] * R[k + (i64)j * K];
        rn[k] = r;
        vnext[k] = nipals ? w : r;
    }
}

}
```

Before: 756.6 components/s.

## Fold per-component update into head of next fused deflation pass

Splits the single-component update into p/critical/rest phases. Every block of the next fused pass now recomputes the small critical path (p, q, deflated XY, norm, new weight) from the reduction buffer and precomputes r·XY, so it no longer has to wait for a separate update kernel launch. One designated block writes the full update outputs (P, Q, W, R, XY) into alternate double-buffered XY and reduction storage. This removes a serialized tiny kernel and its launch gap between passes, at the cost of redundant per-block work, extra LDS barriers, and more complex pending-update bookkeeping.

```diff
diff --git a/pls_amd/csrc/ctx.hpp b/pls_amd/csrc/ctx.hpp
--- a/pls_amd/csrc/ctx.hpp
+++ b/pls_amd/csrc/ctx.hpp
@@ -71,6 +71,7 @@
     unsigned rg_epoch = 0;
     unsigned long long resident_launches = 0;
     struct Env {
+        int head_update = 1;
         bool turnaround = true;
         i64 turn_edge_bytes = plsk::TURN_EDGE_BYTES;
         bool batch_refit = false;
diff --git a/pls_amd/csrc/fused_kernels.hpp b/pls_amd/csrc/fused_kernels.hpp
--- a/pls_amd/csrc/fused_kernels.hpp
+++ b/pls_amd/csrc/fused_kernels.hpp
@@ -77,6 +77,16 @@
     double *XY = nullptr;
     double *W = nullptr, *P = nullptr, *Q = nullptr, *R = nullptr, *vnext = nullptr;
     int A = 0, a = 0, nipals = 0;
+    double *snext = nullptr;
+};
+
+struct HeadUpdate {
+    const double *red = nullptr;
+    const double *XY = nullptr;
+    double *XYn = nullptr;
+    double *W = nullptr, *P = nullptr, *Q = nullptr, *R = nullptr, *vnext = nullptr;
+    int A = 0, a = 0;
+    int bk = -1;
 };
 
 struct WalkWeights {
@@ -113,10 +123,28 @@
 constexpr int TAIL_MIN_WG = 32;
 constexpr int TAIL_AUX_SYS = 17;
 
+__device__ __forceinline__ void red_vec_ld(const double *src, i64 stride, int n, int sys, int L, int j, int h, double (&x)[RED_SLICES]) {
+    typedef unsigned int u32x2 __attribute__((ext_vector_type(2)));
+#pragma unroll
+    for (int m = 0; m < RED_SLICES; ++m) {
+        const int mm = h * RED_SLICES + m;
+        const __amdgpu_buffer_rsrc_t rs = __builtin_amdgcn_make_buffer_rsrc(
+            const_cast<double *>(src + (i64)(mm < n ? mm : 0) * stride), (short)0, L * 8, BUF_WORD3);
+        const u32x2 raw = sys ? __builtin_amdgcn_raw_buffer_load_b64(rs, (uint32_t)j * 8u, 0, TAIL_AUX_SYS)
+                              : __builtin_amdgcn_raw_buffer_load_b64(rs, (uint32_t)j * 8u, 0, AUX_SC1);
+        __builtin_memcpy(&x[m], &raw, 8);
+    }
+}
+__device__ __forceinline__ double red_vec_add(double sum, const double (&x)[RED_SLICES], int n, int h) {
+#pragma unroll
+    for (int m = 0; m < RED_SLICES; ++m)
+        if (h * RED_SLICES + m < n) sum += x[m];
+    return sum;
+}
+
 __device__ __noinline__ void tail_update_m1(const double *src, i64 stride, int n, int sys, int ok, double *XY, double *W, double *P,
                                             double *Q, double *R, double *vnext, int K, int A, int a, int nipals, double *scratch,
-                                            double *wl) {
-    typedef unsigned int u32x2 __attribute__((ext_vector_type(2)));
+                                            double *wl, double *snext) {
     static_assert(XCHG_MAX == 2 * RED_SLICES, "two batches of RED_SLICES loads");
     const int L = K + 1;
     update_m1<512, 1>(
@@ -126,22 +154,29 @@
             for (int h = 0; h < 2; ++h) {
                 if (h * RED_SLICES >= n) break;
                 double x[RED_SLICES];
-#pragma unroll
-                for (int m = 0; m < RED_SLICES; ++m) {
-                    const int mm = h * RED_SLICES + m;
-                    const __amdgpu_buffer_rsrc_t rs = __builtin_amdgcn_make_buffer_rsrc(
-                        const_cast<double *>(src + (i64)(mm < n ? mm : 0) * stride), (short)0, L * 8, BUF_WORD3);
-                    const u32x2 raw = sys ? __builtin_amdgcn_raw_buffer_load_b64(rs, (uint32_t)j * 8u, 0, TAIL_AUX_SYS)
-                                          : __builtin_amdgcn_raw_buffer_load_b64(rs, (uint32_t)j * 8u, 0, AUX_SC1);
-                    __builtin_memcpy(&x[m], &raw, 8);
-                }
-#pragma unroll
-                for (int m = 0; m < RED_SLICES; ++m)
-                    if (h * RED_SLICES + m < n) sum += x[m];
+                red_vec_ld(src, stride, n, sys, L, j, h, x);
+                sum = red_vec_add(sum, x, n, h);
             }
             return ok ? sum : __builtin_nan("");
         },
-        XY, W, P, Q, R, vnext, K, A, a, nipals, 0, scratch + UPD1_VWAVES, scratch, wl);
+        XY, W, P, Q, R, vnext, K, A, a, nipals, 0, scratch + UPD1_VWAVES, scratch, wl, snext);
+}
+
+struct HeadVals {
+    double p, q, xy, nrm;
+};
+__device__ __forceinline__ HeadVals head_update_m1(double sk, double tt, double xy, double rxy, int K, double *sm) {
+    double xv[2][1] = {{xy}, {0.0}}, pv[2][1];
+    upd1_p<512, 1>([&](int) { return sk; }, tt, K, pv);
+    double nrm = 0.0;
+    const double q = upd1_critical<512, 1, true>(rxy, tt, pv, xv, K, true, &nrm, sm);
+    return HeadVals{pv[0][0], q, xv[0][0], nrm};
+}
+__device__ __noinline__ void head_rest_m1(double p, double q, double xy, double nrm, double *XYn, double *W, double *P, double *Q,
+                                          double *R, double *vnext, int K, int A, int a, double *scratch, double *wl) {
+    const double xv[2][1] = {{xy}, {0.0}}, pv[2][1] = {{p}, {0.0}};
+    upd1_rest<512, 1>(xv, pv, q, nrm, XYn, W, P, Q, R, vnext, XYn + K, K, A, a, 1, 0, scratch + UPD1_VWAVES, scratch, wl);
+    __syncthreads();
 }
 
 template <int NT>
@@ -277,10 +312,10 @@
             *gx.status = 1;
             __hip_atomic_store(gx.host_status, 1, __ATOMIC_RELAXED, __HIP_MEMORY_SCOPE_SYSTEM);
         }
-        tail_update_m1(gx.inbox, gx.cap, gx.n, 1, ok, u.XY, u.W, u.P, u.Q, u.R, u.vnext, K, u.A, u.a, u.nipals, scratch, wl);
+        tail_update_m1(gx.inbox, gx.cap, gx.n, 1, ok, u.XY, u.W, u.P, u.Q, u.R, u.vnext, K, u.A, u.a, u.nipals, scratch, wl, u.snext);
         return;
     }
-    tail_update_m1(st.red, LP, RED_SLICES, 0, 1, u.XY, u.W, u.P, u.Q, u.R, u.vnext, K, u.A, u.a, u.nipals, scratch, wl);
+    tail_update_m1(st.red, LP, RED_SLICES, 0, 1, u.XY, u.W, u.P, u.Q, u.R, u.vnext, K, u.A, u.a, u.nipals, scratch, wl, u.snext);
 }
 
 constexpr int AUX_NT = 2;
@@ -316,7 +351,7 @@
     const T *X, i64 ldx, i64 tsx, T *dst, i64 ldd, i64 tsd, i64 N, int K,
     const double *__restrict__ v, const T *__restrict__ tprev, const double *__restrict__ pprev,
     T *__restrict__ tout, double *__restrict__ part, double *__restrict__ sspart, int rdst, i64 NV, const SliceTail st,
-    const WalkWeights wk) {
+    const WalkWeights wk, const HeadUpdate hu) {
     constexpr int RP = R / V;
     constexpr int CG = NT / RP;
     constexpr int NW = NT / WAVE;
@@ -342,9 +377,17 @@
     PLS_STAMP(0);
     constexpr bool LATE_OK = TILED && DEFL && CG * CPT <= NT;
     const bool LATE_FILL = LATE_OK && (rdst & 0x10000);
+    const bool HEAD = LATE_FILL && hu.red != nullptr;
     double v_late = 0.0, p_late = 0.0;
+    double hs[RED_SLICES] = {}, ht[RED_SLICES] = {}, hxy = 0.0, hrxy = 0.0;
     if (LATE_FILL) {
-        if (tid < CG * CPT) {
+        if (HEAD) {
+            static_assert(!LATE_OK || NT == 512, "head_update_m1 plays the update's 1024 virtual threads with 512");
+            red_vec_ld(hu.red, K + 1, RED_SLICES, 0, K + 1, tid, 0, hs);
+            red_vec_ld(hu.red, K + 1, RED_SLICES, 0, K + 1, K, 0, ht);
+            hxy = (tid < K) ? hu.XY[tid] : 0.0;
+            hrxy = hu.XY[K];
+        } else if (tid < CG * CPT) {
             v_late = (tid < K) ? v[tid] : 0.0;
             p_late = (tid < K) ? pprev[tid] : 0.0;
         }
@@ -983,7 +1026,8 @@
                       i64 N, int K, const double *v, const T *tprev, const double *pprev, T *tout,
                       double *part, int max_rows, double *sspart, int *nb, int *nss, int grid_hint, int rdst = 0,
                       bool src_padded = false, const SliceTail *tail = nullptr, bool *tail_used = nullptr,
-                      bool *upd_done = nullptr, bool store = true, const Turn &turn = Turn()) {
+                      bool *upd_done = nullptr, bool store = true, const Turn &turn = Turn(), const HeadUpdate *head = nullptr,
+                      bool *head_done = nullptr) {
     constexpr int V = 16 / sizeof(T);
     constexpr int R = tile_rows<T, CGX>(), NT = 512;
     constexpr int CG = NT / (R / V);
@@ -1008,6 +1052,8 @@
     i64 grid = 0;
     if (tail_used) *tail_used = false;
     if (upd_done) *upd_done = false;
+    if (head_done) *head_done = false;
+    if (head && head->red && Nf <= 0) return 2;
     if (Nf > 0) {
         const i64 ntiles = (Nf + R - 1) / R;
         const bool onewg = !defl && K <= CG * 16 && CGX <= 64 && edge == 0 && tail && tail->cnt && rdst == 0 &&
@@ -1029,6 +1075,15 @@
                 st.gx.n = 0;
             }
         }
+        const bool tiled = defl && edge == 0 && rdst == 0 && ldx == R && tsx == (i64)R * K && (!stores || (ldd == R && tsd == (i64)R * K));
+        HeadUpdate hu;
+        const bool head_ok = head && head->red && head_done && tiled && CGX <= 32 && K <= NT && Nf >= N && !st.upd.XY &&
+                             st.npush == 0 && 2 * (NT / WAVE) * R >= UPD1_VWAVES + head->A;
+        if (head && head->red && !head_ok) return 2;
+        if (head_ok) {
+            hu = *head;
+            if (hu.bk < 0 || hu.bk >= (int)grid) hu.bk = (int)grid - 1;
+        }
         if (Nf < N) {
             TailArgs<T> a;
             a.src = X; a.lds = ldx; a.tss = tsx; a.rs = R;
@@ -1040,7 +1095,6 @@
             a.row0 = Nf; a.nrows = (int)(N - Nf); a.K = K; a.zero_rows = V - a.nrows;
             launch_tail_rows(stream, a);
         }
-        const bool tiled = defl && edge == 0 && rdst == 0 && ldx == R && tsx == (i64)R * K && (!stores || (ldd == R && tsd == (i64)R * K));
         WalkWeights wk;
         {
             constexpr double rho = 1.08;
@@ -1069,13 +1123,16 @@
         if constexpr (!(DEFL_) && (CPT_) <= 16 && CGX <= 64 && (EDGE_) == 0) {                                            \
             if (onewg) {                                                                                                  \
                 auto kfn1 = &fused_pass_kernel<T, V, R, NT, CPT_, DEFL_, AUX_NT, AUX_NT, false, EDGE_, TILED_, true>;     \
-                hipLaunchKernelGGL(kfn1, g, b, dyn_, stream, X, ldx, tsx, dst, ldd, tsd, Nf, K, v, tprev, pprev, tout, part, sspart, 0, N, st, wk); \
+                hipLaunchKernelGGL(kfn1, g, b, dyn_, stream, X, ldx, tsx, dst, ldd, tsd, Nf, K, v, tprev, pprev, tout, part, sspart, 0, N, st, wk, HeadUpdate()); \
                 break;                                                                                                    \
             }                                                                                                             \
         }                                                                                                                 \
         auto kfn = &fused_pass_kernel<T, V, R, NT, CPT_, DEFL_, AUX_NT, AUX_NT, false, EDGE_, TILED_, false, STORE_>;    \
         if ((dyn_) > 48 * 1024 && !raise_dynamic_lds(reinterpret_cast<const void *>(kfn), (int)(dyn_))) return 1;         \
-        hipLaunchKernelGGL(kfn, g, b, dyn_, stream, X, ldx, tsx, dst, ldd, tsd, Nf, K, v, tprev, pprev, tout, part, sspart, (TILED_) ? ((STORE_) ? 2 * (CPT_) : 0) | 0x10000 : 0, N, st, wk); \
+        const bool hd_ = head_ok && (TILED_) && (DEFL_) && CG * (CPT_) <= NT;                  \
+        if (head_ok && !hd_) return -2;                            \
+        if (hd_) *head_done = true;                                                                                       \
+        hipLaunchKernelGGL(kfn, g, b, dyn_, stream, X, ldx, tsx, dst, ldd, tsd, Nf, K, v, tprev, pprev, tout, part, sspart, (TILED_) ? ((STORE_) ? 2 * (CPT_) : 0) | 0x10000 : 0, N, st, wk, hd_ ? hu : HeadUpdate()); \
     } while (0)
 #define FUSED_EDGE(CPT_, DEFL_, STORE_, dyn_)                                                                             \
     do {                                                                                                                  \
@@ -1100,7 +1157,7 @@
                 auto kfn = edge == 2 ? &fused_pass_kernel<T, V, R, NT, 32, true, AUX_NT, AUX_NT, true, 2>
                                      : (edge == 1 ? &fused_pass_kernel<T, V, R, NT, 32, true, AUX_NT, AUX_NT, true, 1>
                                                   : &fused_pass_kernel<T, V, R, NT, 32, true, AUX_NT, AUX_NT, true, 0>);
-                hipLaunchKernelGGL(kfn, g, b, 0, stream, X, ldx, tsx, dst, ldd, tsd, Nf, K, v, tprev, pprev, tout, part, sspart, rdst, N, st, wk);
+                hipLaunchKernelGGL(kfn, g, b, 0, stream, X, ldx, tsx, dst, ldd, tsd, Nf, K, v, tprev, pprev, tout, part, sspart, rdst, N, st, wk, HeadUpdate());
             } else if (K <= CG * 4) FUSED_CASE(4);
             else if (K <= CG * 8) FUSED_CASE(8);
             else if (K <= CG * 12) FUSED_CASE(12);
diff --git a/pls_amd/csrc/fused_pass_tile.inc b/pls_amd/csrc/fused_pass_tile.inc
--- a/pls_amd/csrc/fused_pass_tile.inc
+++ b/pls_amd/csrc/fused_pass_tile.inc
@@ -19,11 +19,20 @@
             if constexpr (LATE_OK) {
                 if (LATE_FILL && first_tile) {
                     first_tile = false;
+                    HeadVals hv{};
+                    if (HEAD) {
+                        hv = head_update_m1(red_vec_add(0.0, hs, RED_SLICES, 0), red_vec_add(0.0, ht, RED_SLICES, 0), hxy, hrxy, K,
+                                            &tred[0][0][0]);
+                        v_late = (tid < K) ? upd1_w(hv.xy, hv.nrm) : 0.0;
+                        p_late = hv.p;
+                    }
                     if (tid < CG * CPT) {
                         vs[tid] = v_late;
                         ps[tid] = p_late;
                     }
                     __syncthreads();
+                    if (HEAD && (int)blockIdx.x == hu.bk)
+                        head_rest_m1(hv.p, hv.q, hv.xy, hv.nrm, hu.XYn, hu.W, hu.P, hu.Q, hu.R, hu.vnext, K, hu.A, hu.a, &tred[0][0][0], vs);
                 }
             }
         } else {
diff --git a/pls_amd/csrc/launch_update.hpp b/pls_amd/csrc/launch_update.hpp
--- a/pls_amd/csrc/launch_update.hpp
+++ b/pls_amd/csrc/launch_update.hpp
@@ -90,8 +90,13 @@
     return !(n < A && n > 0 && (i64)n * K >= ROTATE_SPLIT_MIN);
 }
 
+bool update_emits_rxy(int K, int M, int A, int a) {
+    return M == 1 && K <= plsk::UPD1_KMAX && a >= 0 && a + 1 < A && update_is_single(K, M, A, a);
+}
+
 int launch_update(pls_hip_context *c, double *red, double *XY, double *W, double *P,
-                  double *Q, double *R, double *v, int K, int M, int A, int a, int nip, const plsk::XchgGather *gx = nullptr) {
+                  double *Q, double *R, double *v, int K, int M, int A, int a, int nip, const plsk::XchgGather *gx = nullptr,
+                  double *snext = nullptr) {
     const int n = a + 1;
     if (M > plsk::MMAX || (M > 8 && (i64)K * M >= 16384))
         return launch_update_large(c, (const double *)red, XY, W, P, Q, R, v, K, M, A, a, nip);
@@ -163,7 +168,7 @@
     } else {
         hipLaunchKernelGGL(plsk::component_update_kernel, dim3(1), dim3(plsk::UPD_THREADS),
                            (size_t)std::min(A, 4096) * sizeof(double), c->stream, (const double *)red, XY, W, P, Q, R, v, K, M, A, a, nip,
-                           (int)c->opt_power_iters, (int)split);
+                           (int)c->opt_power_iters, (int)split, split ? nullptr : snext);
     }
     LAUNCH_CHECK(c);
     if (split) {
diff --git a/pls_amd/csrc/plan_fit.hpp b/pls_amd/csrc/plan_fit.hpp
--- a/pls_amd/csrc/plan_fit.hpp
+++ b/pls_amd/csrc/plan_fit.hpp
@@ -10,21 +10,24 @@
     bool retiled = false;
     bool xx_local_done = false;
     int nip;
+    double *XY_alt = nullptr, *red_alt = nullptr;
 };
 
 template <typename T>
 int fit_workspace(pls_hip_context *c, const plsk::FitShape &shape, plsk::FitPlan &plan, FitWork<T> &w) {
     CHK(ensure(c, c->part, plan.part_bytes));
     CHK(ensure(c, c->sspart, plan.sspart_bytes));
-    CHK(ensure(c, c->xy, (size_t)shape.K * shape.M * 8));
+    const size_t xy_len = (size_t)shape.K * shape.M + 1;
+    CHK(ensure(c, c->xy, 2 * xy_len * 8));
     CHK(ensure(c, c->v, (size_t)shape.K * 8));
     CHK(ensure(c, c->cs, (size_t)shape.A * 8));
     if (c->user_red) {
         if (c->user_red_count < (i64)(plan.red_bytes / 8)) return fail(c, PLS_HIP_ERR_INVALID, "reduce buffer too small");
         w.red = c->user_red;
     } else {
-        CHK(ensure(c, c->red, plan.red_bytes));
+        CHK(ensure(c, c->red, 2 * plan.red_bytes));
         w.red = (double *)c->red.p;
+        w.red_alt = w.red + plan.red_bytes / 8;
     }
     if (plan.retile_fit && ensure(c, c->work, plan.work_bytes) != PLS_HIP_OK) {
         c->err.clear();
@@ -34,6 +37,7 @@
     w.part = (double *)c->part.p;
     w.sspart = (double *)c->sspart.p;
     w.XY = (double *)c->xy.p;
+    w.XY_alt = w.XY + xy_len;
     w.v = (double *)c->v.p;
     w.work = (T *)c->work.p;
     if (c->env.tail && c->opt_fuse && shape.N > 0) {
@@ -164,7 +168,19 @@
     bool tail_used, upd_done;
     bool store_x;
     plsk::Turn turn;
+    bool upd_pending = false;
+    double *pend_red = nullptr;
+    bool rxy_ok = false;
+    bool head_done;
 };
+
+template <typename T>
+int flush_update(pls_hip_context *c, const FitArgs<T> &f, FitWork<T> &w, PassState<T> &st, int a) {
+    if (!st.upd_pending) return PLS_HIP_OK;
+    st.upd_pending = false;
+    CHK(launch_update(c, st.pend_red, w.XY, f.W, f.P, f.Q, f.R, w.v, f.K, f.M, f.A, a - 1, w.nip, nullptr, w.XY + f.K));
+    return PLS_HIP_OK;
+}
 constexpr int PASS_NOT_COVERED = -1;
 
 template <typename T>
@@ -206,7 +222,14 @@
     const T *tprev = (nipals && a > 0) ? f.Tm + (i64)(a - 1) * f.ldt : nullptr;
     const double *pprev = (nipals && a > 0) ? f.P + (i64)(a - 1) * K : nullptr;
     int rc;
-    {
+    if (p.mid_cg && a >= 2) CHK(flush_update(c, f, w, st, a));
+    for (int attempt = 0; attempt < 2; ++attempt) {
+        plsk::HeadUpdate hu;
+        if (st.upd_pending) {
+            hu.red = st.pend_red; hu.XY = w.XY; hu.XYn = w.XY_alt;
+            hu.W = f.W; hu.P = f.P; hu.Q = f.Q; hu.R = f.R; hu.vnext = w.v; hu.A = f.A; hu.a = a - 1;
+            hu.bk = c->env.head_update == 2 ? 0 : -1;
+        }
         const i64 bytes = ((tprev && st.store_x) ? 2 : 1) * (i64)N * K * sizeof(T) +
                           (tprev ? 2 : 1) * (i64)N * sizeof(T) + (tprev ? 3 : 2) * (i64)K * 8;
         Scope s(c, PLS_HIP_FAM_FUSED, bytes);
@@ -219,9 +242,16 @@
                 return plsk::launch_fused_pass<T, decltype(cg)::value>(
                     c->stream, c->num_cu, st.Xc, st.ldc, st.tsc, (tprev && st.store_x) ? work : nullptr, p.ldw, p.tsw, N, K, w.v, tprev, pprev,
                     f.Tm + (i64)a * f.ldt, w.part, (int)p.prow, w.sspart, &nb, &nss, (int)c->opt_fused_grid,
-                    (p.mid_cg && tprev && st.store_x) ? (int)p.WR : 0, st.Xc == work, &w.tail, &st.tail_used, &st.upd_done, st.store_x, st.turn);
+                    (p.mid_cg && tprev && st.store_x) ? (int)p.WR : 0, st.Xc == work, &w.tail, &st.tail_used, &st.upd_done, st.store_x, st.turn,
+                    &hu, &st.head_done);
             });
         if (rc != 0) s.on = false;
+        if (rc != 2) break;
+        CHK(flush_update(c, f, w, st, a));
+    }
+    if (st.head_done) {
+        st.upd_pending = false;
+        std::swap(w.XY, w.XY_alt);
     }
     if (rc != 0) return fail(c, PLS_HIP_ERR_DEVICE, "fused pass launch failed");
     LAUNCH_CHECK(c);
@@ -337,7 +367,7 @@
     const Route routes[] = {pass_deferred<T>, pass_tall<T>, pass_short_tile<T>, pass_unfused<T>};
     for (int a = 0; a < A; ++a) {
         Range r_comp("component", a);
-        st.tail_used = st.upd_done = false;
+        st.tail_used = st.upd_done = st.head_done = false;
         const bool want_push = tail.cnt && p.xep_ok && update_is_single(K, M, A, a);
         const bool defl_pass = w.nip && a > 0;
         st.store_x = (a + 1 < A);
@@ -358,9 +388,17 @@
             }
             if (want_upd) tail.gx = exchange_gather(c, seq);
         }
+        const bool tall_route = p.fused_mode && !p.retile_fit && !(p.defer > 1) && !p.mid_cg;
+        if (st.upd_pending) {
+            st.pend_red = w.red;
+            std::swap(w.red, w.red_alt);
+            tail.red = w.red;
+            if (!tall_route || want_upd || N <= 0) CHK(flush_update(c, f, w, st, a));
+        }
         if (want_upd) {
             tail.upd.XY = w.XY; tail.upd.W = f.W; tail.upd.P = f.P; tail.upd.Q = f.Q; tail.upd.R = f.R; tail.upd.vnext = w.v;
             tail.upd.A = A; tail.upd.a = a; tail.upd.nipals = w.nip;
+            if (M == 1 && c->env.head_update) tail.upd.snext = w.XY + K;
         }
         if (N > 0) {
             int rc = PASS_NOT_COVERED;
@@ -370,14 +408,24 @@
         } else {
             HIPCHK(c, hipMemsetAsync(w.red, 0, (size_t)plsk::RED_SLICES * (K + 1) * 8, c->stream));
         }
-        if (st.upd_done) {
+        if (st.head_done) st.rxy_ok = true;
+        const bool defer_upd = c->env.head_update && w.nip && M == 1 && a >= 1 && a + 1 < A && N > 0 && !st.upd_done &&
+                               !want_push && !c->reducer && w.red_alt && tall_route && p.tiled_work && st.cur_tiled && K <= 512 &&
+                               st.rxy_ok && update_emits_rxy(K, M, A, a);
+        if (defer_upd) {
+            st.upd_pending = true;
+        } else if (st.upd_done) {
             if (want_push) ++*c->xep.seq;
+            st.rxy_ok = tail.upd.snext != nullptr;
         } else if (st.tail_used && want_push) {
             const plsk::XchgGather gx = exchange_gather(c, ++*c->xep.seq);
             CHK(launch_update(c, w.red, w.XY, f.W, f.P, f.Q, f.R, w.v, K, M, A, a, w.nip, &gx));
+            st.rxy_ok = false;
         } else {
             CHK(do_allreduce(c, w.red, (i64)plsk::RED_SLICES * (K + 1)));
-            CHK(launch_update(c, w.red, w.XY, f.W, f.P, f.Q, f.R, w.v, K, M, A, a, w.nip));
+            st.rxy_ok = c->env.head_update && w.nip && update_emits_rxy(K, M, A, a);
+            CHK(launch_update(c, w.red, w.XY, f.W, f.P, f.Q, f.R, w.v, K, M, A, a, w.nip, nullptr,
+                              st.rxy_ok ? w.XY + K : nullptr));
         }
     }
     if (f.B) {
diff --git a/pls_amd/csrc/pls_hip.hip b/pls_amd/csrc/pls_hip.hip
--- a/pls_amd/csrc/pls_hip.hip
+++ b/pls_amd/csrc/pls_hip.hip
@@ -117,6 +117,7 @@
         c->env.replica_guard = !off("PLS_HIP_REPLICA_GUARD");
         c->env.resident = !off("PLS_HIP_RESIDENT");
         c->env.turnaround = !off("PLS_HIP_TURNAROUND");
+        if (const char *e = getenv("PLS_HIP_HEAD_UPDATE")) c->env.head_update = atoi(e) >= 2 ? 2 : (atoi(e) == 0 ? 0 : 1);
 #ifdef PLS_HIP_TESTING
         if (const char *e = getenv("PLS_HIP_TEST_TURN_EDGE_BYTES")) c->env.turn_edge_bytes = atoll(e);
 #endif
diff --git a/pls_amd/csrc/small_kernels.hpp b/pls_amd/csrc/small_kernels.hpp
--- a/pls_amd/csrc/small_kernels.hpp
+++ b/pls_amd/csrc/small_kernels.hpp
@@ -344,7 +344,8 @@
                                              double *__restrict__ P, double *__restrict__ Q,
                                              double *__restrict__ R, double *__restrict__ vnext, int K,
                                              int M, int A, int a, int nipals, int power_iters,
-                                             int split_rotate, double *cs, UpdShared &sh) {
+                                             int split_rotate, double *cs, UpdShared &sh,
+                                             double *__restrict__ snext = nullptr) {
     double *sred = sh.sred, *qs = sh.qs, *Gs = sh.Gs, *Bs = sh.Bs, *Cs = sh.Cs;
     const int tid = threadIdx.x, lane = tid & 63, wv = tid >> 6;
 
@@ -361,10 +362,10 @@
     } else if (fast) {
         if (K <= UPD1_VTHREADS)
             update_m1<UPD_THREADS, 1>([&](int j) { return red_sum_n(red, nsl, K + 1, j); }, XY, W, P, Q, R, vnext, K, A, a, nipals,
-                                      split_rotate, cs, sred, (double *)nullptr);
+                                      split_rotate, cs, sred, (double *)nullptr, snext);
         else
             update_m1<UPD_THREADS, 4>([&](int j) { return red_sum_n(red, nsl, K + 1, j); }, XY, W, P, Q, R, vnext, K, A, a, nipals,
-                                      split_rotate, cs, sred, (double *)nullptr);
+                                      split_rotate, cs, sred, (double *)nullptr, snext);
         return;
     } else if (a < 0) {
         if (red)
@@ -488,11 +489,11 @@
     const double *__restrict__ red, double *__restrict__ XY, double *__restrict__ W,
     double *__restrict__ P, double *__restrict__ Q, double *__restrict__ R,
     double *__restrict__ vnext, int K, int M, int A, int a, int nipals, int power_iters,
-    int split_rotate) {
+    int split_rotate, double *__restrict__ snext) {
     extern __shared__ double cs[];
     __shared__ UpdShared sh;
     component_update_body(red, RED_SLICES, XY, W, P, Q, R, vnext, K, M, A, a, nipals, power_iters, split_rotate,
-                          cs, sh);
+                          cs, sh, snext);
 }
 
 constexpr int AUX_SYS = 17;
diff --git a/pls_amd/csrc/update_m1.hpp b/pls_amd/csrc/update_m1.hpp
--- a/pls_amd/csrc/update_m1.hpp
+++ b/pls_amd/csrc/update_m1.hpp
@@ -7,47 +7,61 @@
 constexpr int UPD1_VWAVES = UPD1_VTHREADS / WAVE;
 constexpr int UPD1_KMAX = 4 * UPD1_VTHREADS;
 
-template <int NT>
+template <int NT, bool LDSB = false>
 __device__ __forceinline__ double vblock_sum(const double (&x)[UPD1_VTHREADS / NT], double *sm) {
     constexpr int VT = UPD1_VTHREADS / NT, NW = NT / WAVE;
     double xs[VT];
 #pragma unroll
     for (int u = 0; u < VT; ++u) xs[u] = wave_sum(x[u]);
     const int w = threadIdx.x >> 6;
-    __syncthreads();
+    if constexpr (LDSB) lds_barrier(); else __syncthreads();
     if ((threadIdx.x & 63) == 0) {
 #pragma unroll
         for (int u = 0; u < VT; ++u) sm[w + u * NW] = xs[u];
     }
-    __syncthreads();
+    if constexpr (LDSB) lds_barrier(); else __syncthreads();
     double s = 0.0;
 #pragma unroll
     for (int i = 0; i < UPD1_VWAVES; ++i) s += sm[i];
     return s;
 }
 
-template <int NT, int KI, typename SumF>
-__device__ __forceinline__ void update_m1(SumF S, double *__restrict__ XY, double *__restrict__ W, double *__restrict__ P,
-                                          double *__restrict__ Q, double *__restrict__ R, double *__restrict__ vnext, int K, int A,
-                                          int a, int nipals, int split_rotate, double *cs, double *sm, double *wl) {
-    constexpr int VT = UPD1_VTHREADS / NT, NW = NT / WAVE;
-    const int tid = threadIdx.x, lane = tid & 63, wv = tid >> 6;
-    const double tt = S(K);
-    const double *ra = R + (i64)a * K;
-    double xv[VT][KI], pv[VT][KI], part[VT];
+template <int NT, int KI, typename RF>
+__device__ __forceinline__ double upd1_rxy(RF rv, const double (&xv)[UPD1_VTHREADS / NT][KI], int K, double *sm) {
+    constexpr int VT = UPD1_VTHREADS / NT;
+    const int tid = threadIdx.x;
+    double part[VT];
 #pragma unroll
     for (int u = 0; u < VT; ++u) {
         part[u] = 0.0;
 #pragma unroll
         for (int i = 0; i < KI; ++i) {
             const int k = tid + u * NT + i * UPD1_VTHREADS;
-            xv[u][i] = (k < K) ? XY[k] : 0.0;
-            pv[u][i] = (k < K) ? S(k) / tt : 0.0;
-            part[u] = fma((k < K) ? ra[k] : 0.0, xv[u][i], part[u]);
+            part[u] = fma((k < K) ? rv(k) : 0.0, xv[u][i], part[u]);
         }
     }
-    const double q = vblock_sum<NT>(part, sm) / tt;
-    if (tid == 0) Q[(i64)a] = q;
+    return vblock_sum<NT>(part, sm);
+}
+
+template <int NT, int KI, typename SumF>
+__device__ __forceinline__ void upd1_p(SumF S, double tt, int K, double (&pv)[UPD1_VTHREADS / NT][KI]) {
+    constexpr int VT = UPD1_VTHREADS / NT;
+    const int tid = threadIdx.x;
+#pragma unroll
+    for (int u = 0; u < VT; ++u)
+#pragma unroll
+        for (int i = 0; i < KI; ++i) {
+            const int k = tid + u * NT + i * UPD1_VTHREADS;
+            pv[u][i] = (k < K) ? S(k) / tt : 0.0;
+        }
+}
+
+template <int NT, int KI, bool LDSB = false>
+__device__ __forceinline__ double upd1_critical(double rxy, double tt, const double (&pv)[UPD1_VTHREADS / NT][KI],
+                                                double (&xv)[UPD1_VTHREADS / NT][KI], int K, bool next, double *nrm, double *sm) {
+    constexpr int VT = UPD1_VTHREADS / NT;
+    const int tid = threadIdx.x;
+    const double q = rxy / tt;
     double ssn[VT];
 #pragma unroll
     for (int u = 0; u < VT; ++u) {
@@ -56,16 +70,38 @@
         for (int i = 0; i < KI; ++i) {
             const int k = tid + u * NT + i * UPD1_VTHREADS;
             if (k < K) {
-                P[k + (i64)a * K] = pv[u][i];
                 xv[u][i] -= (pv[u][i] * q) * tt;
-                XY[k] = xv[u][i];
                 ssn[u] = fma(xv[u][i], xv[u][i], ssn[u]);
             }
         }
     }
+    if (next) *nrm = sqrt(vblock_sum<NT, LDSB>(ssn, sm));
+    return q;
+}
+
+__device__ __forceinline__ double upd1_w(double xy, double nrm) { return xy / nrm; }
+
+template <int NT, int KI>
+__device__ __forceinline__ void upd1_rest(const double (&xv)[UPD1_VTHREADS / NT][KI], const double (&pv)[UPD1_VTHREADS / NT][KI], double q,
+                                          double nrm, double *__restrict__ XYo, double *__restrict__ W, double *__restrict__ P,
+                                          double *__restrict__ Q, double *__restrict__ R, double *__restrict__ vnext,
+                                          double *__restrict__ snext, int K, int A, int a, int nipals, int split_rotate, double *cs,
+                                          double *sm, double *wl) {
+    constexpr int VT = UPD1_VTHREADS / NT, NW = NT / WAVE;
+    const int tid = threadIdx.x, lane = tid & 63, wv = tid >> 6;
+    if (tid == 0) Q[(i64)a] = q;
+#pragma unroll
+    for (int u = 0; u < VT; ++u)
+#pragma unroll
+        for (int i = 0; i < KI; ++i) {
+            const int k = tid + u * NT + i * UPD1_VTHREADS;
+            if (k < K) {
+                P[k + (i64)a * K] = pv[u][i];
+                XYo[k] = xv[u][i];
+            }
+        }
     const int n = a + 1;
     if (n >= A) return;
-    const double nrm = sqrt(vblock_sum<NT>(ssn, sm));
     double *wn = W + (i64)n * K;
 #pragma unroll
     for (int u = 0; u < VT; ++u)
@@ -73,7 +109,7 @@
         for (int i = 0; i < KI; ++i) {
             const int k = tid + u * NT + i * UPD1_VTHREADS;
             if (k < K) {
-                const double w = xv[u][i] / nrm;
+                const double w = upd1_w(xv[u][i], nrm);
                 wn[k] = w;
                 if (wl) wl[k] = w;
             }
@@ -114,6 +150,34 @@
         rn[k] = r;
         vnext[k] = nipals ? w : r;
     }
+    if (!snext) return;
+    __syncthreads();
+    const double s = upd1_rxy<NT, KI>([&](int k) { return rn[k]; }, xv, K, sm);
+    if (tid == 0) *snext = s;
+}
+
+template <int NT, int KI, typename SumF>
+__device__ __forceinline__ void update_m1(SumF S, double *__restrict__ XY, double *__restrict__ W, double *__restrict__ P,
+                                          double *__restrict__ Q, double *__restrict__ R, double *__restrict__ vnext, int K, int A,
+                                          int a, int nipals, int split_rotate, double *cs, double *sm, double *wl,
+                                          double *__restrict__ snext = nullptr) {
+    constexpr int VT = UPD1_VTHREADS / NT;
+    const int tid = threadIdx.x;
+    const double tt = S(K);
+    const double *ra = R + (i64)a * K;
+    double xv[VT][KI], pv[VT][KI];
+#pragma unroll
+    for (int u = 0; u < VT; ++u)
+#pragma unroll
+        for (int i = 0; i < KI; ++i) {
+            const int k = tid + u * NT + i * UPD1_VTHREADS;
+            xv[u][i] = (k < K) ? XY[k] : 0.0;
+        }
+    upd1_p<NT, KI>(S, tt, K, pv);
+    const double rxy = upd1_rxy<NT, KI>([&](int k) { return ra[k]; }, xv, K, sm);
+    double nrm = 0.0;
+    const double q = upd1_critical<NT, KI>(rxy, tt, pv, xv, K, a + 1 < A, &nrm, sm);
+    upd1_rest<NT, KI>(xv, pv, q, nrm, XY, W, P, Q, R, vnext, snext, K, A, a, nipals, split_rotate, cs, sm, wl);
 }
 
 }
```

Result: no change. 758.9 components/s, median of 6 (+0.3%).
